# ChenKaiXuSan/Skiing_Analysis_PyTorch

Hardware: AMD Instinct MI355X
Metric: 3D-pose frames/sec, 8-view 518px clips (higher is better)
Workload: dtype f16

## Files before the change

include/skimi.h:

```cpp
#ifndef SKIMI_H
#define SKIMI_H

#include <stddef.h>
#include <stdint.h>

#ifdef __cplusplus
extern "C" {
#endif

#define SKIMI_OK 0
#define SKIMI_ERR_ARG (-1)
#define SKIMI_ERR_HIP (-2)
#define SKIMI_ERR_STATE (-3)
#define SKIMI_ERR_WORKSPACE (-4)

#define SKIMI_F32 0
#define SKIMI_BF16 1
#define SKIMI_BF16X3_REC 2
#define SKIMI_FP8MX 3
#define SKIMI_F16 4

#define SKIMI_PREC_BF16 0
#define SKIMI_PREC_BF16X3 1
#define SKIMI_PREC_FP8 2
#define SKIMI_PREC_F16 3

#define SKIMI_ACT_NONE 0
#define SKIMI_ACT_RELU 1
#define SKIMI_ACT_GELU 2
#define SKIMI_ACT_SILU 3
#define SKIMI_ACT_SIGMOID 4

const char* skimi_last_error(void);
int skimi_version(void);
int skimi_sizeof_gemm_desc(void);
int skimi_device_count(void);

int skimi_profile_start(int32_t kind, int64_t min_size);
int skimi_profile_stop(double* total_ms, int64_t* launches, double* flops, double* bytes);

typedef struct skimi_gemm_desc {
    int32_t M, N, K;
    const void* A;
    const void* W;
    int32_t a_dtype, w_dtype;
    int64_t lda, ldw;
    int32_t prec;
    int32_t a_mode;
    int32_t cN, cH, cW, cC, KH, KW, stride, pad, dil, OH, OW;
    const float* bias;
    const float* gamma;
    const void* resid;
    int32_t resid_dtype;
    int64_t ldr;
    int32_t resid_rows_per_batch;
    int64_t resid_batch_stride;
    int64_t resid_row_off;
    int32_t act;
    const void* resid2;
    int64_t ldr2;
    int32_t post_act;
    int32_t out_rows_per_batch;
    int64_t out_batch_stride;
    int64_t out_row_off;
    void* out;
    void* out2;
    int32_t out_dtype;
    int64_t ldo, ldo2;
    int32_t store_mode, ps_s, ps_C;
    void* splitk_scratch;
    uint64_t splitk_scratch_bytes;
    int32_t force_splitk;
    int32_t splitk_scratch_zeroed;
    const void* W_split;
    void* x3_scratch;
    uint64_t x3_scratch_bytes;
    void* out_records;
} skimi_gemm_desc;

int skimi_split_planes(const float* x, int64_t ld, int64_t rows, int32_t C, void* hi, void* lo, void* stream);

int skimi_split_records(const float* x, int64_t ld, int64_t rows, int32_t C, void* records, void* stream);

int skimi_dpt_fold_pack(const float* w_T, const float* b_T, const float* w_rn, int32_t C_in, int32_t C_mid, int32_t C_out,
                        int32_t s, void* w_records, float* beta, void* stream);

int skimi_gemm(const skimi_gemm_desc* d, void* stream);

#define SKIMI_GEMM_PATH_GENERIC 1
#define SKIMI_GEMM_PATH_SPLITK_ORDERED 2
#define SKIMI_GEMM_PATH_SPLITK_ATOMIC 3
#define SKIMI_GEMM_PATH_X3DMA_WIDE 4
#define SKIMI_GEMM_PATH_X3DMA_NARROW 5
#define SKIMI_GEMM_PATH_GEMM256 6
#define SKIMI_GEMM_PATH_CONV_WIN 7
int32_t skimi_gemm_last_path(void);

int skimi_quant_mx(const void* x, int32_t dtype, int64_t ldx, int64_t rows, int32_t K, void* payload, void* scales,
                   void* stream);
int skimi_layernorm_mx(const float* x, int64_t ldx, int64_t rows, int32_t C, const float* gamma, const float* beta,
                       float eps, void* payload, void* scales, void* stream);
int skimi_gemm_fp8(const void* A, const void* A_scales, const void* W, const void* W_scales, int32_t M, int32_t N,
                   int32_t K, const float* bias, int32_t act, const float* gamma, const float* resid, int64_t ldr,
                   void* out, int32_t out_dtype, int64_t ldo, void* out_scales, void* stream);

int skimi_conv3x3_n32_pack(const float* w, void* packed, int32_t C, void* stream);
int skimi_conv3x3_n32(const void* in_hi, const void* in_lo, const void* packed_w, const float* bias, float* out,
                      int32_t F, int32_t H, int32_t W, int32_t C, int32_t relu, void* stream);
int skimi_conv3x3_n32_strided(const void* in_hi, const void* in_lo, const void* packed_w, const float* bias, float* out,
                              int32_t F, int32_t H, int32_t W, int32_t C, int32_t relu, int64_t px_stride, void* stream);

int skimi_resample_u8(const uint8_t* in, uint8_t* out, int64_t outer, int32_t n_in, int32_t n_out, int64_t inner,
                      const int32_t* kk, const int32_t* bounds, int32_t ksize, void* stream);
int skimi_u8_hwc_to_f32_chw(const uint8_t* in, int32_t H, int32_t W, float* out, int32_t OH, int32_t OW, int32_t y_off,
                            int32_t x_off, float fill, void* stream);

int skimi_layernorm(const float* x, const float* x2, int64_t ldx, int64_t rows, int32_t C,
                    const float* gamma, const float* beta, float eps,
                    void* out, int32_t out_dtype, int64_t ldo, void* stream);

int skimi_qknorm_rope(void* qkv, int32_t dtype, int64_t tokens, int32_t heads,
                      const float* qn_w, const float* qn_b, const float* kn_w, const float* kn_b,
                      float eps, const int32_t* pos, const float* rope_cos, const float* rope_sin,
                      int32_t rope_npos, void* stream);

int skimi_attention(const void* qkv, void* out, int32_t dtype, int32_t batch, int32_t seq,
                    int32_t heads, int32_t head_dim, void* stream);
int skimi_attention_out(const void* qkv, void* out, int32_t dtype, int32_t out_dtype, int32_t batch, int32_t seq,
                        int32_t heads, int32_t head_dim, void* stream);

int skimi_qknorm_rope_scaled(void* qkv, int32_t dtype, int64_t tokens, int32_t heads,
                             const float* qn_w, const float* qn_b, const float* kn_w, const float* kn_b,
                             float eps, const int32_t* pos, const float* rope_cos, const float* rope_sin,
                             int32_t rope_npos, float q_scale, int32_t* q_scaled, void* stream);
int skimi_attention_ex(const void* qkv, void* out, int32_t dtype, int32_t out_dtype, int32_t batch, int32_t seq,
                       int32_t heads, int32_t head_dim, int32_t q_prescaled, void* x3_scratch,
                       uint64_t x3_scratch_bytes, int32_t* out_records, void* stream);
uint64_t skimi_attention_x3_scratch_bytes(int64_t tokens, int64_t row_elems);
void skimi_attention_last_plan(int32_t out[8]);

int skimi_layernorm_ex(const float* x, const float* x2, int64_t ldx, int64_t in_rows, int64_t rows, int32_t C,
                       const float* gamma, const float* beta, float eps, void* out, int32_t out_dtype, int64_t ldo,
                       int64_t grp_rows, int64_t grp_stride, int64_t grp_off, void* stream);
int skimi_attention_f32_strided(const float* q, const float* k, const float* v, float* out, const int64_t* q_strides,
                                const int64_t* k_strides, const int64_t* v_strides, const int64_t* o_strides,
                                int32_t batch, int32_t batch_inner, int32_t heads, int32_t seq_q, int32_t seq_k,
                                int32_t head_dim, float scale, void* stream);

typedef struct skimi_vp3d skimi_vp3d;

skimi_vp3d* skimi_vp3d_create(int32_t joints_in, int32_t in_features, int32_t joints_out,
                              const int32_t* filter_widths, int32_t n_widths,
                              int32_t channels, int32_t causal);
skimi_vp3d* skimi_vp3d_create_ex(int32_t joints_in, int32_t in_features, int32_t joints_out,
                                 const int32_t* filter_widths, int32_t n_widths,
                                 int32_t channels, int32_t causal, int32_t dense);
void skimi_vp3d_destroy(skimi_vp3d*);
int skimi_vp3d_set_weight(skimi_vp3d*, const char* key, const float* host_data, int64_t n);
int skimi_vp3d_finalize(skimi_vp3d*, int32_t prec);
int32_t skimi_vp3d_receptive_field(const skimi_vp3d*);
size_t skimi_vp3d_workspace_bytes(const skimi_vp3d*, int32_t batch, int32_t frames_in);
int skimi_vp3d_forward(skimi_vp3d*, const float* x, float* out, int32_t batch, int32_t frames_in,
                       void* workspace, size_t workspace_bytes, void* stream);

typedef struct skimi_vggt skimi_vggt;

typedef struct skimi_vggt_config {
    int32_t patch_size, embed_dim, depth, num_heads, num_register_tokens;
    int32_t use_dino;
    int32_t dino_depth, dino_heads, dino_img_size;
    int32_t cam_trunk_depth, cam_heads, cam_iters;
    int32_t dpt_features, dpt_out_channels[4], dpt_layers[4];
    int32_t track_features, track_hidden, track_corr_levels, track_corr_radius, track_iters, track_depth,
        track_heads, track_virtual;
    int32_t enable_camera, enable_depth, enable_point, enable_track;
    int32_t prec;
    int32_t head_prec;
} skimi_vggt_config;

skimi_vggt* skimi_vggt_create(const skimi_vggt_config* cfg);
void skimi_vggt_destroy(skimi_vggt*);
int skimi_vggt_set_weight(skimi_vggt*, const char* key, const float* data, int64_t n, int32_t on_device);
int skimi_vggt_finalize(skimi_vggt*);
int skimi_vggt_set_pos_embed(skimi_vggt*, int32_t H, int32_t W, const float* pos_embed, int32_t on_device);
size_t skimi_vggt_workspace_bytes(skimi_vggt*, int32_t B, int32_t S, int32_t H, int32_t W, int32_t n_query);
int skimi_vggt_rope_positions(skimi_vggt*, int32_t frames, int32_t H, int32_t W, int32_t* positions);

typedef struct skimi_vggt_outputs {
    float* pose_enc;
    float* pose_enc_list;
    float* depth;
    float* depth_conf;
    float* world_points;
    float* world_points_conf;
    float* track;
    float* vis;
    float* conf;
    float* tokens_last;
} skimi_vggt_outputs;

int skimi_vggt_forward(skimi_vggt*, const float* images, const float* query_points, int32_t B, int32_t S,
                       int32_t H, int32_t W, int32_t n_query, const skimi_vggt_outputs* out,
                       void* workspace, size_t workspace_bytes, void* stream);

int skimi_pose_to_cameras(const float* pose_enc, int64_t rows, int32_t H, int32_t W, float* extrinsic,
                          float* intrinsic, void* stream);
int skimi_unproject_depth(const float* depth, const float* extrinsic, const float* intrinsic,
                          float* world_points, int32_t frames, int32_t H, int32_t W, void* stream);
int skimi_triangulate_dlt(const float* K, const float* R, const float* t, const float* keypoints,
                          float* joints3d, int64_t steps, int32_t views, int32_t joints, void* stream);

int skimi_triangulate_triage(const float* K, const float* R, const float* t, const float* keypoints, const float* conf,
                             double conf_thr, double err_thresh_px, int64_t steps, int32_t views, int32_t joints,
                             float* joints3d, float* joints3d_clean, double* err, double* depth, uint8_t* keep,
                             double* view_stats, double* report, void* stream);

int skimi_triangulate_robust(const float* K, const float* R, const float* t, const float* keypoints, const float* conf,
                             double conf_thr, double inlier_px, int32_t min_inliers, int32_t refine_iters, int32_t weighted,
                             int64_t steps, int32_t views, int32_t joints, float* joints3d, double* err,
                             uint8_t* inlier_views, double* rms_px, uint8_t* ok, float* joints3d_ok,
                             double* view_inlier_ratio, double* report, void* stream);

size_t skimi_person_workspace_bytes(int64_t maps, int32_t H, int32_t W);
int skimi_person_origin(const float* points, const float* boxes, int64_t maps, int32_t H, int32_t W, int32_t src_h,
                        int32_t src_w, void* workspace, double* stats, void* stream);
int skimi_recenter_cameras(const double* stats, const float* extrinsic, int64_t steps, int32_t views, double* origin_out,
                           float* R_out, float* t_out, void* stream);

size_t skimi_icp_workspace_bytes(int64_t n_src, int64_t n_tgt);
int skimi_estimate_normals(const float* points, int64_t n, double radius, double* normals_out,
                           int32_t* neighbour_count_out, void* ws, size_t ws_bytes, void* stream);
int skimi_icp_correspondences(const float* src, int64_t n_src, const float* tgt, int64_t n_tgt, const double* T4x4,
                              double max_dist, int32_t* tgt_index_out, void* ws, size_t ws_bytes, void* stream);
int skimi_icp_point_to_plane(const float* src, int64_t n_src, const float* tgt, int64_t n_tgt, double max_corr_dist,
                             double normal_radius, int32_t max_iteration, double rel_fitness, double rel_rmse,
                             const double* init4x4, double* T_out, double* fitness_out, double* rmse_out,
                             int32_t* iterations_out, void* ws, size_t ws_bytes, void* stream);

#define SKIMI_BA_POSE_ONLY 0
#define SKIMI_BA_POSE_CAM_T 1
#define SKIMI_BA_FULL 2
#define SKIMI_BA_AUTO 0
#define SKIMI_BA_LDS 1
#define SKIMI_BA_WORKSPACE 2
size_t skimi_ba_workspace_bytes(int64_t T, int32_t C, int32_t J, int32_t modes);
int skimi_bundle_adjust(const double* K, const double* R0, const double* t0, const double* X0, const double* x2d,
                        const double* conf, int64_t T, int32_t C, int32_t J, const int32_t* modes, int32_t n_modes,
                        int32_t num_iters, double lr, double w_reproj, double w_smooth, double w_baseline,
                        double w_bone_length, double w_pose_temporal, int32_t placement, double* R_out, double* t_out,
                        double* X_out, double* history_out, void* ws, size_t ws_bytes, void* stream);

#define SKIMI_RESECT_LINEAR 0
#define SKIMI_RESECT_SOFT_L1 1
size_t skimi_resect_workspace_bytes(int64_t n_points, int32_t views, int64_t group_size);
int skimi_resect_cameras(const double* X, const double* x2d, const double* conf, const double* K, const double* R0,
                         const double* t0, int64_t n_points, int32_t views, int64_t group_size, int32_t loss, double f_scale,
                         double min_conf, int32_t max_evals, double* R, double* t, double* K_out, double* cost0, double* cost,
                         int32_t* n_evals, int32_t* n_used, int32_t* success, double* err, double* stats, void* ws,
                         size_t ws_bytes, void* stream);
int skimi_relative_pose(const double* R, const double* t, int64_t groups, int32_t views, double* R_rel, double* t_rel,
                        void* stream);

size_t skimi_refine_workspace_bytes(int64_t n_points, int32_t views, int64_t group_size);
int skimi_refine_cameras_points(const double* X, const double* x2d, const double* conf, const double* K, const double* R0,
                                const double* t0, int64_t n_points, int32_t views, int64_t group_size, double lambda_x,
                                int32_t loss, double f_scale, double min_conf, int32_t max_evals, double* R, double* t,
                                double* K_out, double* X_opt, double* cost0, double* cost, int32_t* n_evals, int32_t* n_used,
                                int32_t* success, double* err, double* stats, double* moved, void* ws, size_t ws_bytes,
                                void* stream);

size_t skimi_essential_workspace_bytes(int64_t n_points, int64_t group_size, int32_t hypotheses);
int skimi_essential_ransac(const double* x2d, const double* conf, const double* K, int64_t n_points, int64_t group_size,
                           double min_conf, double threshold, int32_t hypotheses, uint64_t seed, int64_t group_offset,
                           double baseline, double distance_thresh, double* R, double* t, double* E, uint8_t* inliers,
                           uint8_t* pose_mask, int32_t* n_used, int32_t* n_inliers, int32_t* n_pose, int32_t* cheirality,
                           double* cost, int32_t* winner, int32_t* n_solutions, double* confidence, int32_t* success,
                           void* ws, size_t ws_bytes, void* stream);
int skimi_five_point(const double* a, const double* b, int64_t samples, double* E, int32_t* counts, void* stream);

int64_t skimi_scene_tile(int64_t n);
size_t skimi_scene_workspace_bytes(int64_t B, int64_t n);
int skimi_scene_cloud(const float* points, const float* conf, const float* images, const float* extrinsic, int64_t B, int32_t S,
                      int32_t H, int32_t W, int32_t images_nchw, double conf_thres, int32_t mask_black_bg, int32_t mask_white_bg,
                      int32_t align, int64_t cap, void* workspace, float* xyz, uint8_t* rgb, int64_t* count, double* stats,
                      double* transform, void* stream);

int skimi_fuse_h36m(const double* left, const double* right, int64_t frames, double tau, const double* tau_j, const double* wL,
                    int64_t wL_stride, const double* wR, int64_t wR_stride, int32_t allow_scale, int32_t mirror_right_x,
                    double* fused, double* R, double* t, double* s, double* diag, int32_t* status, void* stream);

#define SKIMI_FUSE_SCALE_HIP 0
#define SKIMI_FUSE_SCALE_TORSO 1
int skimi_fuse_views(const double* X_l, const double* X_r, const double* U_l, const double* U_r, int64_t frames, int32_t joints,
                     int32_t root_idx, int32_t left_hip_idx, int32_t right_hip_idx, int32_t left_shoulder_idx,
                     int32_t right_shoulder_idx, double sigma_px, double sigma_3d, int32_t scale_mode, int32_t min_points,
                     double* fused, double* aligned, double* q_l, double* q_r, double* conf_l, double* conf_r, double* conf_x,
                     double* err_l, double* err_r, double* dist, int32_t* fit_ok, void* stream);

int skimi_smooth_ema(const double* X, int64_t frames, int64_t joints, const double* base, int32_t adaptive, double alpha_min,
                     double alpha_max, double speed_gain, double* Y, void* stream);

int skimi_smooth_ema_batch(const double* X, int64_t clips, int64_t frames, int64_t joints, const double* base, int32_t adaptive,
                           double alpha_min, double alpha_max, double speed_gain, double* Y, void* stream);

size_t skimi_fuse_group_workspace_bytes(int64_t views, int64_t frames, int32_t joints);
int skimi_fuse_group(const double* X, const double* U, const double* quality, int64_t views, int64_t frames, int32_t joints,
                     int32_t root_idx, int32_t left_hip_idx, int32_t right_hip_idx, int32_t left_shoulder_idx,
                     int32_t right_shoulder_idx, double sigma_px, double sigma_3d, int32_t scale_mode, int32_t min_points,
                     int32_t align, void* workspace, size_t workspace_bytes, double* fused, double* aligned, double* q_a, double* q_b,
                     double* conf_x, double* dist, double* conf, double* err, int32_t* fit_ok, void* stream);

int skimi_joint_quality(const double* X, const double* U, int64_t views, int64_t frames, int32_t joints, const int32_t* edges,
                        int32_t n_edges, const double* size, double beta_temp, double w_bone, double w_temp, double w_san,
                        int32_t med_given, const double* bias, int64_t bias_stride, double* med_lens, double* q, double* q_bone,
                        double* q_temp, double* q_san, void* stream);

#define SKIMI_SKELETON_COCO_TO_H36M 0
#define SKIMI_SKELETON_H36M_TO_COCO 1
int skimi_convert_skeleton(const double* X, int64_t frames, int32_t coords, int32_t direction, int32_t synthesize, double* Y,
                           void* stream);

int skimi_smooth_savgol(const double* X, int64_t frames, int64_t joints, int32_t win, int32_t poly, const double* fir,
                        const double* first, const double* last, double* Y, void* stream);

#define SKIMI_KIN_SERIES 42
#define SKIMI_KIN_BASE_SERIES 14
#define SKIMI_KIN_ROLES 13
#define SKIMI_KIN_LDS_FRAMES 2048
enum {
    SKIMI_KIN_SHOULDER_L = 0, SKIMI_KIN_SHOULDER_R, SKIMI_KIN_ELBOW_L, SKIMI_KIN_ELBOW_R, SKIMI_KIN_HIP_L, SKIMI_KIN_HIP_R,
    SKIMI_KIN_KNEE_L, SKIMI_KIN_KNEE_R, SKIMI_KIN_FOOT_L, SKIMI_KIN_FOOT_R, SKIMI_KIN_HAND_L, SKIMI_KIN_HAND_R, SKIMI_KIN_NECK
};
size_t skimi_kin_workspace_bytes(int64_t clips, int64_t frames);
int skimi_kinematics(const double* X, const int32_t* lengths, int64_t clips, int64_t frames, int32_t joints,
                     const int32_t* layout, const double* up, int32_t min_turn_frames, double min_heading_change_deg,
                     int32_t heading_window, int32_t velocity_window, int32_t max_turns, void* workspace,
                     size_t workspace_bytes, double* series, double* heading, double* heading_smooth, double* velocity_smooth,
                     uint8_t* boundary, int32_t* n_turns, int32_t* turn_frames, double* turn_heading_change,
                     int32_t* turn_direction, double* turn_stats, int32_t* turn_counts, void* stream);

#define SKIMI_EVAL_MAX_JOINTS 128
#define SKIMI_EVAL_MAX_EDGES 128
#define SKIMI_EVAL_MAX_PAIRS 64
#define SKIMI_EVAL_LDS_ELEMS 1440
enum { SKIMI_PE_MPJPE = 0, SKIMI_PE_P_MPJPE, SKIMI_PE_N_MPJPE, SKIMI_PE_MPJVE };
enum {
    SKIMI_CQ_BONE_CV_POOLED = 0, SKIMI_CQ_BONE_CV_MEAN, SKIMI_CQ_LR_LENGTH_SYMMETRY, SKIMI_CQ_SPEED_MEAN, SKIMI_CQ_JERK_MEAN,
    SKIMI_CQ_SPEED_P95, SKIMI_CQ_ACCEL_P95, SKIMI_CQ_MIRROR_SYMMETRY, SKIMI_CQ_SCALARS
};
size_t skimi_eval_workspace_bytes(int64_t clips, int64_t frames, int32_t joints);
int skimi_pose_errors(const double* pred, const double* target, const int32_t* lengths, int64_t clips, int64_t frames, int32_t joints,
                      int32_t zero_root, double* err, double* p_err, double* vel_err, double* mpjpe_f, double* n_mpjpe_f,
                      double* p_mpjpe_f, int32_t* n_valid_f, int32_t* p_status, double* aligned, double* p_R, double* p_scale,
                      double* p_t, double* metrics, int32_t* counts, double* joint_stats, int32_t* joint_n, void* stream);
int skimi_clip_quality(const double* X, const int32_t* lengths, int64_t clips, int64_t frames, int32_t joints, const int32_t* edges,
                       int32_t n_edges, const int32_t* left_edges, int32_t n_left, const int32_t* right_edges, int32_t n_right,
                       const int32_t* lr_pairs, int32_t n_pairs, void* workspace, size_t workspace_bytes, double* scalars,
                       double* bone_cv_edge, double* bone_len, void* stream);

#define SKIMI_LENS_MAX_CAMERAS 8
#define SKIMI_LENS_MAX_ITERS 1000
#define SKIMI_LENS_MAX_SIDE 32768
int skimi_distort_points(const double* x, const double* K, const double* dist, const double* P, const double* K_steps,
                         int64_t outer, int32_t C, int64_t n, int32_t normalized, double* out, void* stream);
int skimi_undistort_points(const double* x, const double* K, const double* dist, const double* P, const double* K_steps,
                           int64_t outer, int32_t C, int64_t n, int32_t iters, int32_t normalized, double* out, double* resid_px,
                           void* stream);
int skimi_project_points(const double* X, const double* R, const double* t, const double* K, const double* dist, int64_t outer,
                         int32_t C, int64_t n, double* px, double* depth, void* stream);
int skimi_undistort_u8(const uint8_t* in, uint8_t* out, const double* K, const double* dist, const double* new_K, int32_t C,
                       int32_t F, int32_t H, int32_t W, int32_t OH, int32_t OW, int32_t ch, void* stream);

int skimi_homography_fit(const double* src, const double* dst, const double* post, int64_t G, int32_t n, double* H, double* Hinv,
                         double* Hn, double* err, double* stats, int32_t* status, void* stream);
int skimi_homography_points(const double* x, const double* H, int64_t G, int64_t n, int32_t shared, double eps, double* out,
                            void* stream);
int skimi_warp_perspective_u8(const uint8_t* in, uint8_t* out, const double* Hinv, int32_t per_frame, int32_t C, int32_t F,
                              int32_t H, int32_t W, int32_t OH, int32_t OW, int32_t ch, void* stream);
int skimi_bev_skeleton(const double* X, const double* center_px, const double* center_world_in, int64_t T, int32_t J,
                       double metres_per_pixel, int32_t ax0, int32_t ax1, int32_t rot90_left, double* uv, int32_t* px, uint8_t* valid,
                       double* center_world, void* stream);
int skimi_ground_track(const double* p, int64_t P, int64_t T, double fps, double* out, void* stream);

size_t skimi_calibrate_workspace_bytes(int64_t G, int32_t V, int32_t n);
int skimi_calibrate_camera(const double* obj, const double* img, const uint8_t* use, const double* K0, const double* dist0, int64_t G,
                           int32_t V, int32_t n, int32_t width, int32_t height, int32_t free_mask, int32_t max_evals, double* K,
                           double* dist, double* R, double* t, double* rvec, double* err, double* view_stats, double* rms,
                           double* cost0, double* cost, double* std, int32_t* n_evals, int32_t* n_views, int32_t* n_corners,
                           int32_t* success, void* ws, size_t ws_bytes, void* stream);

#define SKIMI_CHESS_MAX_PIXELS (1 << 28)
#define SKIMI_CHESS_MAX_NMS 15
#define SKIMI_SUBPIX_MAX_WIN 15
#define SKIMI_SUBPIX_MAX_ITERS 1000
size_t skimi_chess_workspace_bytes(int64_t N, int32_t H, int32_t W);
int skimi_chess_candidates(const uint8_t* frames, int64_t N, int32_t H, int32_t W, int32_t ch, int32_t threshold, int32_t nms_radius,
                           int32_t max_candidates, int32_t* xy, int32_t* response, int32_t* count, int32_t* rmax, void* ws,
                           size_t ws_bytes, void* stream);
int skimi_corner_subpix(const uint8_t* frames, int64_t N, int32_t H, int32_t W, int32_t ch, const double* points, const int32_t* count,
                        int32_t M, int32_t win_x, int32_t win_y, int32_t iters, double* out, uint8_t* ok, void* stream);

#define SKIMI_ORB_MAX_LEVELS 8
#define SKIMI_ORB_MAX_FEATURES 4096
#define SKIMI_ORB_BORDER 16
#define SKIMI_ORB_PATTERN_SEED 0x534B494D494F5242ULL
#define SKIMI_ORB_COS                                                                                                          \
    {16384, 16069, 15137, 13623, 11585, 9102, 6270, 3196, 0, -3196, -6270, -9102, -11585, -13623, -15137, -16069, -16384, -16069, \
     -15137, -13623, -11585, -9102, -6270, -3196, 0, 3196, 6270, 9102, 11585, 13623, 15137, 16069}
#define SKIMI_ORB_SIN                                                                                                          \
    {0, 3196, 6270, 9102, 11585, 13623, 15137, 16069, 16384, 16069, 15137, 13623, 11585, 9102, 6270, 3196, 0, -3196, -6270, -9102, \
     -11585, -13623, -15137, -16069, -16384, -16069, -15137, -13623, -11585, -9102, -6270, -3196}
size_t skimi_orb_workspace_bytes(int64_t N, int32_t H, int32_t W, int32_t levels);
int skimi_orb_features(const uint8_t* frames, int64_t N, int32_t H, int32_t W, int32_t ch, int32_t levels, int32_t threshold,
                       int32_t max_features, const double* roi, const int8_t* pattern, int32_t* xy_level, double* xy,
                       int32_t* level, int32_t* direction, int32_t* score, int64_t* harris, int32_t* desc, int32_t* count,
                       int32_t* level_count, void* ws, size_t ws_bytes, void* stream);
int skimi_match_hamming(const int32_t* d1, const int32_t* n1, int32_t M1, const int32_t* d2, const int32_t* n2, int32_t M2,
                        int64_t B, int32_t cross_check, double ratio, int32_t max_distance, int32_t max_matches, int32_t* pairs,
                        int32_t* dist, int32_t* count, void* stream);

#define SKIMI_SIFT_MAX_OCTAVES 8
#define SKIMI_SIFT_MAX_FEATURES 4096
#define SKIMI_SIFT_MAX_CANDIDATES 32768
#define SKIMI_SIFT_BORDER 5
#define SKIMI_SIFT_MIN_SIDE 16
#define SKIMI_SIFT_MAX_RADIUS 13
#define SKIMI_SIFT_RADII {7, 5, 7, 8, 10, 13}
#define SKIMI_SIFT_PRETHRESH 1.7f
#define SKIMI_SIFT_CONTRAST 3.4
#define SKIMI_SIFT_CBRT4 1.5874010519681994
#define SKIMI_SIFT_LN2 0.6931471805599453
size_t skimi_sift_workspace_bytes(int64_t N, int32_t H, int32_t W, int32_t octaves);
int skimi_sift_features(const uint8_t* frames, int64_t N, int32_t H, int32_t W, int32_t ch, int32_t octaves, int32_t max_features,
                        const double* roi, const float* taps, double* xy, int32_t* xy_level, int32_t* octave, int32_t* layer,
                        double* sigma, double* response, double* angle, uint8_t* desc, int32_t* count, int32_t* octave_count,
                        void* ws, size_t ws_bytes, void* stream);
int skimi_match_l2(const uint8_t* d1, const int32_t* n1, int32_t M1, const uint8_t* d2, const int32_t* n2, int32_t M2, int64_t B,
                   int32_t cross_check, double ratio, int32_t max_distance2, int32_t max_matches, int32_t* pairs, int32_t* dist2,
                   int32_t* second2, int32_t* count, void* ws, size_t ws_bytes, void* stream);


int skimi_resize_bilinear(const void* in, void* out, int32_t dtype, int32_t out_dtype, int32_t N, int32_t h, int32_t w,
                          int32_t H, int32_t W, int32_t C, const float* tabx, const float* taby, const float* ln_g,
                          const float* ln_b, float ln_eps, void* stream);
int skimi_resize_bilinear_planes(const float* in, void* out, int32_t N, int32_t h, int32_t w, int32_t H, int32_t W,
                                 int32_t C, const float* tabx, const float* taby, int32_t slice_records, void* zpage,
                                 void* stream);
int skimi_add_uv_pos(void* x, int32_t dtype, const float* tabx, const float* taby, int32_t N, int32_t H, int32_t W,
                     int32_t C, void* stream);
int skimi_add_uv_pos_records(const float* x, const float* tabx, const float* taby, int32_t N, int32_t H, int32_t W,
                             int32_t C, void* rec, void* stream);
int skimi_dpt_out(const void* in, int32_t dtype, const float* W, const float* b, int32_t n_out, float* pts, float* conf,
                  int64_t npix, int32_t mode, void* stream);
int skimi_patch_gather(const float* img, void* out, int32_t out_dtype, int32_t F, int32_t H, int32_t W, int32_t p,
                       int32_t Kp, void* stream);
int skimi_adaln(const float* xn, const float* x, const float* mod, float* out, int64_t rows, int32_t D, void* stream);
int skimi_pose_update(const float* delta, float* pred_pad, float* act_out, int64_t rows, int32_t first, void* stream);
int skimi_special_tokens(float* x, const float* table, int32_t F, int32_t S, int32_t P, int32_t n, int32_t C, void* stream);

int skimi_track_avgpool2(const float* in, float* out, int32_t N, int32_t H, int32_t W, int32_t C, void* stream);
int skimi_track_sample_border(const float* fmap, int64_t img_stride, const float* coords, int64_t coord_stride, float* out,
                              int32_t B, int32_t N, int32_t H, int32_t W, int32_t C, void* stream);
int skimi_track_corr_sample(const float* tgt, const float* fmap, const float* coords, float* out, int64_t rows, int32_t N,
                            int32_t S, int32_t H, int32_t W, int32_t C, int32_t r, int32_t level, int64_t ldo,
                            int32_t out_off, void* stream);
int skimi_track_pos_embed_sample(const float* coords, int64_t coord_stride, float* out, int32_t BN, int32_t H, int32_t W,
                                 int32_t D, void* stream);
int skimi_track_input(const float* coords, const float* fcorr, const float* tfeat, const float* pos, const float* qrt,
                      float* x, int64_t rows, int32_t S, int32_t L, int64_t ldx, float max_scale, void* stream);
int skimi_track_coord_update(float* coords, const float* delta, int64_t ldd, const float* query, float* pred, int64_t rows,
                             int32_t N, int32_t S, float stride, void* stream);
int skimi_track_init(const float* q, float* coords, float* qs, int64_t BN, int32_t S, float stride, void* stream);
int skimi_track_repeat_rows(const float* src, float* dst, int64_t BN, int32_t S, int32_t C, void* stream);
int skimi_track_bns_to_bsn(const float* in, float* out, int32_t B, int32_t N, int32_t S, void* stream);


int skimi_vp3d_pack_weights(const float* w_host, int32_t N, int32_t Npad, int32_t K, void* dst);
int skimi_vp3d_stream_mm(const void* wrec, int32_t Npad, const void* xrec, const float* bias, const float* resid, int32_t resid_L,
                         int32_t resid_off, float* out_f32, int32_t ldo, void* out_rec, int32_t B, int32_t Lin, int32_t C,
                         int32_t taps, int32_t dil, int32_t N, int32_t relu, int32_t force_family, int32_t force_ct,
                         int32_t force_nw, int32_t force_ms, void* stream);
int skimi_vp3d_stream_win(const void* wrec, int32_t Npad, const void* xrec, const float* bias, float* out_f32, int32_t ldo,
                          void* out_rec, int32_t B, int32_t Lin, int32_t C, int32_t taps, int32_t N, int32_t force_ta,
                          int32_t force_msc, void* stream);
int skimi_vp3d_stream_expand(const float* x, const void* w, int32_t ldw, const float* bias, float* out_f32, void* out_rec,
                             int32_t B, int32_t Lin, int32_t Cin, int32_t taps, int32_t C, int32_t valu, int32_t force_ms,
                             void* stream);
void skimi_vp3d_last_plan(int32_t out[8]);

#ifdef __cplusplus
}
#endif
#endif
```

skiing_analysis_pytorch_amd/_lib.py:

```python
from __future__ import annotations

import ctypes as C
from pathlib import Path

LIB_PATH = Path(__file__).resolve().parent / "lib" / "libskimi.so"

F32, BF16 = 0, 1
F16 = 4
BF16X3_REC = 2
FP8MX = 3
PREC_BF16, PREC_BF16X3, PREC_FP8 = 0, 1, 2
PREC_F16 = 3
ACT_NONE, ACT_RELU, ACT_GELU, ACT_SILU, ACT_SIGMOID = 0, 1, 2, 3, 4
GEMM_PATH_GENERIC, GEMM_PATH_SPLITK_ORDERED, GEMM_PATH_SPLITK_ATOMIC = 1, 2, 3
GEMM_PATH_X3DMA_WIDE, GEMM_PATH_X3DMA_NARROW, GEMM_PATH_GEMM256, GEMM_PATH_CONV_WIN = 4, 5, 6, 7
VP3D_CONV, VP3D_MM, VP3D_WIN, VP3D_EXPAND_MFMA, VP3D_EXPAND_VALU = 1, 2, 3, 4, 5


class SkimiError(RuntimeError):
    pass


class GemmDesc(C.Structure):

    _fields_ = [
        ("M", C.c_int32), ("N", C.c_int32), ("K", C.c_int32),
        ("A", C.c_void_p), ("W", C.c_void_p),
        ("a_dtype", C.c_int32), ("w_dtype", C.c_int32),
        ("lda", C.c_int64), ("ldw", C.c_int64),
        ("prec", C.c_int32),
        ("a_mode", C.c_int32),
        ("cN", C.c_int32), ("cH", C.c_int32), ("cW", C.c_int32), ("cC", C.c_int32),
        ("KH", C.c_int32), ("KW", C.c_int32), ("stride", C.c_int32), ("pad", C.c_int32),
        ("dil", C.c_int32), ("OH", C.c_int32), ("OW", C.c_int32),
        ("bias", C.c_void_p), ("gamma", C.c_void_p), ("resid", C.c_void_p),
        ("resid_dtype", C.c_int32),
        ("ldr", C.c_int64),
        ("resid_rows_per_batch", C.c_int32),
        ("resid_batch_stride", C.c_int64),
        ("resid_row_off", C.c_int64),
        ("act", C.c_int32),
        ("resid2", C.c_void_p), ("ldr2", C.c_int64), ("post_act", C.c_int32),
        ("out_rows_per_batch", C.c_int32), ("out_batch_stride", C.c_int64), ("out_row_off", C.c_int64),
        ("out", C.c_void_p), ("out2", C.c_void_p),
        ("out_dtype", C.c_int32),
        ("ldo", C.c_int64), ("ldo2", C.c_int64),
        ("store_mode", C.c_int32), ("ps_s", C.c_int32), ("ps_C", C.c_int32),
        ("splitk_scratch", C.c_void_p),
        ("splitk_scratch_bytes", C.c_uint64),
        ("force_splitk", C.c_int32), ("splitk_scratch_zeroed", C.c_int32),
        ("W_split", C.c_void_p), ("x3_scratch", C.c_void_p), ("x3_scratch_bytes", C.c_uint64),
        ("out_records", C.c_void_p),
    ]


_vp = C.c_void_p
_SIGNATURES = {
    "skimi_last_error": (C.c_char_p, []),
    "skimi_version": (C.c_int, []),
    "skimi_sizeof_gemm_desc": (C.c_int, []),
    "skimi_device_count": (C.c_int, []),
    "skimi_profile_start": (C.c_int, [C.c_int32, C.c_int64]),
    "skimi_profile_stop": (C.c_int, [C.POINTER(C.c_double), C.POINTER(C.c_int64), C.POINTER(C.c_double),
                                    C.POINTER(C.c_double)]),
    "skimi_gemm": (C.c_int, [C.POINTER(GemmDesc), _vp]),
    "skimi_gemm_last_path": (C.c_int32, []),
    "skimi_dpt_fold_pack": (C.c_int, [_vp, _vp, _vp, C.c_int32, C.c_int32, C.c_int32, C.c_int32, _vp, _vp, _vp]),
    "skimi_quant_mx": (C.c_int, [_vp, C.c_int32, C.c_int64, C.c_int64, C.c_int32, _vp, _vp, _vp]),
    "skimi_layernorm_mx": (C.c_int, [_vp, C.c_int64, C.c_int64, C.c_int32, _vp, _vp, C.c_float, _vp, _vp, _vp]),
    "skimi_gemm_fp8": (C.c_int, [_vp, _vp, _vp, _vp, C.c_int32, C.c_int32, C.c_int32, _vp, C.c_int32, _vp, _vp, C.c_int64,
                                 _vp, C.c_int32, C.c_int64, _vp, _vp]),
    "skimi_split_planes": (C.c_int, [_vp, C.c_int64, C.c_int64, C.c_int32, _vp, _vp, _vp]),
    "skimi_split_records": (C.c_int, [_vp, C.c_int64, C.c_int64, C.c_int32, _vp, _vp]),
    "skimi_resample_u8": (C.c_int, [_vp, _vp, C.c_int64, C.c_int32, C.c_int32, C.c_int64, _vp, _vp, C.c_int32, _vp]),
    "skimi_u8_hwc_to_f32_chw": (C.c_int, [_vp, C.c_int32, C.c_int32, _vp, C.c_int32, C.c_int32, C.c_int32, C.c_int32,
                                          C.c_float, _vp]),
    "skimi_conv3x3_n32_pack": (C.c_int, [_vp, _vp, C.c_int32, _vp]),
    "skimi_conv3x3_n32": (C.c_int, [_vp, _vp, _vp, _vp, _vp, C.c_int32, C.c_int32, C.c_int32, C.c_int32, C.c_int32, _vp]),
    "skimi_conv3x3_n32_strided": (C.c_int, [_vp, _vp, _vp, _vp, _vp, C.c_int32, C.c_int32, C.c_int32, C.c_int32, C.c_int32,
                                            C.c_int64, _vp]),
    "skimi_layernorm": (C.c_int, [_vp, _vp, C.c_int64, C.c_int64, C.c_int32, _vp, _vp, C.c_float, _vp,
                                  C.c_int32, C.c_int64, _vp]),
    "skimi_qknorm_rope": (C.c_int, [_vp, C.c_int32, C.c_int64, C.c_int32, _vp, _vp, _vp, _vp, C.c_float,
                                    _vp, _vp, _vp, C.c_int32, _vp]),
    "skimi_attention": (C.c_int, [_vp, _vp, C.c_int32, C.c_int32, C.c_int32, C.c_int32, C.c_int32, _vp]),
    "skimi_attention_out": (C.c_int, [_vp, _vp, C.c_int32, C.c_int32, C.c_int32, C.c_int32, C.c_int32, C.c_int32, _vp]),
    "skimi_qknorm_rope_scaled": (C.c_int, [_vp, C.c_int32, C.c_int64, C.c_int32, _vp, _vp, _vp, _vp, C.c_float,
                                           _vp, _vp, _vp, C.c_int32, C.c_float, C.POINTER(C.c_int32), _vp]),
    "skimi_attention_ex": (C.c_int, [_vp, _vp, C.c_int32, C.c_int32, C.c_int32, C.c_int32, C.c_int32, C.c_int32, C.c_int32,
                                     _vp, C.c_uint64, C.POINTER(C.c_int32), _vp]),
    "skimi_attention_x3_scratch_bytes": (C.c_uint64, [C.c_int64, C.c_int64]),
    "skimi_attention_last_plan": (None, [C.POINTER(C.c_int32)]),
    "skimi_layernorm_ex": (C.c_int, [_vp, _vp, C.c_int64, C.c_int64, C.c_int64, C.c_int32, _vp, _vp, C.c_float, _vp,
                                     C.c_int32, C.c_int64, C.c_int64, C.c_int64, C.c_int64, _vp]),
    "skimi_attention_f32_strided": (C.c_int, [_vp, _vp, _vp, _vp, C.POINTER(C.c_int64), C.POINTER(C.c_int64),
                                              C.POINTER(C.c_int64), C.POINTER(C.c_int64), C.c_int32, C.c_int32, C.c_int32,
                                              C.c_int32, C.c_int32, C.c_int32, C.c_float, _vp]),
    "skimi_vp3d_create": (_vp, [C.c_int32, C.c_int32, C.c_int32, C.POINTER(C.c_int32), C.c_int32,
                                C.c_int32, C.c_int32]),
    "skimi_vp3d_create_ex": (_vp, [C.c_int32, C.c_int32, C.c_int32, C.POINTER(C.c_int32), C.c_int32,
                                   C.c_int32, C.c_int32, C.c_int32]),
    "skimi_vp3d_destroy": (None, [_vp]),
    "skimi_vp3d_set_weight": (C.c_int, [_vp, C.c_char_p, _vp, C.c_int64]),
    "skimi_vp3d_finalize": (C.c_int, [_vp, C.c_int32]),
    "skimi_vp3d_receptive_field": (C.c_int32, [_vp]),
    "skimi_vp3d_workspace_bytes": (C.c_size_t, [_vp, C.c_int32, C.c_int32]),
    "skimi_vp3d_forward": (C.c_int, [_vp, _vp, _vp, C.c_int32, C.c_int32, _vp, C.c_size_t, _vp]),
    "skimi_vp3d_pack_weights": (C.c_int, [_vp, C.c_int32, C.c_int32, C.c_int32, _vp]),
    "skimi_vp3d_stream_mm": (C.c_int, [_vp, C.c_int32, _vp, _vp, _vp, C.c_int32, C.c_int32, _vp, C.c_int32, _vp, C.c_int32,
                                       C.c_int32, C.c_int32, C.c_int32, C.c_int32, C.c_int32, C.c_int32, C.c_int32, C.c_int32,
                                       C.c_int32, C.c_int32, _vp]),
    "skimi_vp3d_stream_win": (C.c_int, [_vp, C.c_int32, _vp, _vp, _vp, C.c_int32, _vp, C.c_int32, C.c_int32, C.c_int32,
                                        C.c_int32, C.c_int32, C.c_int32, C.c_int32, _vp]),
    "skimi_vp3d_stream_expand": (C.c_int, [_vp, _vp, C.c_int32, _vp, _vp, _vp, C.c_int32, C.c_int32, C.c_int32, C.c_int32,
                                           C.c_int32, C.c_int32, C.c_int32, _vp]),
    "skimi_vp3d_last_plan": (None, [C.POINTER(C.c_int32)]),
    "skimi_pose_to_cameras": (C.c_int, [_vp, C.c_int64, C.c_int32, C.c_int32, _vp, _vp, _vp]),
    "skimi_unproject_depth": (C.c_int, [_vp, _vp, _vp, _vp, C.c_int32, C.c_int32, C.c_int32, _vp]),
    "skimi_triangulate_dlt": (C.c_int, [_vp, _vp, _vp, _vp, _vp, C.c_int64, C.c_int32, C.c_int32, _vp]),
    "skimi_triangulate_triage": (C.c_int, [_vp, _vp, _vp, _vp, _vp, C.c_double, C.c_double, C.c_int64, C.c_int32, C.c_int32,
                                           _vp, _vp, _vp, _vp, _vp, _vp, _vp, _vp]),
    "skimi_triangulate_robust": (C.c_int, [_vp, _vp, _vp, _vp, _vp, C.c_double, C.c_double, C.c_int32, C.c_int32, C.c_int32,
                                           C.c_int64, C.c_int32, C.c_int32, _vp, _vp, _vp, _vp, _vp, _vp, _vp, _vp, _vp]),
    "skimi_person_workspace_bytes": (C.c_size_t, [C.c_int64, C.c_int32, C.c_int32]),
    "skimi_person_origin": (C.c_int, [_vp, _vp, C.c_int64, C.c_int32, C.c_int32, C.c_int32, C.c_int32, _vp, _vp, _vp]),
    "skimi_recenter_cameras": (C.c_int, [_vp, _vp, C.c_int64, C.c_int32, _vp, _vp, _vp, _vp]),
    "skimi_icp_workspace_bytes": (C.c_size_t, [C.c_int64, C.c_int64]),
    "skimi_estimate_normals": (C.c_int, [_vp, C.c_int64, C.c_double, _vp, _vp, _vp, C.c_size_t, _vp]),
    "skimi_icp_correspondences": (C.c_int, [_vp, C.c_int64, _vp, C.c_int64, C.POINTER(C.c_double), C.c_double, _vp, _vp,
                                            C.c_size_t, _vp]),
    "skimi_icp_point_to_plane": (C.c_int, [_vp, C.c_int64, _vp, C.c_int64, C.c_double, C.c_double, C.c_int32, C.c_double,
                                           C.c_double, C.POINTER(C.c_double), C.POINTER(C.c_double), C.POINTER(C.c_double),
                                           C.POINTER(C.c_double), C.POINTER(C.c_int32), _vp, C.c_size_t, _vp]),
    "skimi_ba_workspace_bytes": (C.c_size_t, [C.c_int64, C.c_int32, C.c_int32, C.c_int32]),
    "skimi_bundle_adjust": (C.c_int, [_vp, _vp, _vp, _vp, _vp, _vp, C.c_int64, C.c_int32, C.c_int32, C.POINTER(C.c_int32),
                                      C.c_int32, C.c_int32, C.c_double, C.c_double, C.c_double, C.c_double, C.c_double,
                                      C.c_double, C.c_int32, _vp, _vp, _vp, _vp, _vp, C.c_size_t, _vp]),
    "skimi_resect_workspace_bytes": (C.c_size_t, [C.c_int64, C.c_int32, C.c_int64]),
    "skimi_resect_cameras": (C.c_int, [_vp, _vp, _vp, _vp, _vp, _vp, C.c_int64, C.c_int32, C.c_int64, C.c_int32, C.c_double,
                                       C.c_double, C.c_int32, _vp, _vp, _vp, _vp, _vp, _vp, _vp, _vp, _vp, _vp, _vp, C.c_size_t,
                                       _vp]),
    "skimi_relative_pose": (C.c_int, [_vp, _vp, C.c_int64, C.c_int32, _vp, _vp, _vp]),
    "skimi_refine_workspace_bytes": (C.c_size_t, [C.c_int64, C.c_int32, C.c_int64]),
    "skimi_refine_cameras_points": (C.c_int, [_vp, _vp, _vp, _vp, _vp, _vp, C.c_int64, C.c_int32, C.c_int64, C.c_double, C.c_int32,
                                              C.c_double, C.c_double, C.c_int32, _vp, _vp, _vp, _vp, _vp, _vp, _vp, _vp, _vp, _vp,
                                              _vp, _vp, _vp, C.c_size_t, _vp]),
    "skimi_essential_workspace_bytes": (C.c_size_t, [C.c_int64, C.c_int64, C.c_int32]),
    "skimi_essential_ransac": (C.c_int, [_vp, _vp, _vp, C.c_int64, C.c_int64, C.c_double, C.c_double, C.c_int32, C.c_uint64,
                                         C.c_int64, C.c_double, C.c_double, _vp, _vp, _vp, _vp, _vp, _vp, _vp, _vp, _vp, _vp, _vp,
                                         _vp, _vp, _vp, _vp, C.c_size_t, _vp]),
    "skimi_five_point": (C.c_int, [_vp, _vp, C.c_int64, _vp, _vp, _vp]),
    "skimi_scene_tile": (C.c_int64, [C.c_int64]),
    "skimi_scene_workspace_bytes": (C.c_size_t, [C.c_int64, C.c_int64]),
    "skimi_scene_cloud": (C.c_int, [_vp, _vp, _vp, _vp, C.c_int64, C.c_int32, C.c_int32, C.c_int32, C.c_int32, C.c_double,
                                    C.c_int32, C.c_int32, C.c_int32, C.c_int64, _vp, _vp, _vp, _vp, _vp, _vp, _vp]),
    "skimi_fuse_h36m": (C.c_int, [_vp, _vp, C.c_int64, C.c_double, _vp, _vp, C.c_int64, _vp, C.c_int64, C.c_int32, C.c_int32,
                                  _vp, _vp, _vp, _vp, _vp, _vp, _vp]),
    "skimi_fuse_views": (C.c_int, [_vp, _vp, _vp, _vp, C.c_int64, C.c_int32, C.c_int32, C.c_int32, C.c_int32, C.c_int32, C.c_int32,
                                   C.c_double, C.c_double, C.c_int32, C.c_int32, _vp, _vp, _vp, _vp, _vp, _vp, _vp, _vp, _vp, _vp,
                                   _vp, _vp]),
    "skimi_smooth_ema": (C.c_int, [_vp, C.c_int64, C.c_int64, _vp, C.c_int32, C.c_double, C.c_double, C.c_double, _vp, _vp]),
    "skimi_smooth_ema_batch": (C.c_int, [_vp, C.c_int64, C.c_int64, C.c_int64, _vp, C.c_int32, C.c_double, C.c_double, C.c_double,
                                         _vp, _vp]),
    "skimi_fuse_group_workspace_bytes": (C.c_size_t, [C.c_int64, C.c_int64, C.c_int32]),
    "skimi_fuse_group": (C.c_int, [_vp, _vp, _vp, C.c_int64, C.c_int64, C.c_int32, C.c_int32, C.c_int32, C.c_int32, C.c_int32,
                                   C.c_int32, C.c_double, C.c_double, C.c_int32, C.c_int32, C.c_int32, _vp, C.c_size_t, _vp, _vp,
                                   _vp, _vp, _vp, _vp, _vp, _vp, _vp, _vp]),
    "skimi_joint_quality": (C.c_int, [_vp, _vp, C.c_int64, C.c_int64, C.c_int32, _vp, C.c_int32, _vp, C.c_double, C.c_double,
                                      C.c_double, C.c_double, C.c_int32, _vp, C.c_int64, _vp, _vp, _vp, _vp, _vp, _vp]),
    "skimi_convert_skeleton": (C.c_int, [_vp, C.c_int64, C.c_int32, C.c_int32, C.c_int32, _vp, _vp]),
    "skimi_smooth_savgol": (C.c_int, [_vp, C.c_int64, C.c_int64, C.c_int32, C.c_int32, _vp, _vp, _vp, _vp, _vp]),
    "skimi_kin_workspace_bytes": (C.c_size_t, [C.c_int64, C.c_int64]),
    "skimi_kinematics": (C.c_int, [_vp, _vp, C.c_int64, C.c_int64, C.c_int32, C.POINTER(C.c_int32), C.POINTER(C.c_double), C.c_int32,
                                   C.c_double, C.c_int32, C.c_int32, C.c_int32, _vp, C.c_size_t, _vp, _vp, _vp, _vp, _vp, _vp, _vp, _vp,
                                   _vp, _vp, _vp, _vp]),
    "skimi_eval_workspace_bytes": (C.c_size_t, [C.c_int64, C.c_int64, C.c_int32]),
    "skimi_pose_errors": (C.c_int, [_vp, _vp, _vp, C.c_int64, C.c_int64, C.c_int32, C.c_int32, _vp, _vp, _vp, _vp, _vp, _vp, _vp, _vp,
                                    _vp, _vp, _vp, _vp, _vp, _vp, _vp, _vp, _vp]),
    "skimi_clip_quality": (C.c_int, [_vp, _vp, C.c_int64, C.c_int64, C.c_int32, C.POINTER(C.c_int32), C.c_int32, C.POINTER(C.c_int32),
                                     C.c_int32, C.POINTER(C.c_int32), C.c_int32, C.POINTER(C.c_int32), C.c_int32, _vp, C.c_size_t, _vp,
                                     _vp, _vp, _vp]),
    "skimi_distort_points": (C.c_int, [_vp, _vp, _vp, _vp, _vp, C.c_int64, C.c_int32, C.c_int64, C.c_int32, _vp, _vp]),
    "skimi_undistort_points": (C.c_int, [_vp, _vp, _vp, _vp, _vp, C.c_int64, C.c_int32, C.c_int64, C.c_int32, C.c_int32, _vp, _vp,
                                         _vp]),
    "skimi_project_points": (C.c_int, [_vp, _vp, _vp, _vp, _vp, C.c_int64, C.c_int32, C.c_int64, _vp, _vp, _vp]),
    "skimi_undistort_u8": (C.c_int, [_vp, _vp, _vp, _vp, _vp, C.c_int32, C.c_int32, C.c_int32, C.c_int32, C.c_int32, C.c_int32,
                                     C.c_int32, _vp]),
    "skimi_homography_fit": (C.c_int, [_vp, _vp, _vp, C.c_int64, C.c_int32, _vp, _vp, _vp, _vp, _vp, _vp, _vp]),
    "skimi_homography_points": (C.c_int, [_vp, _vp, C.c_int64, C.c_int64, C.c_int32, C.c_double, _vp, _vp]),
    "skimi_warp_perspective_u8": (C.c_int, [_vp, _vp, _vp, C.c_int32, C.c_int32, C.c_int32, C.c_int32, C.c_int32, C.c_int32,
                                            C.c_int32, C.c_int32, _vp]),
    "skimi_bev_skeleton": (C.c_int, [_vp, _vp, _vp, C.c_int64, C.c_int32, C.c_double, C.c_int32, C.c_int32, C.c_int32, _vp, _vp, _vp,
                                     _vp, _vp]),
    "skimi_ground_track": (C.c_int, [_vp, C.c_int64, C.c_int64, C.c_double, _vp, _vp]),
    "skimi_calibrate_workspace_bytes": (C.c_size_t, [C.c_int64, C.c_int32, C.c_int32]),
    "skimi_calibrate_camera": (C.c_int, [_vp, _vp, _vp, _vp, _vp, C.c_int64, C.c_int32, C.c_int32, C.c_int32, C.c_int32, C.c_int32,
                                         C.c_int32, _vp, _vp, _vp, _vp, _vp, _vp, _vp, _vp, _vp, _vp, _vp, _vp, _vp, _vp, _vp, _vp,
                                         C.c_size_t, _vp]),
    "skimi_chess_workspace_bytes": (C.c_size_t, [C.c_int64, C.c_int32, C.c_int32]),
    "skimi_chess_candidates": (C.c_int, [_vp, C.c_int64, C.c_int32, C.c_int32, C.c_int32, C.c_int32, C.c_int32, C.c_int32, _vp, _vp,
                                         _vp, _vp, _vp, C.c_size_t, _vp]),
    "skimi_corner_subpix": (C.c_int, [_vp, C.c_int64, C.c_int32, C.c_int32, C.c_int32, _vp, _vp, C.c_int32, C.c_int32, C.c_int32,
                                      C.c_int32, _vp, _vp, _vp]),
    "skimi_orb_workspace_bytes": (C.c_size_t, [C.c_int64, C.c_int32, C.c_int32, C.c_int32]),
    "skimi_orb_features": (C.c_int, [_vp, C.c_int64, C.c_int32, C.c_int32, C.c_int32, C.c_int32, C.c_int32, C.c_int32, _vp, _vp, _vp,
                                     _vp, _vp, _vp, _vp, _vp, _vp, _vp, _vp, _vp, C.c_size_t, _vp]),
    "skimi_match_hamming": (C.c_int, [_vp, _vp, C.c_int32, _vp, _vp, C.c_int32, C.c_int64, C.c_int32, C.c_double, C.c_int32,
                                      C.c_int32, _vp, _vp, _vp, _vp]),
    "skimi_sift_workspace_bytes": (C.c_size_t, [C.c_int64, C.c_int32, C.c_int32, C.c_int32]),
    "skimi_sift_features": (C.c_int, [_vp, C.c_int64, C.c_int32, C.c_int32, C.c_int32, C.c_int32, C.c_int32, _vp, _vp, _vp, _vp, _vp,
                                      _vp, _vp, _vp, _vp, _vp, _vp, _vp, _vp, C.c_size_t, _vp]),
    "skimi_match_l2": (C.c_int, [_vp, _vp, C.c_int32, _vp, _vp, C.c_int32, C.c_int64, C.c_int32, C.c_double, C.c_int32, C.c_int32,
                                 _vp, _vp, _vp, _vp, _vp, C.c_size_t, _vp]),
    "skimi_resize_bilinear": (C.c_int, [_vp, _vp, C.c_int32, C.c_int32, C.c_int32, C.c_int32, C.c_int32, C.c_int32, C.c_int32, C.c_int32, _vp, _vp, _vp, _vp, C.c_float, _vp]),
    "skimi_resize_bilinear_planes": (C.c_int, [_vp, _vp, C.c_int32, C.c_int32, C.c_int32, C.c_int32, C.c_int32, C.c_int32, _vp, _vp, C.c_int32, _vp, _vp]),
    "skimi_add_uv_pos": (C.c_int, [_vp, C.c_int32, _vp, _vp, C.c_int32, C.c_int32, C.c_int32, C.c_int32, _vp]),
    "skimi_add_uv_pos_records": (C.c_int, [_vp, _vp, _vp, C.c_int32, C.c_int32, C.c_int32, C.c_int32, _vp, _vp]),
    "skimi_dpt_out": (C.c_int, [_vp, C.c_int32, _vp, _vp, C.c_int32, _vp, _vp, C.c_int64, C.c_int32, _vp]),
    "skimi_patch_gather": (C.c_int, [_vp, _vp, C.c_int32, C.c_int32, C.c_int32, C.c_int32, C.c_int32, C.c_int32, _vp]),
    "skimi_adaln": (C.c_int, [_vp, _vp, _vp, _vp, C.c_int64, C.c_int32, _vp]),
    "skimi_pose_update": (C.c_int, [_vp, _vp, _vp, C.c_int64, C.c_int32, _vp]),
    "skimi_special_tokens": (C.c_int, [_vp, _vp, C.c_int32, C.c_int32, C.c_int32, C.c_int32, C.c_int32, _vp]),
    "skimi_track_avgpool2": (C.c_int, [_vp, _vp, C.c_int32, C.c_int32, C.c_int32, C.c_int32, _vp]),
    "skimi_track_sample_border": (C.c_int, [_vp, C.c_int64, _vp, C.c_int64, _vp, C.c_int32, C.c_int32, C.c_int32, C.c_int32, C.c_int32, _vp]),
    "skimi_track_corr_sample": (C.c_int, [_vp, _vp, _vp, _vp, C.c_int64, C.c_int32, C.c_int32, C.c_int32, C.c_int32, C.c_int32, C.c_int32, C.c_int32, C.c_int64, C.c_int32, _vp]),
    "skimi_track_pos_embed_sample": (C.c_int, [_vp, C.c_int64, _vp, C.c_int32, C.c_int32, C.c_int32, C.c_int32, _vp]),
    "skimi_track_input": (C.c_int, [_vp, _vp, _vp, _vp, _vp, _vp, C.c_int64, C.c_int32, C.c_int32, C.c_int64, C.c_float, _vp]),
    "skimi_track_coord_update": (C.c_int, [_vp, _vp, C.c_int64, _vp, _vp, C.c_int64, C.c_int32, C.c_int32, C.c_float, _vp]),
    "skimi_track_init": (C.c_int, [_vp, _vp, _vp, C.c_int64, C.c_int32, C.c_float, _vp]),
    "skimi_track_repeat_rows": (C.c_int, [_vp, _vp, C.c_int64, C.c_int32, C.c_int32, _vp]),
    "skimi_track_bns_to_bsn": (C.c_int, [_vp, _vp, C.c_int32, C.c_int32, C.c_int32, _vp]),
    "skimi_vggt_create": (_vp, [_vp]),
    "skimi_vggt_destroy": (None, [_vp]),
    "skimi_vggt_set_weight": (C.c_int, [_vp, C.c_char_p, _vp, C.c_int64, C.c_int32]),
    "skimi_vggt_finalize": (C.c_int, [_vp]),
    "skimi_vggt_set_pos_embed": (C.c_int, [_vp, C.c_int32, C.c_int32, _vp, C.c_int32]),
    "skimi_vggt_rope_positions": (C.c_int, [_vp, C.c_int32, C.c_int32, C.c_int32, _vp]),
    "skimi_vggt_workspace_bytes": (C.c_size_t, [_vp, C.c_int32, C.c_int32, C.c_int32, C.c_int32, C.c_int32]),
    "skimi_vggt_forward": (C.c_int, [_vp, _vp, _vp, C.c_int32, C.c_int32, C.c_int32, C.c_int32, C.c_int32, _vp,
                                     _vp, C.c_size_t, _vp]),
}

_lib = None


def exported_symbols():
    return sorted(_SIGNATURES)


def lib() -> C.CDLL:
    global _lib
    if _lib is not None:
        return _lib
    if not LIB_PATH.exists():
        raise SkimiError(
            f"{LIB_PATH} not found: build it with `python -m skiing_analysis_pytorch_amd.build` "
            "(or __graft_entry__.build()). There is no fallback path."
        )
    import torch

    handle = C.CDLL(str(LIB_PATH))
    for name, (res, args) in _SIGNATURES.items():
        try:
            fn = getattr(handle, name)
        except AttributeError as e:
            raise SkimiError(f"libskimi.so does not export {name}") from e
        fn.restype = res
        fn.argtypes = args
    if handle.skimi_sizeof_gemm_desc() != C.sizeof(GemmDesc):
        raise SkimiError(f"skimi_gemm_desc is {handle.skimi_sizeof_gemm_desc()} bytes in libskimi.so but "
                         f"{C.sizeof(GemmDesc)} in _lib.py: rebuild the library (python -m skiing_analysis_pytorch_amd.build)")
    _lib = handle
    return _lib


def check(rc: int, what: str = "") -> None:
    if rc != 0:
        msg = lib().skimi_last_error()
        raise SkimiError(f"{what} failed ({rc}): {msg.decode() if msg else ''}")


def ptr(t) -> int | None:
    if t is None:
        return None
    return t.data_ptr()


def current_stream() -> int:
    import torch

    return torch.cuda.current_stream().cuda_stream
```

skiing_analysis_pytorch_amd/csrc/api.hip:

```cpp
#include <stdarg.h>

#include <mutex>
#include <vector>

#include "common.h"
#include "gemm_epilogue.h"
#include "kernels.h"
#include "track_kernels.h"
#include "vggt_kernels.h"

namespace skimi {

static thread_local char g_err[512] = "";

void set_error(const char* fmt, ...) {
    va_list ap;
    va_start(ap, fmt);
    vsnprintf(g_err, sizeof(g_err), fmt, ap);
    va_end(ap);
}

int lds_opt_in(std::atomic<unsigned>& done, const void* kernel, int bytes, const char* what) {
    int dev = 0;
    if (hipGetDevice(&dev) != hipSuccess) {
        set_error("hipGetDevice failed (%s)", what);
        return SKIMI_ERR_HIP;
    }
    const unsigned bit = 1u << (dev & 31);
    if (done.load(std::memory_order_acquire) & bit) return SKIMI_OK;
    const hipError_t e = hipFuncSetAttribute(kernel, hipFuncAttributeMaxDynamicSharedMemorySize, bytes);
    if (e != hipSuccess) {
        set_error("hipFuncSetAttribute(%s, %d bytes of LDS) failed: %s", what, bytes, hipGetErrorString(e));
        return SKIMI_ERR_HIP;
    }
    done.fetch_or(bit, std::memory_order_release);
    return SKIMI_OK;
}

struct ProfState {
    int kind = PROF_NONE;
    long min_key = 0;
    std::vector<std::pair<hipEvent_t, hipEvent_t>> ev;
    std::vector<std::pair<hipEvent_t, hipEvent_t>> pool;
    double flops = 0, bytes = 0;
    hipEvent_t pending = nullptr;
};
static ProfState g_prof;
static std::mutex g_prof_mu;
static thread_local size_t tl_prof_idx = 0;

bool prof_armed(int kind, long size_key) { return g_prof.kind == kind && size_key >= g_prof.min_key; }
void prof_before(hipStream_t st) {
    std::lock_guard<std::mutex> lk(g_prof_mu);
    std::pair<hipEvent_t, hipEvent_t> e;
    if (!g_prof.pool.empty()) {
        e = g_prof.pool.back();
        g_prof.pool.pop_back();
    } else {
        (void)hipEventCreate(&e.first);
        (void)hipEventCreate(&e.second);
    }
    (void)hipEventRecord(e.first, st);
    g_prof.ev.push_back(e);
    tl_prof_idx = g_prof.ev.size() - 1;
}
void prof_after(hipStream_t st, double flops, double bytes) {
    std::lock_guard<std::mutex> lk(g_prof_mu);
    if (tl_prof_idx >= g_prof.ev.size()) return;
    (void)hipEventRecord(g_prof.ev[tl_prof_idx].second, st);
    g_prof.flops += flops;
    g_prof.bytes += bytes;
}

}

using namespace skimi;

extern "C" {

const char* skimi_last_error(void) { return g_err; }

int skimi_version(void) { return 100; }
int skimi_sizeof_gemm_desc(void) { return (int)sizeof(skimi_gemm_desc); }

int skimi_device_count(void) {
    int n = 0;
    if (hipGetDeviceCount(&n) != hipSuccess) return 0;
    return n;
}

int skimi_profile_start(int32_t kind, int64_t min_size) {
    SKIMI_CHECK_ARG(kind == PROF_ATTN_BF16 || kind == PROF_GEMM, "skimi_profile_start: unknown kernel kind %d", kind);
    for (auto& e : g_prof.ev) g_prof.pool.push_back(e);
    g_prof.ev.clear();
    g_prof.flops = g_prof.bytes = 0;
    g_prof.kind = kind;
    g_prof.min_key = min_size;
    return SKIMI_OK;
}

int skimi_profile_stop(double* total_ms, int64_t* launches, double* flops, double* bytes) {
    double ms = 0;
    for (auto& e : g_prof.ev) {
        SKIMI_HIP(hipEventSynchronize(e.second));
        float t = 0;
        SKIMI_HIP(hipEventElapsedTime(&t, e.first, e.second));
        ms += t;
    }
    if (total_ms) *total_ms = ms;
    if (launches) *launches = (int64_t)g_prof.ev.size();
    if (flops) *flops = g_prof.flops;
    if (bytes) *bytes = g_prof.bytes;
    for (auto& e : g_prof.ev) g_prof.pool.push_back(e);
    g_prof.ev.clear();
    g_prof.kind = PROF_NONE;
    return SKIMI_OK;
}

int32_t skimi_gemm_last_path(void) { return gemm_last_path(); }

int skimi_gemm(const skimi_gemm_desc* d, void* stream) {
    if (!d) {
        set_gemm_path(0, 0, 0, 0, 0);
        set_error("skimi_gemm: null descriptor");
        return SKIMI_ERR_ARG;
    }
    return gemm_dispatch(d, (hipStream_t)stream, d->splitk_scratch, (size_t)d->splitk_scratch_bytes,
                         d->force_splitk);
}

int skimi_resample_u8(const uint8_t* in, uint8_t* out, int64_t outer, int32_t n_in, int32_t n_out, int64_t inner,
                      const int32_t* kk, const int32_t* bounds, int32_t ksize, void* stream) {
    return resample_u8_launch(in, out, outer, n_in, n_out, inner, kk, bounds, ksize, (hipStream_t)stream);
}

int skimi_u8_hwc_to_f32_chw(const uint8_t* in, int32_t H, int32_t W, float* out, int32_t OH, int32_t OW, int32_t y_off,
                            int32_t x_off, float fill, void* stream) {
    return u8_hwc_to_f32_chw_launch(in, H, W, out, OH, OW, y_off, x_off, fill, (hipStream_t)stream);
}

int skimi_conv3x3_n32_pack(const float* w, void* packed, int32_t C, void* stream) {
    SKIMI_CHECK_ARG(w && packed && C > 0, "skimi_conv3x3_n32_pack: bad arguments");
    return conv_direct_pack_launch(w, (unsigned short*)packed, C, (hipStream_t)stream);
}

int skimi_conv3x3_n32(const void* in_hi, const void* in_lo, const void* packed_w, const float* bias, float* out,
                      int32_t F, int32_t H, int32_t W, int32_t C, int32_t relu, void* stream) {
    return conv_direct_n32_launch((const unsigned short*)in_hi, (const unsigned short*)in_lo,
                                  (const unsigned short*)packed_w, bias, out, F, H, W, C, relu, (hipStream_t)stream);
}

int skimi_conv3x3_n32_strided(const void* in_hi, const void* in_lo, const void* packed_w, const float* bias, float* out,
                              int32_t F, int32_t H, int32_t W, int32_t C, int32_t relu, int64_t px_stride, void* stream) {
    SKIMI_CHECK_ARG(px_stride > 0, "skimi_conv3x3_n32_strided: px_stride must be positive");
    return conv_direct_n32_launch((const unsigned short*)in_hi, (const unsigned short*)in_lo,
                                  (const unsigned short*)packed_w, bias, out, F, H, W, C, relu, (hipStream_t)stream,
                                  (long)px_stride);
}

int skimi_split_planes(const float* x, int64_t ld, int64_t rows, int32_t C, void* hi, void* lo, void* stream) {
    SKIMI_CHECK_ARG(x && hi && lo && rows > 0 && C > 0, "skimi_split_planes: bad arguments");
    return split_planes_launch(x, (long)ld, (long)rows, C, hi, lo, (hipStream_t)stream);
}

int skimi_split_records(const float* x, int64_t ld, int64_t rows, int32_t C, void* records, void* stream) {
    SKIMI_CHECK_ARG(x && records && rows > 0 && C > 0, "skimi_split_records: bad arguments");
    return split_records_launch(x, (long)ld, (long)rows, C, records, (hipStream_t)stream);
}

int skimi_dpt_fold_pack(const float* w_T, const float* b_T, const float* w_rn, int32_t C_in, int32_t C_mid, int32_t C_out,
                        int32_t s, void* w_records, float* beta, void* stream) {
    SKIMI_CHECK_ARG(w_T && w_rn && w_records && beta, "skimi_dpt_fold_pack: null buffer");
    SKIMI_CHECK_ARG(s >= 2 && s <= 16 && C_in > 0 && C_in % 32 == 0 && C_mid > 0 && C_out > 0, "skimi_dpt_fold_pack: bad sizes");
    float* tmp = nullptr;
    SKIMI_HIP(hipMalloc((void**)&tmp, (size_t)(s + 2) * (s + 2) * C_out * C_in * 4));
    const int rc = dpt_fold_pack_launch(w_T, b_T, w_rn, C_in, C_mid, C_out, s, tmp, w_records, beta, (hipStream_t)stream);
    const hipError_t e = hipStreamSynchronize((hipStream_t)stream);
    (void)hipFree(tmp);
    if (rc) return rc;
    SKIMI_HIP(e);
    return SKIMI_OK;
}

int skimi_quant_mx(const void* x, int32_t dtype, int64_t ldx, int64_t rows, int32_t K, void* payload, void* scales,
                   void* stream) {
    return quant_mx_launch(x, dtype, (long)ldx, (long)rows, K, payload, scales, (hipStream_t)stream);
}

int skimi_layernorm_mx(const float* x, int64_t ldx, int64_t rows, int32_t C, const float* gamma, const float* beta,
                       float eps, void* payload, void* scales, void* stream) {
    return layernorm_mx_launch(x, ldx, rows, C, gamma, beta, eps, payload, scales, (hipStream_t)stream);
}

int skimi_gemm_fp8(const void* A, const void* A_scales, const void* W, const void* W_scales, int32_t M, int32_t N,
                   int32_t K, const float* bias, int32_t act, const float* gamma, const float* resid, int64_t ldr,
                   void* out, int32_t out_dtype, int64_t ldo, void* out_scales, void* stream) {
    return gemm_fp8_launch(A, A_scales, W, W_scales, M, N, K, bias, act, gamma, resid, (long)ldr, out, out_dtype, (long)ldo,
                           (hipStream_t)stream, out_scales);
}

int skimi_layernorm(const float* x, const float* x2, int64_t ldx, int64_t rows, int32_t C,
                    const float* gamma, const float* beta, float eps, void* out, int32_t out_dtype,
                    int64_t ldo, void* stream) {
    return layernorm_launch(x, x2, ldx, rows, C, gamma, beta, eps, out, out_dtype, ldo,
                            (hipStream_t)stream);
}

int skimi_qknorm_rope(void* qkv, int32_t dtype, int64_t tokens, int32_t heads, const float* qn_w,
                      const float* qn_b, const float* kn_w, const float* kn_b, float eps,
                      const int32_t* pos, const float* rope_cos, const float* rope_sin,
                      int32_t rope_npos, void* stream) {
    return qknorm_rope_launch(qkv, dtype, tokens, heads, qn_w, qn_b, kn_w, kn_b, eps, pos, rope_cos,
                              rope_sin, rope_npos, (hipStream_t)stream);
}

static int attention_entry(const void* qkv, void* out, int32_t dtype, int32_t out_dtype, int32_t batch, int32_t seq, int32_t heads,
                           int32_t head_dim, int32_t q_prescaled, void* x3_scratch, uint64_t x3_scratch_bytes,
                           int32_t* out_records, void* stream) {
    AttnRequest r = {};
    r.qkv = qkv; r.out = out; r.dtype = dtype; r.out_dtype = out_dtype;
    r.batch = batch; r.seq = seq; r.heads = heads; r.head_dim = head_dim; r.q_prescaled = q_prescaled;
    r.x3_scratch = x3_scratch; r.x3_scratch_bytes = (size_t)x3_scratch_bytes;
    r.want_records = out_records != nullptr && *out_records != 0;
    return attention_launch(r, (hipStream_t)stream, out_records);
}

int skimi_attention(const void* qkv, void* out, int32_t dtype, int32_t batch, int32_t seq,
                    int32_t heads, int32_t head_dim, void* stream) {
    return attention_entry(qkv, out, dtype, dtype, batch, seq, heads, head_dim, 0, nullptr, 0, nullptr, stream);
}

int skimi_attention_out(const void* qkv, void* out, int32_t dtype, int32_t out_dtype, int32_t batch, int32_t seq,
                        int32_t heads, int32_t head_dim, void* stream) {
    return attention_entry(qkv, out, dtype, out_dtype, batch, seq, heads, head_dim, 0, nullptr, 0, nullptr, stream);
}

int skimi_qknorm_rope_scaled(void* qkv, int32_t dtype, int64_t tokens, int32_t heads, const float* qn_w,
                             const float* qn_b, const float* kn_w, const float* kn_b, float eps,
                             const int32_t* pos, const float* rope_cos, const float* rope_sin,
                             int32_t rope_npos, float q_scale, int32_t* q_scaled, void* stream) {
    return qknorm_rope_launch(qkv, dtype, tokens, heads, qn_w, qn_b, kn_w, kn_b, eps, pos, rope_cos,
                              rope_sin, rope_npos, (hipStream_t)stream, q_scale, q_scaled);
}

int skimi_attention_ex(const void* qkv, void* out, int32_t dtype, int32_t out_dtype, int32_t batch, int32_t seq,
                       int32_t heads, int32_t head_dim, int32_t q_prescaled, void* x3_scratch,
                       uint64_t x3_scratch_bytes, int32_t* out_records, void* stream) {
    return attention_entry(qkv, out, dtype, out_dtype, batch, seq, heads, head_dim, q_prescaled, x3_scratch, x3_scratch_bytes,
                           out_records, stream);
}

void skimi_attention_last_plan(int32_t out[8]) {
    if (!out) return;
    const AttnPlan& p = attention_last_plan();
    const int32_t v[8] = {p.family, p.queries, p.out_form, p.q_prescaled, (int32_t)p.grid, p.hd, p.lds_pad, 0};
    for (int i = 0; i < 8; ++i) out[i] = v[i];
}

uint64_t skimi_attention_x3_scratch_bytes(int64_t tokens, int64_t row_elems) {
    return (uint64_t)attention_x3_scratch_bytes((long)tokens, (long)row_elems);
}

static inline bool is_elem_dtype(int32_t d) { return d == SKIMI_F32 || d == SKIMI_BF16 || d == SKIMI_F16; }
static inline bool al16(const void* p) { return ((uintptr_t)p & 15) == 0; }

int skimi_layernorm_ex(const float* x, const float* x2, int64_t ldx, int64_t in_rows, int64_t rows, int32_t C,
                       const float* gamma, const float* beta, float eps, void* out, int32_t out_dtype, int64_t ldo,
                       int64_t grp_rows, int64_t grp_stride, int64_t grp_off, void* stream) {
    SKIMI_CHECK_ARG(rows > 0 && in_rows > 0 && ldx >= 0, "skimi_layernorm_ex: rows, in_rows must be positive, ldx not negative");
    SKIMI_CHECK_ARG(grp_rows >= 0, "skimi_layernorm_ex: grp_rows = %ld is negative", (long)grp_rows);
    int64_t last = rows - 1;
    if (grp_rows > 0) {
        SKIMI_CHECK_ARG(grp_off >= 0 && grp_stride >= grp_off + grp_rows,
                        "skimi_layernorm_ex: the gather needs grp_off >= 0 and grp_stride >= grp_off + grp_rows (got %ld, %ld, %ld)",
                        (long)grp_rows, (long)grp_stride, (long)grp_off);
        last = (rows - 1) / grp_rows * grp_stride + grp_off + (rows - 1) % grp_rows;
    }
    SKIMI_CHECK_ARG(last < in_rows, "skimi_layernorm_ex: input row %ld is read, the input has %ld rows", (long)last, (long)in_rows);
    SKIMI_CHECK_ARG(out_dtype == SKIMI_BF16X3_REC || ldo >= C, "skimi_layernorm_ex: ldo = %ld is below C = %d", (long)ldo, C);
    return layernorm_launch(x, x2, ldx, rows, C, gamma, beta, eps, out, out_dtype, ldo, (hipStream_t)stream, grp_rows,
                            grp_stride, grp_off);
}

int skimi_attention_f32_strided(const float* q, const float* k, const float* v, float* out, const int64_t* q_strides,
                                const int64_t* k_strides, const int64_t* v_strides, const int64_t* o_strides,
                                int32_t batch, int32_t batch_inner, int32_t heads, int32_t seq_q, int32_t seq_k,
                                int32_t head_dim, float scale, void* stream) {
    SKIMI_CHECK_ARG(q_strides && k_strides && v_strides && o_strides, "skimi_attention_f32_strided: null stride list");
    SKIMI_CHECK_ARG(batch <= 65535 && heads <= 65535, "skimi_attention_f32_strided: batch %d and heads %d are grid dimensions (<= 65535)",
                    batch, heads);
    SKIMI_CHECK_ARG(batch_inner >= 0 && (batch_inner == 0 || batch % batch_inner == 0),
                    "skimi_attention_f32_strided: batch_inner %d must divide batch %d", batch_inner, batch);
    for (int i = 0; i < 4; ++i)
        SKIMI_CHECK_ARG(q_strides[i] % 4 == 0 && k_strides[i] % 4 == 0 && v_strides[i] % 4 == 0 && o_strides[i] % 4 == 0,
                        "skimi_attention_f32_strided: every stride must be a multiple of 4 elements (16-B loads)");
    SKIMI_CHECK_ARG(al16(q) && al16(k) && al16(v) && al16(out), "skimi_attention_f32_strided: 16-byte aligned buffers");
    AttnArgs a;
    a.q = q; a.k = k; a.v = v; a.out = out;
    a.q_row = q_strides[0]; a.k_row = k_strides[0]; a.v_row = v_strides[0]; a.o_row = o_strides[0];
    a.q_head = q_strides[1]; a.k_head = k_strides[1]; a.v_head = v_strides[1]; a.o_head = o_strides[1];
    a.q_batch = q_strides[2]; a.k_batch = k_strides[2]; a.v_batch = v_strides[2]; a.o_batch = o_strides[2];
    a.q_batch2 = q_strides[3]; a.k_batch2 = k_strides[3]; a.v_batch2 = v_strides[3]; a.o_batch2 = o_strides[3];
    a.batch = batch; a.batch_inner = batch_inner; a.heads = heads; a.seq_q = seq_q; a.seq_k = seq_k; a.head_dim = head_dim;
    a.scale = scale;
    return attention_f32_launch(a, (hipStream_t)stream);
}


int skimi_resize_bilinear(const void* in, void* out, int32_t dtype, int32_t out_dtype, int32_t N, int32_t h, int32_t w,
                          int32_t H, int32_t W, int32_t C, const float* tabx, const float* taby, const float* ln_g,
                          const float* ln_b, float ln_eps, void* stream) {
    SKIMI_CHECK_ARG(in && out, "skimi_resize_bilinear: null map");
    SKIMI_CHECK_ARG(N > 0 && h > 0 && w > 0 && H > 0 && W > 0 && C > 0, "skimi_resize_bilinear: sizes must be positive");
    SKIMI_CHECK_ARG(is_elem_dtype(dtype) && (out_dtype < 0 || is_elem_dtype(out_dtype)), "skimi_resize_bilinear: bad dtype");
    SKIMI_CHECK_ARG(al16(in) && al16(out) && al16(tabx) && al16(taby), "skimi_resize_bilinear: 16-byte aligned buffers");
    return bilinear_ac_launch(in, out, dtype, N, h, w, H, W, C, (hipStream_t)stream, tabx, taby, out_dtype, ln_g, ln_b, ln_eps);
}

int skimi_resize_bilinear_planes(const float* in, void* out, int32_t N, int32_t h, int32_t w, int32_t H, int32_t W,
                                 int32_t C, const float* tabx, const float* taby, int32_t slice_records, void* zpage,
                                 void* stream) {
    SKIMI_CHECK_ARG(in && out, "skimi_resize_bilinear_planes: null map");
    SKIMI_CHECK_ARG(N > 0 && h > 0 && w > 0 && H > 0 && W > 0 && C > 0, "skimi_resize_bilinear_planes: sizes must be positive");
    SKIMI_CHECK_ARG(al16(in) && al16(out) && al16(tabx) && al16(taby) && al16(zpage),
                    "skimi_resize_bilinear_planes: 16-byte aligned buffers");
    return bilinear_ac_planes_launch(in, (unsigned short*)out, N, h, w, H, W, C, (hipStream_t)stream, tabx, taby, slice_records,
                                     zpage);
}

int skimi_add_uv_pos(void* x, int32_t dtype, const float* tabx, const float* taby, int32_t N, int32_t H, int32_t W,
                     int32_t C, void* stream) {
    SKIMI_CHECK_ARG(x && tabx && taby, "skimi_add_uv_pos: null map or table");
    SKIMI_CHECK_ARG(N > 0 && H > 0 && W > 0 && C > 0, "skimi_add_uv_pos: sizes must be positive");
    SKIMI_CHECK_ARG(is_elem_dtype(dtype), "skimi_add_uv_pos: bad dtype %d", dtype);
    SKIMI_CHECK_ARG(al16(x) && al16(tabx) && al16(taby), "skimi_add_uv_pos: 16-byte aligned buffers");
    return add_uv_pos_launch(x, dtype, tabx, taby, N, H, W, C, (hipStream_t)stream);
}

int skimi_add_uv_pos_records(const float* x, const float* tabx, const float* taby, int32_t N, int32_t H, int32_t W,
                             int32_t C, void* rec, void* stream) {
    SKIMI_CHECK_ARG(x && rec, "skimi_add_uv_pos_records: null map or records");
    SKIMI_CHECK_ARG(tabx == nullptr || taby != nullptr, "skimi_add_uv_pos_records: needs both tables or none");
    SKIMI_CHECK_ARG(N > 0 && H > 0 && W > 0 && C > 0, "skimi_add_uv_pos_records: sizes must be positive");
    SKIMI_CHECK_ARG(al16(x) && al16(tabx) && al16(taby) && al16(rec), "skimi_add_uv_pos_records: 16-byte aligned buffers");
    return add_uv_pos_records_launch(x, tabx, taby, N, H, W, C, rec, (hipStream_t)stream);
}

int skimi_dpt_out(const void* in, int32_t dtype, const float* W, const float* b, int32_t n_out, float* pts, float* conf,
                  int64_t npix, int32_t mode, void* stream) {
    SKIMI_CHECK_ARG(in && W && b && pts && conf, "skimi_dpt_out: null buffer");
    SKIMI_CHECK_ARG(npix > 0, "skimi_dpt_out: npix must be positive");
    SKIMI_CHECK_ARG(is_elem_dtype(dtype) && (mode == 0 || mode == 1), "skimi_dpt_out: bad dtype or mode");
    SKIMI_CHECK_ARG(al16(in), "skimi_dpt_out: 16-byte aligned input");
    return dpt_out_launch(in, dtype, W, b, n_out, pts, conf, (long)npix, mode, (hipStream_t)stream);
}

int skimi_patch_gather(const float* img, void* out, int32_t out_dtype, int32_t F, int32_t H, int32_t W, int32_t p,
                       int32_t Kp, void* stream) {
    SKIMI_CHECK_ARG(img && out, "skimi_patch_gather: null buffer");
    SKIMI_CHECK_ARG(F > 0 && p > 0 && H >= p && W >= p, "skimi_patch_gather: needs F > 0 and 0 < p <= H, W");
    SKIMI_CHECK_ARG(is_elem_dtype(out_dtype), "skimi_patch_gather: bad out_dtype %d", out_dtype);
    SKIMI_CHECK_ARG((long)Kp >= 3L * p * p, "skimi_patch_gather: Kp = %d is less than 3 p^2", Kp);
    return patch_gather_launch(img, out, out_dtype, F, H, W, p, Kp, (hipStream_t)stream);
}

int skimi_adaln(const float* xn, const float* x, const float* mod, float* out, int64_t rows, int32_t D, void* stream) {
    SKIMI_CHECK_ARG(xn && x && mod && out, "skimi_adaln: null buffer");
    SKIMI_CHECK_ARG(rows > 0 && D > 0, "skimi_adaln: sizes must be positive");
    return adaln_launch(xn, x, mod, out, (long)rows, D, (hipStream_t)stream);
}

int skimi_pose_update(const float* delta, float* pred_pad, float* act_out, int64_t rows, int32_t first, void* stream) {
    SKIMI_CHECK_ARG(delta && pred_pad && act_out, "skimi_pose_update: null buffer");
    SKIMI_CHECK_ARG(rows > 0, "skimi_pose_update: rows must be positive");
    return pose_update_launch(delta, pred_pad, act_out, (long)rows, first, (hipStream_t)stream);
}

int skimi_special_tokens(float* x, const float* table, int32_t F, int32_t S, int32_t P, int32_t n, int32_t C, void* stream) {
    SKIMI_CHECK_ARG(x && table, "skimi_special_tokens: null buffer");
    SKIMI_CHECK_ARG(F > 0 && S > 0 && n > 0 && C > 0, "skimi_special_tokens: sizes must be positive");
    SKIMI_CHECK_ARG(n <= P, "skimi_special_tokens: n = %d special tokens exceed the %d tokens of a frame", n, P);
    return special_tokens_launch(x, table, F, S, P, n, C, (hipStream_t)stream);
}

int skimi_track_avgpool2(const float* in, float* out, int32_t N, int32_t H, int32_t W, int32_t C, void* stream) {
    SKIMI_CHECK_ARG(in && out, "skimi_track_avgpool2: null buffer");
    SKIMI_CHECK_ARG(N > 0 && H >= 2 && W >= 2 && C > 0, "skimi_track_avgpool2: needs N, C > 0 and H, W >= 2");
    return avgpool2_launch(in, out, N, H, W, C, (hipStream_t)stream);
}

int skimi_track_sample_border(const float* fmap, int64_t img_stride, const float* coords, int64_t coord_stride, float* out,
                              int32_t B, int32_t N, int32_t H, int32_t W, int32_t C, void* stream) {
    SKIMI_CHECK_ARG(fmap && coords && out, "skimi_track_sample_border: null buffer");
    SKIMI_CHECK_ARG(B > 0 && N > 0 && H > 0 && W > 0 && C > 0, "skimi_track_sample_border: sizes must be positive");
    SKIMI_CHECK_ARG(img_stride >= (int64_t)H * W * C, "skimi_track_sample_border: img_stride is less than H * W * C");
    SKIMI_CHECK_ARG(coord_stride >= 2, "skimi_track_sample_border: coord_stride must be >= 2");
    return sample_border_launch(fmap, (long)img_stride, coords, (long)coord_stride, out, B, N, H, W, C, (hipStream_t)stream);
}

int skimi_track_corr_sample(const float* tgt, const float* fmap, const float* coords, float* out, int64_t rows, int32_t N,
                            int32_t S, int32_t H, int32_t W, int32_t C, int32_t r, int32_t level, int64_t ldo,
                            int32_t out_off, void* stream) {
    SKIMI_CHECK_ARG(tgt && fmap && coords && out, "skimi_track_corr_sample: null buffer");
    SKIMI_CHECK_ARG(rows > 0 && N > 0 && S > 0 && H > 0 && W > 0 && C > 0, "skimi_track_corr_sample: sizes must be positive");
    SKIMI_CHECK_ARG(rows % ((int64_t)N * S) == 0, "skimi_track_corr_sample: rows must be a multiple of N * S");
    SKIMI_CHECK_ARG(r >= 0 && r <= 64 && level >= 0 && level < 16, "skimi_track_corr_sample: needs 0 <= r <= 64, 0 <= level < 16");
    SKIMI_CHECK_ARG(out_off >= 0 && ldo >= (int64_t)out_off + (2 * r + 1) * (2 * r + 1),
                    "skimi_track_corr_sample: ldo is less than out_off + (2r+1)^2");
    return corr_sample_launch(tgt, fmap, coords, out, (long)rows, N, S, H, W, C, r, level, (long)ldo, out_off, (hipStream_t)stream);
}

int skimi_track_pos_embed_sample(const float* coords, int64_t coord_stride, float* out, int32_t BN, int32_t H, int32_t W,
                                 int32_t D, void* stream) {
    SKIMI_CHECK_ARG(coords && out, "skimi_track_pos_embed_sample: null buffer");
    SKIMI_CHECK_ARG(BN > 0 && H > 0 && W > 0 && D > 0, "skimi_track_pos_embed_sample: sizes must be positive");
    SKIMI_CHECK_ARG(D % 4 == 0, "skimi_track_pos_embed_sample: needs D %% 4 == 0 (got %d)", D);
    SKIMI_CHECK_ARG(coord_stride >= 2, "skimi_track_pos_embed_sample: coord_stride must be >= 2");
    return pos_embed_sample_launch(coords, (long)coord_stride, out, BN, H, W, D, (hipStream_t)stream);
}

int skimi_track_input(const float* coords, const float* fcorr, const float* tfeat, const float* pos, const float* qrt,
                      float* x, int64_t rows, int32_t S, int32_t L, int64_t ldx, float max_scale, void* stream) {
    SKIMI_CHECK_ARG(coords && fcorr && tfeat && pos && qrt && x, "skimi_track_input: null buffer");
    SKIMI_CHECK_ARG(rows > 0 && S > 0 && L > 0 && rows % S == 0, "skimi_track_input: needs rows, S, L > 0 and rows %% S == 0");
    SKIMI_CHECK_ARG(L % 4 == 0, "skimi_track_input: needs L %% 4 == 0 (got %d)", L);
    SKIMI_CHECK_ARG(ldx >= 3L * L + 4, "skimi_track_input: ldx is less than 3 L + 4");
    SKIMI_CHECK_ARG(max_scale > 0.f, "skimi_track_input: max_scale must be positive");
    return track_input_launch(coords, fcorr, tfeat, pos, qrt, x, (long)rows, S, L, (long)ldx, max_scale, (hipStream_t)stream);
}

int skimi_track_coord_update(float* coords, const float* delta, int64_t ldd, const float* query, float* pred, int64_t rows,
                             int32_t N, int32_t S, float stride, void* stream) {
    SKIMI_CHECK_ARG(coords && delta && query, "skimi_track_coord_update: null buffer");
    SKIMI_CHECK_ARG(rows > 0 && N > 0 && S > 0 && rows % ((int64_t)N * S) == 0,
                    "skimi_track_coord_update: needs rows, N, S > 0 and rows a multiple of N * S");
    SKIMI_CHECK_ARG(ldd >= 2, "skimi_track_coord_update: ldd must be >= 2");
    return track_coord_update_launch(coords, delta, (long)ldd, query, pred, (long)rows, N, S, stride, (hipStream_t)stream);
}

int skimi_track_init(const float* q, float* coords, float* qs, int64_t BN, int32_t S, float stride, void* stream) {
    SKIMI_CHECK_ARG(q && coords && qs, "skimi_track_init: null buffer");
    SKIMI_CHECK_ARG(BN > 0 && S > 0, "skimi_track_init: sizes must be positive");
    SKIMI_CHECK_ARG(stride > 0.f, "skimi_track_init: stride must be positive");
    return track_init_launch(q, coords, qs, (long)BN, S, stride, (hipStream_t)stream);
}

int skimi_track_repeat_rows(const float* src, float* dst, int64_t BN, int32_t S, int32_t C, void* stream) {
    SKIMI_CHECK_ARG(src && dst, "skimi_track_repeat_rows: null buffer");
    SKIMI_CHECK_ARG(BN > 0 && S > 0 && C > 0, "skimi_track_repeat_rows: sizes must be positive");
    return repeat_rows_launch(src, dst, (long)BN, S, C, (hipStream_t)stream);
}

int skimi_track_bns_to_bsn(const float* in, float* out, int32_t B, int32_t N, int32_t S, void* stream) {
    SKIMI_CHECK_ARG(in && out, "skimi_track_bns_to_bsn: null buffer");
    SKIMI_CHECK_ARG(B > 0 && N > 0 && S > 0, "skimi_track_bns_to_bsn: sizes must be positive");
    return bns_to_bsn_launch(in, out, B, N, S, (hipStream_t)stream);
}

}
```

skiing_analysis_pytorch_amd/csrc/conv_direct.hip:

```cpp
#include "common.h"
#include "gfx950.h"
#include "kernels.h"

namespace skimi {

__device__ uint4 g_conv_zero_page[4] = {{0, 0, 0, 0}, {0, 0, 0, 0}, {0, 0, 0, 0}, {0, 0, 0, 0}};

constexpr int CD_WIN = 18 * 18;
constexpr int CD_IN_PLANE = 21 * 1024;
constexpr int CD_W_PLANE = 9 * 32 * 64;
constexpr int CD_BUF = 2 * CD_IN_PLANE + 2 * CD_W_PLANE;

__global__ void conv_direct_pack_kernel(const float* __restrict__ w, unsigned short* __restrict__ out, int Cin) {
    const long n = 32L * Cin * 9;
    for (long i = (long)blockIdx.x * 256 + threadIdx.x; i < n; i += (long)gridDim.x * 256) {
        const int c32 = (int)(i % 32);
        const int co = (int)((i / 32) % 32);
        const int tap = (int)((i / 1024) % 9);
        const int cs = (int)(i / 9216);
        const float v = w[((long)co * Cin + cs * 32 + c32) * 9 + tap];
        const unsigned short hi = f2bf(v);
        const unsigned short lo = f2bf(v - bf2f(hi));
        const long base = (long)cs * 2 * 9216 + tap * 1024 + co * 32 + c32;
        out[base] = hi;
        out[base + 9216] = lo;
    }
}

int conv_direct_pack_launch(const float* w, unsigned short* out, int Cin, hipStream_t st) {
    SKIMI_CHECK_ARG(Cin % 32 == 0, "conv_direct: Cin %% 32 != 0");
    hipLaunchKernelGGL(conv_direct_pack_kernel, dim3(64), dim3(256), 0, st, w, out, Cin);
    SKIMI_LAUNCH_CHECK();
    return SKIMI_OK;
}

struct ConvDirectArgs {
    const unsigned short* in_hi;
    const unsigned short* in_lo;
    const unsigned short* w;
    const float* bias;
    float* out;
    int F, H, W, C, relu, tiles_x, tiles_y;
    long px_stride;
};

__global__ __launch_bounds__(512, 2) void conv_direct_n32_kernel(const ConvDirectArgs p) {
    extern __shared__ __attribute__((aligned(16))) char smem[];
    const int tid = threadIdx.x, lane = tid & 63;
    const int wave = __builtin_amdgcn_readfirstlane(tid >> 6);
    const int l31 = lane & 31, lh = lane >> 5;

    int bid = blockIdx.x;
    const int tx = bid % p.tiles_x;
    bid /= p.tiles_x;
    const int ty = bid % p.tiles_y;
    const int f = bid / p.tiles_y;
    const int y0 = ty * 16, x0 = tx * 16;
    const int nsl = p.C / 32;
    const unsigned short* zero = reinterpret_cast<const unsigned short*>(g_conv_zero_page);

    long in_off[3];
    int in_piece[3];
    int nin = 0;
#pragma unroll
    for (int j = 0; j < 3; ++j) {
        const int q = wave + 8 * j;
        in_piece[j] = q;
        in_off[j] = -1;
        if (q < 21) {
            nin = j + 1;
            const int px = 16 * q + (lane >> 2);
            const int hy = px / 18, hx = px - hy * 18;
            const int y = y0 - 1 + hy, x = x0 - 1 + hx;
            const int sc = (lane & 3) ^ (((hx + 2 * hy) >> 2) & 3);
            if (px < CD_WIN && y >= 0 && y < p.H && x >= 0 && x < p.W)
                in_off[j] = (((long)f * p.H + y) * p.W + x) * p.px_stride + sc * 8;
        }
    }
    int w_off[3], w_piece[3];
    int nw = 0;
#pragma unroll
    for (int j = 0; j < 3; ++j) {
        const int q = wave + 8 * j;
        w_piece[j] = q;
        w_off[j] = 0;
        if (q < 18) {
            nw = j + 1;
            const int row = 16 * q + (lane >> 2);
            const int sc = (lane & 3) ^ ((row >> 2) & 3);
            w_off[j] = row * 32 + sc * 8;
        }
    }
    auto stage = [&](int buf, int s) {
        char* base = smem + buf * CD_BUF;
#pragma unroll
        for (int j = 0; j < 3; ++j) {
            if (j < nin) {
                const bool ok = in_off[j] >= 0;
                const unsigned short* sh = ok ? p.in_hi + in_off[j] + s * 32 : zero;
                const unsigned short* sl = ok ? p.in_lo + in_off[j] + s * 32 : zero;
                char* dst = base + in_piece[j] * 1024;
                __builtin_amdgcn_global_load_lds((gbl_void*)sh, (lds_void*)dst, 16, 0, 0);
                __builtin_amdgcn_global_load_lds((gbl_void*)sl, (lds_void*)(dst + CD_IN_PLANE), 16, 0, 0);
            }
        }
        const unsigned short* ws = p.w + (long)s * 2 * 9216;
#pragma unroll
        for (int j = 0; j < 3; ++j) {
            if (j < nw) {
                char* dst = base + 2 * CD_IN_PLANE + w_piece[j] * 1024;
                __builtin_amdgcn_global_load_lds((gbl_void*)(ws + w_off[j]), (lds_void*)dst, 16, 0, 0);
                __builtin_amdgcn_global_load_lds((gbl_void*)(ws + 9216 + w_off[j]), (lds_void*)(dst + CD_W_PLANE), 16, 0, 0);
            }
        }
    };

    const int col = ((l31 & 15) + ((l31 >> 4) ? 14 : 0)) & 15;
    int a_off[9][2];
#pragma unroll
    for (int tap = 0; tap < 9; ++tap) {
        const int dy = tap / 3, dx = tap - dy * 3;
        const int hy = 2 * wave + (l31 >> 4) + dy, hx = col + dx;
        const int px = hy * 18 + hx;
#pragma unroll
        for (int ks = 0; ks < 2; ++ks) a_off[tap][ks] = px * 64 + (((2 * ks + lh) ^ (((hx + 2 * hy) >> 2) & 3)) << 4);
    }
    int b_off[2];
#pragma unroll
    for (int ks = 0; ks < 2; ++ks) b_off[ks] = l31 * 64 + (((2 * ks + lh) ^ ((l31 >> 2) & 3)) << 4);

    f32x16 acc;
#pragma unroll
    for (int r = 0; r < 16; ++r) acc[r] = 0.f;

    stage(0, 0);
    __syncthreads();
    for (int s = 0; s < nsl; ++s) {
        const int cur = s & 1;
        if (s + 1 < nsl) stage(cur ^ 1, s + 1);
        const char* ih = smem + cur * CD_BUF;
        const char* wh = ih + 2 * CD_IN_PLANE;
#pragma unroll
        for (int tap = 0; tap < 9; ++tap) {
#pragma unroll
            for (int ks = 0; ks < 2; ++ks) {
                const bf16x8 a_hi = *reinterpret_cast<const bf16x8*>(ih + a_off[tap][ks]);
                const bf16x8 a_lo = *reinterpret_cast<const bf16x8*>(ih + CD_IN_PLANE + a_off[tap][ks]);
                const bf16x8 w_hi = *reinterpret_cast<const bf16x8*>(wh + tap * 2048 + b_off[ks]);
                const bf16x8 w_lo = *reinterpret_cast<const bf16x8*>(wh + CD_W_PLANE + tap * 2048 + b_off[ks]);
                acc = __builtin_amdgcn_mfma_f32_32x32x16_bf16(a_lo, w_hi, acc, 0, 0, 0);
                acc = __builtin_amdgcn_mfma_f32_32x32x16_bf16(a_hi, w_lo, acc, 0, 0, 0);
                acc = __builtin_amdgcn_mfma_f32_32x32x16_bf16(a_hi, w_hi, acc, 0, 0, 0);
            }
        }
        __syncthreads();
    }

    const float bs = p.bias ? p.bias[l31] : 0.f;
    const bool interior = y0 + 16 <= p.H && x0 + 16 <= p.W;
    float* ob = p.out + ((long)f * p.H * p.W) * 32 + l31;
    if (interior) {
#pragma unroll
        for (int r = 0; r < 16; ++r) {
            const int pix = (r & 3) + 8 * (r >> 2) + 4 * lh;
            const int y = y0 + 2 * wave + (pix >> 4), x = x0 + (((pix & 15) + ((pix >> 4) ? 14 : 0)) & 15);
            float v = acc[r] + bs;
            if (p.relu) v = fmaxf(v, 0.f);
            ob[((long)y * p.W + x) * 32] = v;
        }
    } else {
#pragma unroll 1
        for (int r = 0; r < 16; ++r) {
            const int pix = (r & 3) + 8 * (r >> 2) + 4 * lh;
            const int y = y0 + 2 * wave + (pix >> 4), x = x0 + (((pix & 15) + ((pix >> 4) ? 14 : 0)) & 15);
            float v = acc[r] + bs;
            if (p.relu) v = fmaxf(v, 0.f);
            if (y < p.H && x < p.W) ob[((long)y * p.W + x) * 32] = v;
        }
    }
}

int conv_direct_n32_launch(const unsigned short* in_hi, const unsigned short* in_lo, const unsigned short* w_packed,
                           const float* bias, float* out, int F, int H, int W, int C, int relu, hipStream_t st,
                           long px_stride) {
    SKIMI_CHECK_ARG(in_hi && in_lo && w_packed && out, "conv_direct: null buffer");
    SKIMI_CHECK_ARG(C % 32 == 0 && C >= 32 && F > 0 && H > 0 && W > 0, "conv_direct: bad shape");
    SKIMI_CHECK_ARG((((uintptr_t)in_hi | (uintptr_t)in_lo | (uintptr_t)w_packed) & 15) == 0, "conv_direct: 16-B alignment");
    if (px_stride <= 0) px_stride = C;
    SKIMI_CHECK_ARG(px_stride >= C, "conv_direct: px_stride < C");
    SKIMI_CHECK_ARG(px_stride % 8 == 0, "conv_direct: px_stride %% 8 != 0 (16-B aligned pixels)");
    constexpr size_t lds = 2ull * CD_BUF;
    SKIMI_LDS_OPT_IN(conv_direct_n32_kernel, lds, "conv_direct");
    ConvDirectArgs a;
    a.in_hi = in_hi; a.in_lo = in_lo; a.w = w_packed; a.bias = bias; a.out = out;
    a.F = F; a.H = H; a.W = W; a.C = C; a.relu = relu;
    a.px_stride = px_stride;
    a.tiles_x = (int)cdiv(W, 16);
    a.tiles_y = (int)cdiv(H, 16);
    const long nblk = (long)F * a.tiles_x * a.tiles_y;
    SKIMI_CHECK_ARG(nblk < (1l << 31), "conv_direct: grid too large");
    hipLaunchKernelGGL(conv_direct_n32_kernel, dim3((unsigned)nblk), dim3(512), lds, st, a);
    SKIMI_LAUNCH_CHECK();
    return SKIMI_OK;
}

}
```

skiing_analysis_pytorch_amd/csrc/kernels.h:

```cpp
#pragma once
#include "common.h"

namespace skimi {

int gemm_dispatch(const skimi_gemm_desc* d, hipStream_t st, void* scratch, size_t scratch_bytes,
                  int force_splitk);

int layernorm_launch(const float* x, const float* x2, int64_t ldx, int64_t rows, int C,
                     const float* gamma, const float* beta, float eps, void* out, int out_dtype,
                     int64_t ldo, hipStream_t st, int64_t grp_rows = 0, int64_t grp_stride = 0,
                     int64_t grp_off = 0);
static inline bool layernorm_records_ok(int C) {
    return C % 256 == 0 && (C / 256 <= 4 || C / 256 == 6 || C / 256 == 8);
}

int qknorm_rope_launch(void* qkv, int dtype, int64_t tokens, int heads, const float* qn_w,
                       const float* qn_b, const float* kn_w, const float* kn_b, float eps,
                       const int32_t* pos, const float* rope_cos, const float* rope_sin, int rope_npos,
                       hipStream_t st, float q_scale = 1.f, int* q_scaled = nullptr);

struct AttnArgs {
    const void* q;
    const void* k;
    const void* v;
    void* out;
    long q_row, k_row, v_row, o_row;
    long q_batch, k_batch, v_batch, o_batch;
    long q_head, k_head, v_head, o_head;
    int batch, heads, seq_q, seq_k, head_dim;
    float scale;
    int batch_inner = 0;
    long q_batch2 = 0, k_batch2 = 0, v_batch2 = 0, o_batch2 = 0;
    int q_prescaled = 0;
    int out_f16 = 0;
    void* out_mx = nullptr;
    void* out_mx_scales = nullptr;
    long mx_row = 0, mx_srow = 0;
};

enum { ATTN_FAM_F32 = 1, ATTN_FAM_X3 = 2, ATTN_FAM_BF16_Q32 = 3, ATTN_FAM_BF16_Q64 = 4 };
enum { ATTN_OUT_ROWS = 0, ATTN_OUT_F16 = 1, ATTN_OUT_MX = 2, ATTN_OUT_RECORDS = 3 };
struct AttnRequest {
    const void* qkv;
    void* out;
    int dtype, out_dtype;
    int batch, seq, heads, head_dim;
    int q_prescaled;
    void* x3_scratch;
    size_t x3_scratch_bytes;
    bool want_records;
    void* out_scales;
};
struct AttnSwitches { int x3, mx, q64; long ldspad; int abl; };
struct AttnPlan {
    int family;
    int hd;
    int queries;
    long grid;
    int out_form;
    int q_prescaled;
    int lds_pad;
    int dbg;
    long c0, pw, koff, voff;
};
int check_attention(const AttnRequest& r);
AttnPlan plan_attention(const AttnRequest& r, const AttnSwitches& s);
AttnPlan plan_attention_f32(int batch, int heads, int seq_q, int head_dim);
AttnArgs attention_args(const AttnRequest& r, const AttnPlan& p);
int attention_launch(const AttnRequest& r, hipStream_t st, int* out_records = nullptr);
void attention_set_last_plan(const AttnPlan& plan);
const AttnPlan& attention_last_plan();
bool attention_mx_output_ok(int dtype, int heads, int head_dim);
int check_attention_shape(const AttnArgs& a);
int attention_f32_launch(const AttnArgs& a, const AttnPlan& p, hipStream_t st);
int attention_bf16_launch(const AttnArgs& a, const AttnPlan& p, hipStream_t st);
int attention_q64_dispatch(const AttnArgs& a, const AttnPlan& p, hipStream_t st);
size_t attention_x3_scratch_bytes(long tokens, long row_elems);
int attention_x3_launch(const AttnArgs& a, const AttnPlan& p, void* scratch, hipStream_t st);
int check_attention_f32(const AttnArgs& a);
int attention_f32_launch(const AttnArgs& a, hipStream_t st);
int resample_u8_launch(const unsigned char* in, unsigned char* out, long outer, int n_in, int n_out, long inner,
                       const int* kk, const int* bounds, int ksize, hipStream_t st);
int u8_hwc_to_f32_chw_launch(const unsigned char* in, int H, int W, float* out, int OH, int OW, int y_off, int x_off,
                             float fill, hipStream_t st);
int conv_direct_pack_launch(const float* w, unsigned short* out, int Cin, hipStream_t st);
int conv_direct_n32_launch(const unsigned short* in_hi, const unsigned short* in_lo, const unsigned short* w_packed,
                           const float* bias, float* out, int F, int H, int W, int C, int relu, hipStream_t st,
                           long px_stride = 0);

int vp3d_im2col_launch(const float* x, float* a0, int B, int L, int Cin, int k, int Kpad, hipStream_t st);

int quant_mx_launch(const void* x, int dtype, long ldx, long rows, int K, void* q, void* scales, hipStream_t st);
int gemm_fp8_launch(const void* A, const void* As, const void* W, const void* Ws, int M, int N, int K, const float* bias, int act,
                    const float* gamma, const float* resid, long ldr, void* out, int out_dtype, long ldo, hipStream_t st,
                    void* out_scales = nullptr);
bool gemm_fp8_mx_output_ok(int M, int N);
int layernorm_mx_launch(const float* x, int64_t ldx, int64_t rows, int C, const float* gamma, const float* beta, float eps,
                        void* payload, void* scales, hipStream_t st);

enum { VP3D_FAM_CONV = 1, VP3D_FAM_MM = 2, VP3D_FAM_WIN = 3, VP3D_FAM_EXPAND_MFMA = 4, VP3D_FAM_EXPAND_VALU = 5 };
struct Vp3dPlan {
    int family;
    int ct;
    int rt;
    int taps;
    int nw;
    int ms;
    int R;
    int grid;
    int lds;
};
struct Vp3dForce {
    int family;
    int ct;
    int nw;
    int ms;
};
int plan_vp3d_mm(int Npad, int B, int Lin, int C, int taps, int dil, const Vp3dForce* force, Vp3dPlan* plan);
int plan_vp3d_expand(int B, int Lin, int Cin, int taps, int C, int valu, int force_ms, Vp3dPlan* plan);
void vp3d_set_last_plan(const Vp3dPlan& plan);
const Vp3dPlan& vp3d_last_plan();
int vp3d_expand_launch(const float* x, const float* w, int ldw, const float* bias, float* out_f32, void* out_rec, int B, int Lin,
                       int Cin, int taps, int C, hipStream_t st, int force_ms = 0);
int vp3d_expand_mfma_launch(const float* x, const void* wfrag, int Kpad, const float* bias, float* out_f32, void* out_rec, int B,
                            int Lin, int Cin, int taps, int C, hipStream_t st, int force_ms = 0);
int vp3d_mm_launch(const void* wrec, int Npad, const void* xrec, const float* bias, const float* resid, int resid_L,
                   int resid_off, float* out_f32, int ldo, void* out_rec, int B, int Lin, int C, int taps, int dil, int N,
                   int relu, hipStream_t st, const Vp3dForce* force = nullptr);
bool vp3d_window_enabled();
int plan_vp3d_win(int Npad, int B, int Lin, int C, int taps, const Vp3dForce* force, Vp3dPlan* plan);
int vp3d_win_launch(const void* wrec, int Npad, const void* xrec, const float* bias, float* out_f32, int ldo, void* out_rec,
                    int B, int Lin, int C, int taps, int N, hipStream_t st, const Vp3dForce* force = nullptr);

}
```

skiing_analysis_pytorch_amd/csrc/vggt_dpt.hip:

```cpp
#include "env.h"
#include "gemm_epilogue.h"
#include "kernels.h"
#include "vggt_kernels.h"
#include "vggt_model.h"

namespace skimi {
namespace vggt {

const UvTab* find_uv(const ShapeTabs* h, int w, int hh, int C) {
    if (!h) return nullptr;
    for (const auto& t : h->uv)
        if (t.w == w && t.h == hh && t.C == C) return &t;
    return nullptr;
}

bool dpt_fused_ln(const DptW& w, int f2, int udt) {
    const bool off = !(int)env_once("SKIMI_TRACK_LN_FUSED", 1);
    return !off && w.feature_only && w.out_ln != nullptr && w.out_ln->g != nullptr && w.out_ln->b != nullptr && f2 == 128 && udt == SKIMI_F32;
}

static int uv_missing() {
    set_error("uv table missing");
    return SKIMI_ERR_STATE;
}

void* run_dpt(Ctx& c, const DptW& w, float* const* sf, float* const* sg, int F, int P, int nsp, int ph, int pw, int C,
              int H, int W, float* pts, float* conf, int act_mode) {
    const int prec = w.proj[0].prec;
    const int adt = Ctx::act_dt(prec);
    const size_t es = Ctx::esz(adt);
    const int D = 2 * C, np = ph * pw, feat = w.features;
    const size_t mk = c.ar.mark();
    int hh[4] = {ph * 4, ph * 2, ph, (ph - 1) / 2 + 1};
    int ww[4] = {pw * 4, pw * 2, pw, (pw - 1) / 2 + 1};
    void* rn[4];
    for (int i = 0; i < 4; ++i) rn[i] = c.ar.alloc((size_t)F * hh[i] * ww[i] * feat * es);
    char* const fake = (char*)(uintptr_t)0x10000000;
    auto rec_bytes = [&](int lvl) { return (size_t)F * hh[lvl] * ww[lvl] * feat * 4 + 256; };
    auto takes_records = [&](const Lin& L, const ConvW* cw, int lvl) {
        if (adt != SKIMI_F32 || feat % 32 != 0 || L.w_split == nullptr) return false;
        auto d = Ctx::as_records(c.desc(L, nullptr, adt, feat, F * hh[lvl] * ww[lvl], fake, adt, L.N), fake, rec_bytes(lvl) - 256);
        if (cw) c.conv_geom(d, *cw, F, hh[lvl], ww[lvl], hh[lvl], ww[lvl]);
        return gemm_x3dma_eligible(&d);
    };
    bool use_rec[4];
    char* rn_rec[4] = {nullptr, nullptr, nullptr, nullptr};
    for (int i = 0; i < 4; ++i) {
        use_rec[i] = takes_records(w.ref[i].r2c1.lin, &w.ref[i].r2c1, i);
        if (use_rec[i]) rn_rec[i] = (char*)c.ar.alloc(rec_bytes(i));
    }
    {
        const size_t mk2 = c.ar.mark();
        void* lnb = c.ar.alloc((size_t)F * np * D * es);
        void* lnb_rec = adt == SKIMI_F32 ? c.ar.alloc((size_t)F * np * D * 4 + 256) : nullptr;
        for (int i = 0; i < 4; ++i) {
            const size_t mk3 = c.ar.mark();
            void* t0 = c.ar.alloc((size_t)F * np * w.oc[i] * es);
            {
                auto d = c.desc(w.proj[i], lnb, adt, D, F * np, t0, adt, w.oc[i]);
                bool rec_in = false;
                if (adt == SKIMI_F32 && layernorm_records_ok(D) && w.proj[i].w_split != nullptr) {
                    const auto q = Ctx::as_records(d, lnb_rec, (size_t)F * np * D * 4);
                    if ((rec_in = gemm_x3dma_eligible(&q))) d = q;
                }
                c.ln(sf[i], sg[i], C, (long)F * np, D, w.norm, 1e-5f, rec_in ? lnb_rec : lnb, rec_in ? SKIMI_BF16X3_REC : adt, np, P, nsp);
                c.gemm(d);
            }
            if (i < 2 && adt == SKIMI_F32 && w.fold[i].w_split != nullptr) {
                const size_t t0_bytes = (size_t)F * np * w.oc[i] * 4;
                auto d = Ctx::as_records(c.desc(w.fold[i], nullptr, adt, w.oc[i], F * np, fake, adt, feat), fake, t0_bytes);
                d.a_mode = 3; d.store_mode = 2; d.ps_s = i == 0 ? 4 : 2; d.ps_C = feat;
                d.cN = F; d.cH = ph; d.cW = pw; d.cC = w.oc[i];
                d.act = SKIMI_ACT_RELU;
                if (gemm_x3dma_eligible(&d)) {
                    char* t0_rec = (char*)c.ar.alloc(t0_bytes + 256);
                    const UvTab* t = w.pos_embed ? find_uv(c.tabs, pw, ph, w.oc[i]) : nullptr;
                    if (w.pos_embed && !t) c.run(uv_missing);
                    c.run([&] {
                        return add_uv_pos_records_launch((const float*)t0, t ? t->tx : nullptr, t ? t->ty : nullptr, F, ph, pw, w.oc[i],
                                                         t0_rec, c.st);
                    });
                    d = Ctx::as_records(d, t0_rec, t0_bytes);
                    d.out = rn[i];
                    d.out_records = rn_rec[i];
                    c.gemm(d);
                    c.ar.release(mk3);
                    continue;
                }
            }
            if (w.pos_embed)
                c.run([&] {
                    const UvTab* t = find_uv(c.tabs, pw, ph, w.oc[i]);
                    return t ? add_uv_pos_launch(t0, adt, t->tx, t->ty, F, ph, pw, w.oc[i], c.st) : uv_missing();
                });
            void* t1 = t0;
            if (i == 0 || i == 1) {
                const int s = i == 0 ? 4 : 2;
                const Lin& L = i == 0 ? w.rs0 : w.rs1;
                t1 = c.ar.alloc((size_t)F * hh[i] * ww[i] * w.oc[i] * es);
                auto d = c.desc(L, t0, adt, w.oc[i], F * np, t1, adt, w.oc[i]);
                d.store_mode = 1; d.ps_s = s; d.ps_C = w.oc[i];
                d.cN = F; d.cH = ph; d.cW = pw;
                c.gemm(d);
            } else if (i == 3) {
                t1 = c.ar.alloc((size_t)F * hh[i] * ww[i] * w.oc[i] * es);
                auto d = c.desc(w.rs3.lin, t0, adt, w.oc[i], F * hh[i] * ww[i], t1, adt, w.oc[i]);
                c.conv_geom(d, w.rs3, F, ph, pw, hh[i], ww[i]);
                c.gemm(d);
            }
            {
                auto d = c.desc(w.rn[i].lin, t1, adt, w.oc[i], F * hh[i] * ww[i], rn[i], adt, feat);
                c.conv_geom(d, w.rn[i], F, hh[i], ww[i], hh[i], ww[i]);
                d.act = SKIMI_ACT_RELU;
                d.out_records = rn_rec[i];
                c.gemm(d);
            }
            c.ar.release(mk3);
        }
        c.ar.release(mk2);
    }
    void* prev = nullptr;
    char* prev_rec = nullptr;
    for (int r = 3; r >= 0; --r) {
        const FusionW& f = w.ref[r];
        const int h0 = hh[r], w0 = ww[r];
        const int M = F * h0 * w0;
        const size_t bytes = (size_t)M * feat * es;
        const bool recs = use_rec[r];
        auto conv_in = [&](const ConvW& cw, const void* in_f32, char* in_rec, void* out_f32, char* out_rec) {
            auto d = c.desc(cw.lin, in_f32, adt, feat, M, out_f32, adt, feat);
            c.conv_geom(d, cw, F, h0, w0, h0, w0);
            if (recs) d = Ctx::as_records(d, in_rec, rec_bytes(r) - 256);
            d.out_records = out_rec;
            return d;
        };
        void* cur;
        char* cur_rec = nullptr;
        void* tmp = recs ? nullptr : c.ar.alloc(bytes);
        char* tmp_rec = recs ? (char*)c.ar.alloc(rec_bytes(r)) : nullptr;
        if (f.has_r1) {
            cur = c.ar.alloc(bytes);
            if (recs) cur_rec = (char*)c.ar.alloc(rec_bytes(r));
            auto d1 = conv_in(f.r1c1, rn[r], rn_rec[r], tmp, tmp_rec);
            d1.act = SKIMI_ACT_RELU;
            c.gemm(d1);
            auto d2 = conv_in(f.r1c2, tmp, tmp_rec, cur, cur_rec);
            d2.resid = rn[r]; d2.ldr = feat; d2.resid_dtype = adt;
            d2.resid2 = prev; d2.ldr2 = feat;
            d2.post_act = SKIMI_ACT_RELU;
            c.gemm(d2);
        } else {
            cur = rn[r];
            cur_rec = rn_rec[r];
        }
        const bool u_recs = recs && takes_records(f.out_conv, nullptr, r);
        void* u = u_recs ? nullptr : c.ar.alloc(bytes);
        char* u_rec = u_recs ? (char*)c.ar.alloc(rec_bytes(r)) : nullptr;
        {
            auto d1 = conv_in(f.r2c1, cur, cur_rec, tmp, tmp_rec);
            d1.act = SKIMI_ACT_RELU;
            c.gemm(d1);
            auto d2 = conv_in(f.r2c2, tmp, tmp_rec, u, u_rec);
            d2.resid = cur; d2.ldr = feat; d2.resid_dtype = adt;
            c.gemm(d2);
        }
        const int h1 = r > 0 ? hh[r - 1] : 2 * h0, w1 = r > 0 ? ww[r - 1] : 2 * w0;
        void* olow = c.ar.alloc(bytes);
        {
            auto d = c.desc(f.out_conv, u, adt, feat, M, olow, adt, feat);
            if (u_recs) d = Ctx::as_records(d, u_rec, rec_bytes(r) - 256);
            c.gemm(d);
        }
        if (r == 0 && adt == SKIMI_F32 && w.oc1.lin.w_split != nullptr && feat % 32 == 0) {
            const size_t rec_bytes = (size_t)F * h1 * w1 * feat * 4;
            const size_t mk_rec = c.ar.mark();
            char* rec = (char*)c.ar.alloc(rec_bytes + 256);
            auto d = Ctx::as_records(c.desc(w.oc1.lin, nullptr, adt, feat, F * h1 * w1, rec, adt, w.feature_only ? feat : feat / 2), rec,
                                     rec_bytes);
            c.conv_geom(d, w.oc1, F, h1, w1, h1, w1);
            if (gemm_x3dma_eligible(&d)) {
                prev_rec = rec;
                c.run([&] {
                    return bilinear_ac_planes_launch((const float*)olow, (unsigned short*)rec, F, h0, w0, h1, w1, feat, c.st,
                                                     nullptr, nullptr, 1, rec + rec_bytes);
                });
                prev = nullptr;
                hh[r] = h1; ww[r] = w1;
                continue;
            }
            c.ar.release(mk_rec);
        }
        void* o = c.ar.alloc((size_t)F * h1 * w1 * feat * es);
        c.run([&] { return bilinear_ac_launch(olow, o, adt, F, h0, w0, h1, w1, feat, c.st); });
        prev = o;
        hh[r] = h1; ww[r] = w1;
    }
    const int h1 = hh[0], w1 = ww[0];
    const int f2 = w.feature_only ? feat : feat / 2;
    void* c1 = c.ar.alloc((size_t)F * h1 * w1 * f2 * es);
    if (prev_rec != nullptr) {
        auto d = Ctx::as_records(c.desc(w.oc1.lin, nullptr, adt, feat, F * h1 * w1, c1, adt, f2), prev_rec, (size_t)F * h1 * w1 * feat * 4);
        c.conv_geom(d, w.oc1, F, h1, w1, h1, w1);
        c.gemm(d);
    } else {
        auto d = c.desc(w.oc1.lin, prev, adt, feat, F * h1 * w1, c1, adt, f2);
        c.conv_geom(d, w.oc1, F, h1, w1, h1, w1);
        c.gemm(d);
    }
    const int Ho = ph * c.h->cfg.patch_size / w.down_ratio, Wo = pw * c.h->cfg.patch_size / w.down_ratio;
    const UvTab* uvt = w.pos_embed ? find_uv(c.tabs, Wo, Ho, f2) : nullptr;
    if (w.pos_embed && !uvt) c.run(uv_missing);
    const int no_direct = !(int)env_once("SKIMI_CONV_DIRECT", 1);
    const bool direct = !w.feature_only && w.oc2a_direct != nullptr && adt == SKIMI_F32 && !no_direct;
    void* c2 = nullptr;
    if (direct) {
        const size_t pe = (size_t)F * Ho * Wo * f2;
        unsigned short* rec = (unsigned short*)c.ar.alloc(pe * 4);
        c2 = c.ar.alloc((size_t)F * Ho * Wo * 32 * es);
        c.run([&] {
            return bilinear_ac_planes_launch((const float*)c1, rec, F, h1, w1, Ho, Wo, f2, c.st, uvt ? uvt->tx : nullptr,
                                             uvt ? uvt->ty : nullptr);
        });
        c.run([&] {
            return conv_direct_n32_launch(rec, rec + f2, w.oc2a_direct, w.oc2a.lin.b, (float*)c2, F, Ho, Wo, f2, 1, c.st,
                                          2L * f2);
        });
    } else {
        const int udt = (w.feature_only && w.out_f32) ? SKIMI_F32 : adt;
        void* c1u = c.ar.alloc((size_t)F * Ho * Wo * f2 * Ctx::esz(udt));
        c.run([&] {
            return dpt_fused_ln(w, f2, udt)
                       ? bilinear_ac_launch(c1, c1u, adt, F, h1, w1, Ho, Wo, f2, c.st, uvt ? uvt->tx : nullptr, uvt ? uvt->ty : nullptr, udt,
                                            w.out_ln->g, w.out_ln->b, 1e-5f)
                       : bilinear_ac_launch(c1, c1u, adt, F, h1, w1, Ho, Wo, f2, c.st, uvt ? uvt->tx : nullptr, uvt ? uvt->ty : nullptr, udt);
        });
        if (w.feature_only) return c1u;
        c2 = c.ar.alloc((size_t)F * Ho * Wo * 32 * es);
        auto d = c.desc(w.oc2a.lin, c1u, adt, f2, F * Ho * Wo, c2, adt, 32);
        c.conv_geom(d, w.oc2a, F, Ho, Wo, Ho, Wo);
        d.act = SKIMI_ACT_RELU;
        c.gemm(d);
    }
    c.run([&] { return dpt_out_launch(c2, adt, w.oc2b_w, w.oc2b_b, w.n_out, pts, conf, (long)F * Ho * Wo, act_mode, c.st); });
    c.ar.release(mk);
    (void)H; (void)W;
    return nullptr;
}

}
}
```

skiing_analysis_pytorch_amd/csrc/vggt_kernels.h:

```cpp
#pragma once
#include "common.h"

namespace skimi {

int patch_gather_launch(const float* img, void* out, int out_dtype, int F, int H, int W, int p, int Kp,
                        hipStream_t st);
int special_tokens_launch(float* x, const float* table, int F, int S, int P, int n, int C, hipStream_t st);
int bilinear_ac_planes_launch(const float* in, unsigned short* out, int N, int h, int w, int H, int W, int C, hipStream_t st,
                              const float* tabx = nullptr, const float* taby = nullptr,
                              int slice_records = 0, void* zpage = nullptr);
int bilinear_ac_launch(const void* in, void* out, int dtype, int N, int h, int w, int H, int W, int C,
                       hipStream_t st, const float* tabx = nullptr, const float* taby = nullptr, int out_dtype = -1,
                       const float* ln_g = nullptr, const float* ln_b = nullptr, float ln_eps = 0.f);
int add_uv_pos_launch(void* x, int dtype, const float* tabx, const float* taby, int N, int H, int W, int C,
                      hipStream_t st);
int add_uv_pos_records_launch(const float* x, const float* tabx, const float* taby, int N, int H, int W, int C, void* rec,
                              hipStream_t st);
int dpt_fold_pack_launch(const float* wT, const float* bT, const float* wrn, int Ci, int Cm, int Co, int s, float* tmp, void* rec,
                         float* beta, hipStream_t st);
int adaln_launch(const float* xn, const float* x, const float* mod, float* out, long rows, int D, hipStream_t st);
int pose_update_launch(const float* delta, float* pred_pad, float* act_out, long rows, int first, hipStream_t st);
int dpt_out_launch(const void* in, int dtype, const float* W, const float* b, int n_out, float* pts, float* conf,
                   long npix, int mode, hipStream_t st);
int f32_to_bf16_launch(const float* in, void* out, long n, hipStream_t st);
int f32_to_f16_launch(const float* in, void* out, long n, hipStream_t st);
int permute_conv_launch(const float* in, float* out, int Co, int Ci, int kh, int kw, hipStream_t st, int slice_major = 0);
int permute_convT_launch(const float* in, float* out, int Ci, int Co, int s, hipStream_t st);
int pad_cols_launch(const float* in, float* out, long rows, int K, int Kp, hipStream_t st);
int tile_vec_launch(const float* in, float* out, int n, int reps, hipStream_t st);

}
```

skiing_analysis_pytorch_amd/csrc/vggt_kernels.hip:

```cpp
#include <algorithm>

#include "common.h"
#include "gemm_epilogue.h"
#include "vggt_kernels.h"

namespace skimi {

static inline int grid_for(long n, int per_block = 256, int cap = 8192) {
    return (int)std::max<long>(1, std::min<long>(cdiv(n, per_block), cap));
}

template <typename T, bool F16 = false>
__global__ __launch_bounds__(256) void patch_gather_kernel(const float* __restrict__ img, T* __restrict__ out,
                                                           int F, int H, int W, int p, int Kp) {
    const int ph = H / p, pw = W / p, K = 3 * p * p;
    const long total = (long)F * ph * pw * Kp;
    const float mean[3] = {0.485f, 0.456f, 0.406f};
    const float stdv[3] = {0.229f, 0.224f, 0.225f};
    for (long i = (long)blockIdx.x * 256 + threadIdx.x; i < total; i += (long)gridDim.x * 256) {
        const int k = (int)(i % Kp);
        const long r = i / Kp;
        float v = 0.f;
        if (k < K) {
            const int px = (int)(r % pw);
            const int py = (int)((r / pw) % ph);
            const long f = r / ((long)pw * ph);
            const int c = k / (p * p);
            const int rem = k - c * p * p;
            const int dy = rem / p, dx = rem - dy * p;
            const float x = img[((f * 3 + c) * H + (py * p + dy)) * (long)W + (px * p + dx)];
            v = (x - mean[c]) / stdv[c];
        }
        if (sizeof(T) == 4) ((float*)out)[i] = v;
        else ((unsigned short*)out)[i] = F16 ? f2h(v) : f2bf(v);
    }
}

int patch_gather_launch(const float* img, void* out, int out_dtype, int F, int H, int W, int p, int Kp,
                        hipStream_t st) {
    const long total = (long)F * (H / p) * (W / p) * Kp;
    if (out_dtype == SKIMI_F32)
        hipLaunchKernelGGL(patch_gather_kernel<float>, dim3(grid_for(total)), dim3(256), 0, st, img, (float*)out, F, H, W, p, Kp);
    else if (out_dtype == SKIMI_F16)
        hipLaunchKernelGGL((patch_gather_kernel<unsigned short, true>), dim3(grid_for(total)), dim3(256), 0, st, img,
                           (unsigned short*)out, F, H, W, p, Kp);
    else
        hipLaunchKernelGGL(patch_gather_kernel<unsigned short>, dim3(grid_for(total)), dim3(256), 0, st, img,
                           (unsigned short*)out, F, H, W, p, Kp);
    SKIMI_LAUNCH_CHECK();
    return SKIMI_OK;
}

__global__ __launch_bounds__(256) void special_tokens_kernel(float* __restrict__ x, const float* __restrict__ table,
                                                             int F, int S, int P, int n, int C) {
    const long total = (long)F * n * C;
    for (long i = (long)blockIdx.x * 256 + threadIdx.x; i < total; i += (long)gridDim.x * 256) {
        const int c = (int)(i % C);
        const int t = (int)((i / C) % n);
        const long f = i / ((long)C * n);
        const int sel = (f % S == 0) ? 0 : 1;
        x[(f * P + t) * C + c] = table[((long)sel * n + t) * C + c];
    }
}

int special_tokens_launch(float* x, const float* table, int F, int S, int P, int n, int C, hipStream_t st) {
    hipLaunchKernelGGL(special_tokens_kernel, dim3(grid_for((long)F * n * C)), dim3(256), 0, st, x, table, F, S, P, n, C);
    SKIMI_LAUNCH_CHECK();
    return SKIMI_OK;
}

template <typename T, typename TO = T, bool LN = false>
__global__ __launch_bounds__(256) void bilinear_ac_kernel(const T* __restrict__ in, TO* __restrict__ out, int N,
                                                          int h, int w, int H, int W, int C,
                                                          const float* __restrict__ tabx,
                                                          const float* __restrict__ taby, bool f16 = false,
                                                          const float* __restrict__ ln_g = nullptr,
                                                          const float* __restrict__ ln_b = nullptr, float ln_eps = 0.f) {
    const int C4 = C / 4;
    const int rowlen = W * C4;
    const float sy = H > 1 ? (float)(h - 1) / (float)(H - 1) : 0.f;
    const float sx = W > 1 ? (float)(w - 1) / (float)(W - 1) : 0.f;
    const int Y = (int)(blockIdx.y % (unsigned)H);
    const long n = blockIdx.y / (unsigned)H;
    for (int i = blockIdx.x * 256 + threadIdx.x; i < rowlen; i += gridDim.x * 256) {
        const int X = i / C4;
        const int c4 = i - X * C4;
        const float fy = sy * Y, fx = sx * X;
        const int y0 = min((int)fy, h - 1), x0 = min((int)fx, w - 1);
        const int y1 = min(y0 + 1, h - 1), x1 = min(x0 + 1, w - 1);
        const float ly1 = fminf(fmaxf(fy - y0, 0.f), 1.f), lx1 = fminf(fmaxf(fx - x0, 0.f), 1.f);
        const float ly0 = 1.f - ly1, lx0 = 1.f - lx1;
        const T* base = in + n * (long)h * w * C + c4 * 4;
        float p00[4], p01[4], p10[4], p11[4];
        auto ld = [&](const T* p, float* d) {
            if (sizeof(T) == 4) {
                const float4 v = *reinterpret_cast<const float4*>(p);
                d[0] = v.x; d[1] = v.y; d[2] = v.z; d[3] = v.w;
            } else {
                const bf16x4 v = *reinterpret_cast<const bf16x4*>(p);
#pragma unroll
                for (int k = 0; k < 4; ++k) d[k] = x16tof((unsigned short)v[k], f16);
            }
        };
        ld(base + ((long)y0 * w + x0) * C, p00);
        ld(base + ((long)y0 * w + x1) * C, p01);
        ld(base + ((long)y1 * w + x0) * C, p10);
        ld(base + ((long)y1 * w + x1) * C, p11);
        float r[4];
#pragma unroll
        for (int k = 0; k < 4; ++k)
            r[k] = ly0 * (lx0 * p00[k] + lx1 * p01[k]) + ly1 * (lx0 * p10[k] + lx1 * p11[k]);
        if (tabx != nullptr) {
            const int half = C / 2, c = c4 * 4;
            const float4 e = *reinterpret_cast<const float4*>(c < half ? tabx + (long)X * half + c
                                                                        : taby + (long)Y * half + (c - half));
            r[0] += e.x; r[1] += e.y; r[2] += e.z; r[3] += e.w;
        }
        if constexpr (LN) {
            float s = (r[0] + r[1]) + (r[2] + r[3]);
#pragma unroll
            for (int o_ = 16; o_ > 0; o_ >>= 1) s += __shfl_xor(s, o_, 32);
            const float mean = s * (1.0f / 128.0f);
            float q = 0.f;
#pragma unroll
            for (int k = 0; k < 4; ++k) {
                r[k] -= mean;
                q += r[k] * r[k];
            }
#pragma unroll
            for (int o_ = 16; o_ > 0; o_ >>= 1) q += __shfl_xor(q, o_, 32);
            const float rstd = rsqrtf(q * (1.0f / 128.0f) + ln_eps);
            const float4 g4 = *reinterpret_cast<const float4*>(ln_g + c4 * 4), b4 = *reinterpret_cast<const float4*>(ln_b + c4 * 4);
            r[0] = r[0] * rstd * g4.x + b4.x;
            r[1] = r[1] * rstd * g4.y + b4.y;
            r[2] = r[2] * rstd * g4.z + b4.z;
            r[3] = r[3] * rstd * g4.w + b4.w;
        }
        TO* o = out + ((n * H + Y) * (long)W + X) * C + c4 * 4;
        if (sizeof(TO) == 4) {
            *reinterpret_cast<float4*>(o) = make_float4(r[0], r[1], r[2], r[3]);
        } else {
            bf16x4 v;
#pragma unroll
            for (int k = 0; k < 4; ++k) v[k] = (short)f2x16(r[k], f16);
            *reinterpret_cast<bf16x4*>(o) = v;
        }
    }
}

__global__ __launch_bounds__(256) void bilinear_ac_planes_kernel(const float* __restrict__ in,
                                                                 unsigned short* __restrict__ out, int N, int h, int w,
                                                                 int H, int W, int C, const float* __restrict__ tabx,
                                                                 const float* __restrict__ taby, int slice_records,
                                                                 uint4* __restrict__ zpage) {
    if (zpage != nullptr && blockIdx.x == 0 && blockIdx.y == 0 && threadIdx.x < 16) zpage[threadIdx.x] = uint4{0, 0, 0, 0};
    const int C8 = C / 8;
    const int rowlen = W * C8;
    const float sy = H > 1 ? (float)(h - 1) / (float)(H - 1) : 0.f;
    const float sx = W > 1 ? (float)(w - 1) / (float)(W - 1) : 0.f;
    const int Y = (int)(blockIdx.y % (unsigned)H);
    const long n = blockIdx.y / (unsigned)H;
    for (int i = blockIdx.x * 256 + threadIdx.x; i < rowlen; i += gridDim.x * 256) {
        const int X = i / C8;
        const int c8 = i - X * C8;
        const float fy = sy * Y, fx = sx * X;
        const int y0 = min((int)fy, h - 1), x0 = min((int)fx, w - 1);
        const int y1 = min(y0 + 1, h - 1), x1 = min(x0 + 1, w - 1);
        const float ly1 = fminf(fmaxf(fy - y0, 0.f), 1.f), lx1 = fminf(fmaxf(fx - x0, 0.f), 1.f);
        const float ly0 = 1.f - ly1, lx0 = 1.f - lx1;
        const float* base = in + n * (long)h * w * C + c8 * 8;
        float p00[8], p01[8], p10[8], p11[8];
        auto ld8 = [&](const float* q, float* d) {
            const float4 a = *reinterpret_cast<const float4*>(q), b = *reinterpret_cast<const float4*>(q + 4);
            d[0] = a.x; d[1] = a.y; d[2] = a.z; d[3] = a.w; d[4] = b.x; d[5] = b.y; d[6] = b.z; d[7] = b.w;
        };
        ld8(base + ((long)y0 * w + x0) * C, p00);
        ld8(base + ((long)y0 * w + x1) * C, p01);
        ld8(base + ((long)y1 * w + x0) * C, p10);
        ld8(base + ((long)y1 * w + x1) * C, p11);
        float r[8];
#pragma unroll
        for (int k = 0; k < 8; ++k)
            r[k] = ly0 * (lx0 * p00[k] + lx1 * p01[k]) + ly1 * (lx0 * p10[k] + lx1 * p11[k]);
        if (tabx != nullptr) {
            const int half = C / 2, c = c8 * 8;
            float e[8];
            ld8(c < half ? tabx + (long)X * half + c : taby + (long)Y * half + (c - half), e);
#pragma unroll
            for (int k = 0; k < 8; ++k) r[k] += e[k];
        }
        bf16x8 hi, lo;
#pragma unroll
        for (int k = 0; k < 8; ++k) {
            const unsigned short hb = f2bf(r[k]);
            hi[k] = (short)hb;
            lo[k] = (short)f2bf(r[k] - bf2f(hb));
        }
        const long pix = ((n * H + Y) * (long)W + X) * 2 * C;
        if (slice_records) {
            const int c = c8 * 8;
            const long o = pix + (c >> 5) * 64 + (c & 31);
            __builtin_nontemporal_store(hi, reinterpret_cast<bf16x8*>(out + o));
            __builtin_nontemporal_store(lo, reinterpret_cast<bf16x8*>(out + o + 32));
        } else {
            const long o = pix + c8 * 8;
            __builtin_nontemporal_store(hi, reinterpret_cast<bf16x8*>(out + o));
            __builtin_nontemporal_store(lo, reinterpret_cast<bf16x8*>(out + o + C));
        }
    }
}

int bilinear_ac_planes_launch(const float* in, unsigned short* out, int N, int h, int w, int H, int W, int C, hipStream_t st,
                              const float* tabx, const float* taby, int slice_records, void* zpage) {
    SKIMI_CHECK_ARG(C % 16 == 0, "bilinear resize into planes needs C %% 16 == 0");
    SKIMI_CHECK_ARG(!slice_records || C % 32 == 0, "bilinear resize into records needs C %% 32 == 0");
    SKIMI_CHECK_ARG(tabx == nullptr || taby != nullptr, "fused uv pos embed needs both tables");
    SKIMI_CHECK_ARG((long)N * H < 65536, "bilinear resize into planes: N * H must be < 65536");
    const int rowlen = W * (C / 8);
    hipLaunchKernelGGL(bilinear_ac_planes_kernel, dim3((unsigned)cdiv(rowlen, 256), (unsigned)(N * H)), dim3(256), 0, st, in, out, N,
                       h, w, H, W, C, tabx, taby, slice_records, (uint4*)zpage);
    SKIMI_LAUNCH_CHECK();
    return SKIMI_OK;
}

int bilinear_ac_launch(const void* in, void* out, int dtype, int N, int h, int w, int H, int W, int C,
                       hipStream_t st, const float* tabx, const float* taby, int out_dtype, const float* ln_g, const float* ln_b,
                       float ln_eps) {
    if (out_dtype < 0) out_dtype = dtype;
    if (ln_g != nullptr) {
        SKIMI_CHECK_ARG(ln_b != nullptr && C == 128 && out_dtype == SKIMI_F32 && (((uintptr_t)ln_g | (uintptr_t)ln_b) & 15) == 0,
                        "bilinear resize + LayerNorm: C == 128, fp32 output, 16-byte aligned gamma / beta");
        SKIMI_CHECK_ARG(tabx == nullptr || taby != nullptr, "fused uv pos embed needs both tables");
        SKIMI_CHECK_ARG((long)N * H < 65536, "bilinear resize: N * H must be < 65536");
        const dim3 grid((unsigned)cdiv((long)W * (C / 4), 256), (unsigned)(N * H));
        if (dtype == SKIMI_F32)
            hipLaunchKernelGGL((bilinear_ac_kernel<float, float, true>), grid, dim3(256), 0, st, (const float*)in, (float*)out, N, h, w,
                               H, W, C, tabx, taby, false, ln_g, ln_b, ln_eps);
        else
            hipLaunchKernelGGL((bilinear_ac_kernel<unsigned short, float, true>), grid, dim3(256), 0, st, (const unsigned short*)in,
                               (float*)out, N, h, w, H, W, C, tabx, taby, dtype == SKIMI_F16, ln_g, ln_b, ln_eps);
        SKIMI_LAUNCH_CHECK();
        return SKIMI_OK;
    }
    SKIMI_CHECK_ARG(out_dtype == dtype || (dtype != SKIMI_F32 && out_dtype == SKIMI_F32),
                    "bilinear resize: the output type is the input's, or fp32 from a 16-bit map");
    SKIMI_CHECK_ARG(C % 4 == 0, "bilinear resize needs C %% 4 == 0");
    SKIMI_CHECK_ARG(tabx == nullptr || (taby != nullptr && C % 8 == 0), "fused uv pos embed needs both tables, C %% 8 == 0");
    SKIMI_CHECK_ARG((long)N * H < 65536, "bilinear resize: N * H must be < 65536");
    const dim3 grid((unsigned)cdiv((long)W * (C / 4), 256), (unsigned)(N * H));
    if (dtype == SKIMI_F32)
        hipLaunchKernelGGL(bilinear_ac_kernel<float>, grid, dim3(256), 0, st, (const float*)in, (float*)out, N, h, w, H, W, C,
                           tabx, taby);
    else if (out_dtype == SKIMI_F32)
        hipLaunchKernelGGL((bilinear_ac_kernel<unsigned short, float>), grid, dim3(256), 0, st, (const unsigned short*)in,
                           (float*)out, N, h, w, H, W, C, tabx, taby, dtype == SKIMI_F16);
    else
        hipLaunchKernelGGL(bilinear_ac_kernel<unsigned short>, grid, dim3(256), 0, st, (const unsigned short*)in,
                           (unsigned short*)out, N, h, w, H, W, C, tabx, taby, dtype == SKIMI_F16);
    SKIMI_LAUNCH_CHECK();
    return SKIMI_OK;
}

template <typename T>
__global__ __launch_bounds__(256) void add_uv_pos_kernel(T* __restrict__ x, const float* __restrict__ tabx,
                                                         const float* __restrict__ taby, int N, int H, int W, int C, bool f16 = false) {
    const int C4 = C / 4, half = C / 2;
    const long total = (long)N * H * W * C4;
    for (long i = (long)blockIdx.x * 256 + threadIdx.x; i < total; i += (long)gridDim.x * 256) {
        const int c = (int)(i % C4) * 4;
        const int X = (int)((i / C4) % W);
        const int Y = (int)((i / ((long)C4 * W)) % H);
        const float* t = c < half ? tabx + (long)X * half + c : taby + (long)Y * half + (c - half);
        const float4 e = *reinterpret_cast<const float4*>(t);
        T* p = x + i * 4;
        if (sizeof(T) == 4) {
            float4 v = *reinterpret_cast<float4*>(p);
            v.x += e.x; v.y += e.y; v.z += e.z; v.w += e.w;
            *reinterpret_cast<float4*>(p) = v;
        } else {
            bf16x4 v = *reinterpret_cast<bf16x4*>(p);
            v[0] = (short)f2x16(x16tof((unsigned short)v[0], f16) + e.x, f16);
            v[1] = (short)f2x16(x16tof((unsigned short)v[1], f16) + e.y, f16);
            v[2] = (short)f2x16(x16tof((unsigned short)v[2], f16) + e.z, f16);
            v[3] = (short)f2x16(x16tof((unsigned short)v[3], f16) + e.w, f16);
            *reinterpret_cast<bf16x4*>(p) = v;
        }
    }
}

int add_uv_pos_launch(void* x, int dtype, const float* tabx, const float* taby, int N, int H, int W, int C,
                      hipStream_t st) {
    SKIMI_CHECK_ARG(C % 8 == 0, "uv pos embed needs C %% 8 == 0");
    const long total = (long)N * H * W * (C / 4);
    if (dtype == SKIMI_F32)
        hipLaunchKernelGGL(add_uv_pos_kernel<float>, dim3(grid_for(total, 256, 65536)), dim3(256), 0, st, (float*)x, tabx, taby, N, H, W, C);
    else
        hipLaunchKernelGGL(add_uv_pos_kernel<unsigned short>, dim3(grid_for(total, 256, 65536)), dim3(256), 0, st,
                           (unsigned short*)x, tabx, taby, N, H, W, C, dtype == SKIMI_F16);
    SKIMI_LAUNCH_CHECK();
    return SKIMI_OK;
}

__global__ __launch_bounds__(256) void adaln_kernel(const float* __restrict__ xn, const float* __restrict__ x,
                                                    const float* __restrict__ mod, float* __restrict__ out, long rows,
                                                    int D) {
    const long total = rows * D;
    for (long i = (long)blockIdx.x * 256 + threadIdx.x; i < total; i += (long)gridDim.x * 256) {
        const long r = i / D;
        const int c = (int)(i - r * D);
        const float shift = mod[r * 3 * D + c], scale = mod[r * 3 * D + D + c], gate = mod[r * 3 * D + 2 * D + c];
        out[i] = gate * (xn[i] * (1.f + scale) + shift) + x[i];
    }
}

int adaln_launch(const float* xn, const float* x, const float* mod, float* out, long rows, int D, hipStream_t st) {
    hipLaunchKernelGGL(adaln_kernel, dim3(grid_for(rows * D)), dim3(256), 0, st, xn, x, mod, out, rows, D);
    SKIMI_LAUNCH_CHECK();
    return SKIMI_OK;
}

__global__ void pose_update_kernel(const float* __restrict__ delta, float* __restrict__ pred_pad,
                                   float* __restrict__ act_out, long rows, int first) {
    const long i = (long)blockIdx.x * blockDim.x + threadIdx.x;
    if (i >= rows * 9) return;
    const long r = i / 9;
    const int c = (int)(i - r * 9);
    const float p = first ? delta[i] : pred_pad[r * 16 + c] + delta[i];
    pred_pad[r * 16 + c] = p;
    act_out[i] = c >= 7 ? fmaxf(p, 0.f) : p;
}

int pose_update_launch(const float* delta, float* pred_pad, float* act_out, long rows, int first, hipStream_t st) {
    hipLaunchKernelGGL(pose_update_kernel, dim3((unsigned)cdiv(rows * 9, 128)), dim3(128), 0, st, delta, pred_pad, act_out, rows, first);
    SKIMI_LAUNCH_CHECK();
    return SKIMI_OK;
}

template <typename T, int NOUT>
__global__ __launch_bounds__(256) void dpt_out_kernel(const T* __restrict__ in, const float* __restrict__ Wt,
                                                      const float* __restrict__ b, float* __restrict__ pts,
                                                      float* __restrict__ conf, long npix, int mode, bool f16 = false) {
    __shared__ float ws[NOUT * 32 + NOUT];
    for (int i = threadIdx.x; i < NOUT * 32 + NOUT; i += 256) ws[i] = i < NOUT * 32 ? Wt[i] : b[i - NOUT * 32];
    __syncthreads();
    for (long px = (long)blockIdx.x * 256 + threadIdx.x; px < npix; px += (long)gridDim.x * 256) {
        float v[32];
        if (sizeof(T) == 4) {
#pragma unroll
            for (int k = 0; k < 8; ++k) {
                const float4 t = *reinterpret_cast<const float4*>((const float*)in + px * 32 + 4 * k);
                v[4 * k] = t.x; v[4 * k + 1] = t.y; v[4 * k + 2] = t.z; v[4 * k + 3] = t.w;
            }
        } else {
#pragma unroll
            for (int k = 0; k < 4; ++k) {
                const bf16x8 t = *reinterpret_cast<const bf16x8*>((const unsigned short*)in + px * 32 + 8 * k);
#pragma unroll
                for (int j = 0; j < 8; ++j) v[8 * k + j] = x16tof((unsigned short)t[j], f16);
            }
        }
        float o[NOUT];
#pragma unroll
        for (int n = 0; n < NOUT; ++n) {
            float s = 0.f;
#pragma unroll
            for (int k = 0; k < 32; ++k) s += v[k] * ws[n * 32 + k];
            o[n] = s + ws[NOUT * 32 + n];
        }
#pragma unroll
        for (int n = 0; n < NOUT - 1; ++n) {
            float y = o[n];
            if (mode == 0) y = expf(y);
            else y = copysignf(expm1f(fabsf(y)), y) * (y != 0.f ? 1.f : 0.f);
            pts[px * (NOUT - 1) + n] = y;
        }
        conf[px] = 1.f + expf(o[NOUT - 1]);
    }
}

int dpt_out_launch(const void* in, int dtype, const float* W, const float* b, int n_out, float* pts, float* conf,
                   long npix, int mode, hipStream_t st) {
    SKIMI_CHECK_ARG(n_out == 2 || n_out == 4, "dpt output stage supports 2 or 4 channels (got %d)", n_out);
    dim3 g(grid_for(npix, 256, 16384)), blk(256);
#define GO(T, N) hipLaunchKernelGGL((dpt_out_kernel<T, N>), g, blk, 0, st, (const T*)in, W, b, pts, conf, npix, mode, dtype == SKIMI_F16)
    if (dtype == SKIMI_F32) { if (n_out == 2) GO(float, 2); else GO(float, 4); }
    else { if (n_out == 2) GO(unsigned short, 2); else GO(unsigned short, 4); }
#undef GO
    SKIMI_LAUNCH_CHECK();
    return SKIMI_OK;
}

__global__ void f32_to_bf16_kernel(const float* __restrict__ in, unsigned short* __restrict__ out, long n) {
    for (long i = (long)blockIdx.x * 256 + threadIdx.x; i < n; i += (long)gridDim.x * 256) out[i] = f2bf(in[i]);
}
int f32_to_bf16_launch(const float* in, void* out, long n, hipStream_t st) {
    hipLaunchKernelGGL(f32_to_bf16_kernel, dim3(grid_for(n)), dim3(256), 0, st, in, (unsigned short*)out, n);
    SKIMI_LAUNCH_CHECK();
    return SKIMI_OK;
}
__global__ void f32_to_f16_kernel(const float* __restrict__ in, unsigned short* __restrict__ out, long n) {
    for (long i = (long)blockIdx.x * 256 + threadIdx.x; i < n; i += (long)gridDim.x * 256) out[i] = f2h(in[i]);
}
int f32_to_f16_launch(const float* in, void* out, long n, hipStream_t st) {
    hipLaunchKernelGGL(f32_to_f16_kernel, dim3(grid_for(n)), dim3(256), 0, st, in, (unsigned short*)out, n);
    SKIMI_LAUNCH_CHECK();
    return SKIMI_OK;
}

__global__ void permute_conv_kernel(const float* __restrict__ in, float* __restrict__ out, int Co, int Ci, int kh, int kw,
                                    int slice_major) {
    const long n = (long)Co * Ci * kh * kw;
    for (long i = (long)blockIdx.x * 256 + threadIdx.x; i < n; i += (long)gridDim.x * 256) {
        int ci, x, y;
        long co;
        if (slice_major) {
            const int c32 = (int)(i % 32);
            x = (int)((i / 32) % kw);
            y = (int)((i / (32L * kw)) % kh);
            const int cs = (int)((i / (32L * kw * kh)) % (Ci / 32));
            co = i / ((long)Ci * kw * kh);
            ci = cs * 32 + c32;
        } else {
            ci = (int)(i % Ci);
            x = (int)((i / Ci) % kw);
            y = (int)((i / ((long)Ci * kw)) % kh);
            co = i / ((long)Ci * kw * kh);
        }
        out[i] = in[((co * Ci + ci) * kh + y) * kw + x];
    }
}
int permute_conv_launch(const float* in, float* out, int Co, int Ci, int kh, int kw, hipStream_t st, int slice_major) {
    SKIMI_CHECK_ARG(!slice_major || Ci % 32 == 0, "slice-major conv weights need Cin %% 32 == 0");
    hipLaunchKernelGGL(permute_conv_kernel, dim3(grid_for((long)Co * Ci * kh * kw)), dim3(256), 0, st, in, out, Co, Ci, kh, kw,
                       slice_major);
    SKIMI_LAUNCH_CHECK();
    return SKIMI_OK;
}

__global__ void permute_convT_kernel(const float* __restrict__ in, float* __restrict__ out, int Ci, int Co, int s) {
    const long n = (long)Ci * Co * s * s;
    for (long i = (long)blockIdx.x * 256 + threadIdx.x; i < n; i += (long)gridDim.x * 256) {
        const int ci = (int)(i % Ci);
        const long r = i / Ci;
        const int co = (int)(r % Co);
        const int ab = (int)(r / Co);
        const int a = ab / s, b = ab - a * s;
        out[i] = in[(((long)ci * Co + co) * s + a) * s + b];
    }
}
int permute_convT_launch(const float* in, float* out, int Ci, int Co, int s, hipStream_t st) {
    hipLaunchKernelGGL(permute_convT_kernel, dim3(grid_for((long)Ci * Co * s * s)), dim3(256), 0, st, in, out, Ci, Co, s);
    SKIMI_LAUNCH_CHECK();
    return SKIMI_OK;
}

__global__ __launch_bounds__(256) void dpt_fold_phase_kernel(const float* __restrict__ wT, const float* __restrict__ wrn, int Ci,
                                                             int Cm, int Co, int s, int p, int q, float* __restrict__ out) {
    const int KH = (p == 0 || p == s - 1) ? 2 : 1, KW = (q == 0 || q == s - 1) ? 2 : 1;
    const int oy = p == 0 ? -1 : 0, ox = q == 0 ? -1 : 0;
    const long K = (long)KH * KW * Ci, total = (long)Co * K;
    for (long i = (long)blockIdx.x * 256 + threadIdx.x; i < total; i += (long)gridDim.x * 256) {
        const int co = (int)(i / K);
        const int k = (int)(i - co * K);
        const int u = k >> 5, tap = u % (KH * KW);
        const int ci = (u / (KH * KW)) * 32 + (k & 31);
        const int ky = tap / KW, kx = tap - ky * KW;
        double acc = 0.0;
        for (int a = 0; a < 3; ++a) {
            const int ty = p + a - 1, fy = ty < 0 ? -1 : ty >= s ? 1 : 0;
            if (fy != oy + ky) continue;
            for (int b = 0; b < 3; ++b) {
                const int tx = q + b - 1, fx = tx < 0 ? -1 : tx >= s ? 1 : 0;
                if (fx != ox + kx) continue;
                const float* r = wrn + (long)co * Cm * 9 + a * 3 + b;
                const float* t = wT + (long)ci * Cm * s * s + (ty - fy * s) * s + (tx - fx * s);
                for (int cm = 0; cm < Cm; ++cm) acc += (double)r[(long)cm * 9] * (double)t[(long)cm * s * s];
            }
        }
        out[i] = (float)acc;
    }
}
__global__ __launch_bounds__(256) void dpt_fold_bias_kernel(const float* __restrict__ bT, const float* __restrict__ wrn, int Cm, int Co,
                                                            float* __restrict__ beta) {
    const int i = blockIdx.x * 256 + threadIdx.x;
    if (i >= 9 * Co) return;
    const int cls = i / Co, co = i - cls * Co, yc = cls / 3, xc = cls - yc * 3;
    double acc = 0.0;
    if (bT != nullptr)
        for (int a = 0; a < 3; ++a) {
            if ((yc == 1 && a == 0) || (yc == 2 && a == 2)) continue;
            for (int b = 0; b < 3; ++b) {
                if ((xc == 1 && b == 0) || (xc == 2 && b == 2)) continue;
                for (int cm = 0; cm < Cm; ++cm) acc += (double)wrn[((long)co * Cm + cm) * 9 + a * 3 + b] * (double)bT[cm];
            }
        }
    beta[i] = (float)acc;
}
int dpt_fold_pack_launch(const float* wT, const float* bT, const float* wrn, int Ci, int Cm, int Co, int s, float* tmp, void* rec,
                         float* beta, hipStream_t st) {
    SKIMI_CHECK_ARG(s >= 2 && Ci % 32 == 0 && Ci > 0 && Cm > 0 && Co > 0, "dpt_fold_pack: needs s >= 2 and Ci %% 32 == 0");
    long off = 0;
    for (int p = 0; p < s; ++p)
        for (int q = 0; q < s; ++q) {
            const int taps = ((p == 0 || p == s - 1) ? 2 : 1) * ((q == 0 || q == s - 1) ? 2 : 1);
            const long n = (long)Co * taps * Ci;
            hipLaunchKernelGGL(dpt_fold_phase_kernel, dim3(grid_for(n)), dim3(256), 0, st, wT, wrn, Ci, Cm, Co, s, p, q, tmp + off);
            SKIMI_LAUNCH_CHECK();
            const int rc = split_records_launch(tmp + off, (long)taps * Ci, Co, taps * Ci, (char*)rec + off * 4, st);
            if (rc) return rc;
            off += n;
        }
    hipLaunchKernelGGL(dpt_fold_bias_kernel, dim3((unsigned)cdiv(9L * Co, 256)), dim3(256), 0, st, bT, wrn, Cm, Co, beta);
    SKIMI_LAUNCH_CHECK();
    return SKIMI_OK;
}

__global__ __launch_bounds__(256) void add_uv_pos_records_kernel(const float* __restrict__ x, const float* __restrict__ tabx,
                                                                 const float* __restrict__ taby, int N, int H, int W, int C,
                                                                 unsigned short* __restrict__ rec) {
    const int C4 = C / 4, half = C / 2;
    const long total = (long)N * H * W * C4;
    if (blockIdx.x == 0 && threadIdx.x < 16) reinterpret_cast<uint4*>(rec + total * 8)[threadIdx.x] = uint4{0, 0, 0, 0};
    for (long i = (long)blockIdx.x * 256 + threadIdx.x; i < total; i += (long)gridDim.x * 256) {
        const int c = (int)(i % C4) * 4;
        float4 v = *reinterpret_cast<const float4*>(x + i * 4);
        if (tabx != nullptr) {
            const int X = (int)((i / C4) % W);
            const int Y = (int)((i / ((long)C4 * W)) % H);
            const float4 e = *reinterpret_cast<const float4*>(c < half ? tabx + (long)X * half + c : taby + (long)Y * half + (c - half));
            v.x += e.x; v.y += e.y; v.z += e.z; v.w += e.w;
        }
        const float f[4] = {v.x, v.y, v.z, v.w};
        bf16x4 h, l;
#pragma unroll
        for (int k = 0; k < 4; ++k) {
            const unsigned short hb = f2bf(f[k]);
            h[k] = (short)hb;
            l[k] = (short)f2bf(f[k] - bf2f(hb));
        }
        unsigned short* o = rec + (i / C4) * (2L * C) + (c >> 5) * 64 + (c & 31);
        *reinterpret_cast<bf16x4*>(o) = h;
        *reinterpret_cast<bf16x4*>(o + 32) = l;
    }
}
int add_uv_pos_records_launch(const float* x, const float* tabx, const float* taby, int N, int H, int W, int C, void* rec,
                              hipStream_t st) {
    SKIMI_CHECK_ARG(C % 32 == 0, "uv pos embed to records needs C %% 32 == 0");
    const long total = (long)N * H * W * (C / 4);
    hipLaunchKernelGGL(add_uv_pos_records_kernel, dim3(grid_for(total, 256, 65536)), dim3(256), 0, st, x, tabx, taby, N, H, W, C,
                       (unsigned short*)rec);
    SKIMI_LAUNCH_CHECK();
    return SKIMI_OK;
}

__global__ void pad_cols_kernel(const float* __restrict__ in, float* __restrict__ out, long rows, int K, int Kp) {
    const long n = rows * Kp;
    for (long i = (long)blockIdx.x * 256 + threadIdx.x; i < n; i += (long)gridDim.x * 256) {
        const int k = (int)(i % Kp);
        out[i] = k < K ? in[(i / Kp) * K + k] : 0.f;
    }
}
int pad_cols_launch(const float* in, float* out, long rows, int K, int Kp, hipStream_t st) {
    hipLaunchKernelGGL(pad_cols_kernel, dim3(grid_for(rows * Kp)), dim3(256), 0, st, in, out, rows, K, Kp);
    SKIMI_LAUNCH_CHECK();
    return SKIMI_OK;
}
__global__ void tile_vec_kernel(const float* __restrict__ in, float* __restrict__ out, int n, int reps) {
    const int i = blockIdx.x * 256 + threadIdx.x;
    if (i < n * reps) out[i] = in[i % n];
}
int tile_vec_launch(const float* in, float* out, int n, int reps, hipStream_t st) {
    hipLaunchKernelGGL(tile_vec_kernel, dim3((unsigned)cdiv((long)n * reps, 256)), dim3(256), 0, st, in, out, n, reps);
    SKIMI_LAUNCH_CHECK();
    return SKIMI_OK;
}

}
```

skiing_analysis_pytorch_amd/ops.py:

```python
from __future__ import annotations

import ctypes as C
from typing import NamedTuple, Optional

import torch

from . import _lib
from ._lib import ACT_NONE, BF16, F16, F32, PREC_BF16, PREC_BF16X3, GemmDesc, check, lib, ptr


def _dt(t: torch.Tensor) -> int:
    if t.dtype == torch.float32:
        return F32
    if t.dtype == torch.bfloat16:
        return BF16
    if t.dtype == torch.float16:
        return F16
    raise TypeError(f"unsupported dtype {t.dtype}")


def _require_cuda(*ts):
    for t in ts:
        if t is not None and not t.is_cuda:
            raise _lib.SkimiError("libskimi ops need device (HBM) tensors; got a CPU tensor")


def gemm(a, w, *, prec=PREC_BF16X3, bias=None, gamma=None, resid=None, act=ACT_NONE, out=None,
         out_dtype=torch.float32, conv=None, resid_map=None, pixel_shuffle=None, splitk_scratch=None,
         force_splitk=0, M=None, lda=None, w_split=None, x3_scratch=None, a_records=None, out_records=None,
         records_only=False, post_act=ACT_NONE, resid2=None, out2=None, out_map=None, splitk_zeroed=False):
    _require_cuda(w, bias, gamma, resid, out, resid2, out2)
    if out_map is not None and out is None:
        raise _lib.SkimiError("gemm: out_map needs a caller-owned out (the remapped rows cannot be sized here)")
    if resid is not None and resid2 is not None and resid.dtype != resid2.dtype:
        raise _lib.SkimiError("gemm: resid and resid2 share one dtype (resid_dtype)")
    d = GemmDesc()
    N, K = w.shape
    d.N, d.K = N, K
    d.W, d.w_dtype = ptr(w), _dt(w)
    if a_records is not None:
        _require_cuda(a_records)
        d.A, d.a_dtype = ptr(a_records), _lib.BF16X3_REC
        d.lda = lda if lda is not None else (conv["C"] if conv is not None else K)
    else:
        _require_cuda(a)
        d.A, d.a_dtype = ptr(a), _dt(a)
        d.lda = lda if lda is not None else a.stride(-2) if a.dim() >= 2 else a.shape[-1]
    dev = w.device
    d.ldw = w.stride(0)
    d.prec = prec
    if conv is not None:
        d.a_mode = 2 if conv.get("slice_major") else 1
        d.cN, d.cH, d.cW, d.cC = conv["N"], conv["H"], conv["W"], conv["C"]
        d.KH, d.KW, d.stride, d.pad, d.dil = conv["KH"], conv["KW"], conv["stride"], conv["pad"], conv["dil"]
        d.OH, d.OW = conv["OH"], conv["OW"]
        d.M = M if M is not None else d.cN * d.OH * d.OW
    else:
        d.M = M if M is not None else a.shape[0]
    if records_only:
        assert out is None and out_records is not None and pixel_shuffle is None
        d.out_dtype = _lib.F32
    elif pixel_shuffle is not None:
        s, cout, n_img, h, w_ = pixel_shuffle
        d.store_mode, d.ps_s, d.ps_C = 1, s, cout
        d.cN, d.cH, d.cW = n_img, h, w_
        if out is None:
            out = torch.empty((n_img, h * s, w_ * s, cout), dtype=out_dtype, device=dev)
        d.ldo = out.stride(-2)
    else:
        if out is None:
            out = torch.empty((d.M, N), dtype=out_dtype, device=dev)
        d.ldo = out.stride(-2)
    if not records_only:
        d.out, d.out_dtype = ptr(out), _dt(out)
    if out2 is not None:
        if out is None or (out2.dtype == torch.float32) == (out.dtype == torch.float32) or \
                (out.dtype == torch.float32 and out2.dtype != torch.bfloat16):
            raise _lib.SkimiError("gemm: out2 is the other dtype of out (bf16 next to fp32, fp32 next to 16-bit)")
        d.out2, d.ldo2 = ptr(out2), out2.stride(-2)
    if out_map is not None:
        d.out_rows_per_batch, d.out_batch_stride, d.out_row_off = out_map
    d.bias, d.gamma, d.resid = ptr(bias), ptr(gamma), ptr(resid)
    if resid is not None:
        d.ldr = resid.stride(-2)
        d.resid_dtype = _dt(resid)
    if resid2 is not None:
        d.resid2, d.ldr2 = ptr(resid2), resid2.stride(-2)
        d.resid_dtype = _dt(resid2)
    if resid_map is not None:
        d.resid_rows_per_batch, d.resid_batch_stride, d.resid_row_off = resid_map
    d.act = act
    d.post_act = post_act
    if splitk_scratch is not None:
        d.splitk_scratch = ptr(splitk_scratch)
        d.splitk_scratch_bytes = splitk_scratch.numel() * splitk_scratch.element_size()
    d.force_splitk = force_splitk
    d.splitk_scratch_zeroed = int(splitk_zeroed)
    if w_split is not None:
        d.W_split = ptr(w_split)
        if a_records is not None:
            d.x3_scratch = ptr(a_records) + a_records.numel() * 2 - 256
            d.x3_scratch_bytes = 256
        else:
            d.x3_scratch = ptr(x3_scratch)
            d.x3_scratch_bytes = x3_scratch.numel() * x3_scratch.element_size()
    if out_records is not None:
        _require_cuda(out_records)
        d.out_records = ptr(out_records)
    check(lib().skimi_gemm(C.byref(d), _lib.current_stream()), "skimi_gemm")
    return out


class GemmPath(NamedTuple):
    family: Optional[str]
    tile: Optional[str]
    loop: Optional[str]
    mfma: Optional[int]
    epi: int
    splitk: int
    raw: int


_PATH_FAMILY = {1: "generic", 2: "splitk_ordered", 3: "splitk_atomic", 4: "x3dma_wide", 5: "x3dma_narrow",
                6: "gemm256", 7: "conv_win"}
_PATH_TILE = {1: "64x64", 2: "128x64", 3: "128x128"}
_PATH_LOOP = {1: "two_phase_256", 2: "two_phase_192", 3: "ping_pong", 4: "single_stream"}


def gemm_last_path() -> GemmPath:
    v = int(lib().skimi_gemm_last_path())
    fam = _PATH_FAMILY.get(v & 15)
    sub = (v >> 4) & 15
    generic = fam in ("generic", "splitk_ordered", "splitk_atomic")
    return GemmPath(family=fam, tile=_PATH_TILE.get(sub) if generic else None,
                    loop=_PATH_LOOP.get(sub) if fam == "gemm256" else None,
                    mfma={1: 16, 2: 32}.get((v >> 8) & 15), epi=(v >> 12) & 15, splitk=(v >> 16) & 255, raw=v)


def layernorm(x, gamma=None, beta=None, eps=1e-5, *, x2=None, out_dtype=torch.float32, out=None, rows=None, ldo=None,
              grp_rows=0, grp_stride=0, grp_off=0):
    _require_cuda(x, x2, gamma, beta, out)
    Cc = x.shape[-1] * (2 if x2 is not None else 1)
    if out is None and rows is None and ldo is None and not grp_rows and not isinstance(out_dtype, str):
        rows = x.numel() // x.shape[-1]
        out = torch.empty((*x.shape[:-1], Cc), dtype=out_dtype, device=x.device)
        check(lib().skimi_layernorm(ptr(x), ptr(x2), x.stride(-2), rows, Cc, ptr(gamma), ptr(beta), eps, ptr(out),
                                    _dt(out), Cc, _lib.current_stream()), "skimi_layernorm")
        return out
    if x.dim() != 2 or x.stride(-1) != 1 or (x2 is not None and (x2.shape != x.shape or x2.stride() != x.stride())):
        raise _lib.SkimiError("layernorm: the strided form takes x [in_rows, C] with unit column stride, x2 laid out like x")
    in_rows = x.shape[0]
    if rows is None:
        rows = in_rows // grp_stride * grp_rows if grp_rows else in_rows
    records = isinstance(out_dtype, str)
    if records:
        assert out_dtype == "records", out_dtype
        if out is None:
            out = records_buffer(rows, Cc, x.device)
        if out.numel() * out.element_size() < rows * Cc * 4 + 256:
            raise _lib.SkimiError("layernorm: `out` is too small for the records and their zero page")
        odt, ldo = _lib.BF16X3_REC, Cc
    else:
        if out is None:
            out = torch.empty((rows, ldo or Cc), dtype=out_dtype, device=x.device)
        odt = _dt(out)
        if out.dim() != 2 or out.stride(1) != 1 or out.shape[0] < rows or out.shape[1] < Cc:
            raise _lib.SkimiError("layernorm: `out` is [>= rows, >= C] with unit column stride")
        if ldo is None:
            ldo = out.stride(0)
        elif ldo != out.stride(0):
            raise _lib.SkimiError("layernorm: ldo is the row stride of `out`")
    check(lib().skimi_layernorm_ex(ptr(x), ptr(x2), x.stride(0), in_rows, rows, Cc, ptr(gamma), ptr(beta), eps, ptr(out), odt,
                                   ldo, grp_rows, grp_stride, grp_off, _lib.current_stream()), "skimi_layernorm_ex")
    return out


def qknorm_rope_(qkv, heads, qn_w=None, qn_b=None, kn_w=None, kn_b=None, eps=1e-5, pos=None, rope_cos=None,
                 rope_sin=None, *, q_scale=None):
    _require_cuda(qkv, pos, rope_cos, rope_sin)
    tokens = qkv.numel() // (3 * heads * 64)
    npos = rope_cos.shape[0] if rope_cos is not None else 0
    if q_scale is not None:
        flag = C.c_int32(0)
        check(lib().skimi_qknorm_rope_scaled(ptr(qkv), _dt(qkv), tokens, heads, ptr(qn_w), ptr(qn_b), ptr(kn_w), ptr(kn_b),
                                             eps, ptr(pos), ptr(rope_cos), ptr(rope_sin), npos, q_scale, C.byref(flag),
                                             _lib.current_stream()), "skimi_qknorm_rope_scaled")
        return qkv, bool(flag.value)
    check(lib().skimi_qknorm_rope(ptr(qkv), _dt(qkv), tokens, heads, ptr(qn_w), ptr(qn_b), ptr(kn_w), ptr(kn_b),
                                  eps, ptr(pos), ptr(rope_cos), ptr(rope_sin), npos, _lib.current_stream()),
          "skimi_qknorm_rope")
    return qkv


def attention_x3_scratch_bytes(tokens, row_elems):
    return int(lib().skimi_attention_x3_scratch_bytes(tokens, row_elems))


class AttnPlan(NamedTuple):
    family: int
    queries: int
    out_form: int
    q_prescaled: int
    grid: int
    hd: int
    lds: int
    reserved: int


def attention_last_plan() -> AttnPlan:
    out = (C.c_int32 * 8)()
    lib().skimi_attention_last_plan(out)
    return AttnPlan(*out)


def attention(qkv, batch, seq, heads, head_dim, out_dtype=None, *, q_prescaled=0, x3_scratch=None, out_records=False,
              out=None):
    _require_cuda(qkv)
    if q_prescaled or x3_scratch is not None or out_records or out is not None:
        return _attention_ex(qkv, batch, seq, heads, head_dim, out_dtype, q_prescaled, x3_scratch, out_records, out)
    if isinstance(out_dtype, str):
        assert out_dtype == "fp8mx", out_dtype
        rows, Kp = batch * seq, (heads * head_dim + 127) // 128 * 128
        buf = torch.zeros(rows * (Kp + Kp // 32), dtype=torch.uint8, device=qkv.device)
        check(lib().skimi_attention_out(ptr(qkv), ptr(buf), _dt(qkv), _lib.FP8MX, batch, seq, heads, head_dim,
                                        _lib.current_stream()), "skimi_attention_out")
        return buf[:rows * Kp].view(rows, Kp), buf[rows * Kp:].view(rows, Kp // 32)
    out = torch.empty((batch * seq, heads * head_dim), dtype=out_dtype or qkv.dtype, device=qkv.device)
    if out_dtype is None or out_dtype == qkv.dtype:
        check(lib().skimi_attention(ptr(qkv), ptr(out), _dt(qkv), batch, seq, heads, head_dim, _lib.current_stream()),
              "skimi_attention")
    else:
        check(lib().skimi_attention_out(ptr(qkv), ptr(out), _dt(qkv), _dt(out), batch, seq, heads, head_dim,
                                        _lib.current_stream()), "skimi_attention_out")
    return out


def attention_f32_strided(q, k, v, out, *, q_strides, k_strides, v_strides, o_strides, batch, heads, seq_q, seq_k, head_dim,
                          scale=None, batch_inner=0):
    _require_cuda(q, k, v, out)
    no, ni = (batch // batch_inner, batch_inner) if batch_inner > 0 else (1, batch)
    for name, t, s, seq in (("q", q, q_strides, seq_q), ("k", k, k_strides, seq_k), ("v", v, v_strides, seq_k),
                            ("out", out, o_strides, seq_q)):
        if t.dtype != torch.float32:
            raise _lib.SkimiError(f"attention_f32_strided: {name} must be fp32")
        if len(s) != 4 or min(s) < 0:
            raise _lib.SkimiError(f"attention_f32_strided: {name}_strides = (token, head, batch, outer batch), not negative")
        room = t.untyped_storage().nbytes() // 4 - t.storage_offset()
        last = (seq - 1) * s[0] + (heads - 1) * s[1] + (ni - 1) * s[2] + (no - 1) * s[3] + head_dim
        if min(batch, heads, seq, head_dim) > 0 and last > room:
            raise _lib.SkimiError(f"attention_f32_strided: the {name} stream ends {last - room} elements past its buffer")
    arr = [(C.c_int64 * 4)(*map(int, s)) for s in (q_strides, k_strides, v_strides, o_strides)]
    sc = float(scale) if scale is not None else (1.0 / head_dim ** 0.5 if head_dim > 0 else 0.0)
    check(lib().skimi_attention_f32_strided(ptr(q), ptr(k), ptr(v), ptr(out), *arr, batch, batch_inner, heads, seq_q, seq_k,
                                            head_dim, sc, _lib.current_stream()), "skimi_attention_f32_strided")
    return out


def _attention_ex(qkv, batch, seq, heads, head_dim, out_dtype, q_prescaled, x3_scratch, out_records, out):
    _require_cuda(x3_scratch, out)
    rows, Cc = batch * seq, heads * head_dim
    flag = C.c_int32(1 if out_records else 0)
    sc_bytes = x3_scratch.numel() * x3_scratch.element_size() if x3_scratch is not None else 0
    mx = isinstance(out_dtype, str)
    if mx:
        assert out_dtype == "fp8mx", out_dtype
        odt, Kp = _lib.FP8MX, (Cc + 127) // 128 * 128
        need = rows * (Kp + Kp // 32)
        if out is None:
            out = torch.zeros(need, dtype=torch.uint8, device=qkv.device)
    else:
        odt = {torch.float32: F32, torch.bfloat16: BF16, torch.float16: F16}[out_dtype or qkv.dtype]
        need = rows * Cc * (4 if odt == F32 else 2) + (256 if out_records else 0)
        if out is None:
            out = records_buffer(rows, Cc, qkv.device) if out_records else \
                torch.empty((rows, Cc), dtype=out_dtype or qkv.dtype, device=qkv.device)
    assert out.numel() * out.element_size() >= need, "attention: `out` is too small"
    check(lib().skimi_attention_ex(ptr(qkv), ptr(out), _dt(qkv), odt, batch, seq, heads, head_dim, int(q_prescaled),
                                   ptr(x3_scratch), sc_bytes, C.byref(flag), _lib.current_stream()), "skimi_attention_ex")
    if mx:
        buf = out.view(torch.uint8).reshape(-1)
        return buf[:rows * Kp].view(rows, Kp), buf[rows * Kp:need].view(rows, Kp // 32)
    return (out, bool(flag.value)) if out_records else out


def conv3x3_n32_pack(w):
    _require_cuda(w)
    Cc = w.shape[1]
    assert w.shape == (32, Cc, 3, 3) and w.dtype == torch.float32
    packed = torch.empty(((Cc + 31) // 32, 2, 9, 32, 32), dtype=torch.bfloat16, device=w.device)
    check(lib().skimi_conv3x3_n32_pack(ptr(w.contiguous()), ptr(packed), Cc, _lib.current_stream()), "skimi_conv3x3_n32_pack")
    return packed


def conv3x3_n32(x, w, bias=None, relu=False, *, planes=None, px_stride=None, packed=None, out=None):
    _require_cuda(bias, packed, out)
    F_, H, W_, Cc = x if planes is not None else x.shape
    st = _lib.current_stream()
    if planes is None:
        _require_cuda(x)
        planes = split_planes(x.reshape(-1, Cc).contiguous())
        dev = x.device
    else:
        _require_cuda(*planes)
        dev = next((t.device for t in planes if t is not None), "cuda")
    if packed is None:
        assert w.shape == (32, Cc, 3, 3) and Cc % 32 == 0
        packed = conv3x3_n32_pack(w)
    if out is None:
        out = torch.empty((F_, H, W_, 32), dtype=torch.float32, device=dev)
    if px_stride is None:
        check(lib().skimi_conv3x3_n32(ptr(planes[0]), ptr(planes[1]), ptr(packed), ptr(bias), ptr(out), F_, H, W_, Cc,
                                      1 if relu else 0, st), "skimi_conv3x3_n32")
    else:
        check(lib().skimi_conv3x3_n32_strided(ptr(planes[0]), ptr(planes[1]), ptr(packed), ptr(bias), ptr(out), F_, H, W_,
                                              Cc, 1 if relu else 0, int(px_stride), st), "skimi_conv3x3_n32_strided")
    return out


def split_records(x):
    _require_cuda(x)
    rows, Cc = x.shape
    out = torch.empty((rows, (Cc + 31) // 32, 2, 32), dtype=torch.bfloat16, device=x.device)
    check(lib().skimi_split_records(ptr(x), x.stride(0), rows, Cc, ptr(out), _lib.current_stream()), "skimi_split_records")
    return out


def records_buffer(rows, Cc, device="cuda"):
    return torch.empty(rows * ((Cc + 31) // 32) * 64 + 128, dtype=torch.bfloat16, device=device)


def x3_scratch_numel(rows, Cc):
    return rows * ((Cc + 31) // 32 * 32) + 64


def dpt_fold_pack(w_T, b_T, w_rn):
    _require_cuda(w_T, b_T, w_rn)
    Ci, Cm, s, s2 = w_T.shape
    Co = w_rn.shape[0]
    assert s == s2 and w_rn.shape == (Co, Cm, 3, 3)
    rec = torch.empty((s + 2) * (s + 2) * Co * Ci * 2, dtype=torch.bfloat16, device=w_T.device)
    beta = torch.empty((9, Co), dtype=torch.float32, device=w_T.device)
    check(lib().skimi_dpt_fold_pack(ptr(w_T.contiguous()), ptr(b_T.contiguous()) if b_T is not None else None, ptr(w_rn.contiguous()),
                                    Ci, Cm, Co, s, ptr(rec), ptr(beta), _lib.current_stream()), "skimi_dpt_fold_pack")
    return rec, beta


def convT_conv3x3_folded(x, w_records, beta, s, Co, *, act=ACT_NONE, out=None, out_records=None, records_only=False,
                         a_records=None):
    _require_cuda(w_records, beta, out, out_records, a_records)
    F_, h, w_, Ci = x if a_records is not None else x.shape
    nrec = F_ * h * w_ * Ci * 2
    ar = a_records
    if ar is None:
        _require_cuda(x)
        ar = records_buffer(F_ * h * w_, Ci, device=x.device)
        ar[:nrec] = split_records(x.reshape(-1, Ci).contiguous()).reshape(-1)
        ar[nrec:] = 0
    d = GemmDesc()
    d.M, d.N, d.K = F_ * h * w_, Co, 4 * Ci
    d.A, d.a_dtype, d.lda = ptr(ar), _lib.BF16X3_REC, Ci
    d.W, d.w_dtype, d.ldw = ptr(w_records), _lib.F32, 4 * Ci
    d.W_split = ptr(w_records)
    d.x3_scratch, d.x3_scratch_bytes = ptr(ar) + nrec * 2, 256
    d.prec = PREC_BF16X3
    d.a_mode, d.store_mode, d.ps_s, d.ps_C = 3, 2, s, Co
    d.cN, d.cH, d.cW, d.cC = F_, h, w_, Ci
    d.bias, d.act = ptr(beta), act
    d.out_dtype = _lib.F32
    if not records_only:
        if out is None:
            out = torch.empty((F_, h * s, w_ * s, Co), dtype=torch.float32, device=w_records.device)
        d.out = ptr(out)
    d.ldo = Co
    if out_records is not None:
        d.out_records = ptr(out_records)
    check(lib().skimi_gemm(C.byref(d), _lib.current_stream()), "skimi_gemm")
    return out


def split_planes(x):
    _require_cuda(x)
    rows, Cc = x.shape
    out = torch.empty((2, rows, Cc), dtype=torch.bfloat16, device=x.device)
    check(lib().skimi_split_planes(ptr(x), x.stride(0), rows, Cc, ptr(out[0]), ptr(out[1]), _lib.current_stream()),
          "skimi_split_planes")
    return out


def quant_mx(x: torch.Tensor):
    _require_cuda(x)
    x = x.contiguous()
    rows, K = x.shape
    Kp = (K + 127) // 128 * 128
    q = torch.empty((rows, Kp), dtype=torch.uint8, device=x.device)
    s = torch.empty((rows, Kp // 32), dtype=torch.uint8, device=x.device)
    check(lib().skimi_quant_mx(ptr(x), _dt(x), x.stride(0), rows, K, ptr(q), ptr(s), _lib.current_stream()), "skimi_quant_mx")
    return q, s


def layernorm_mx(x, gamma, beta, eps=1e-5):
    _require_cuda(x, gamma, beta)
    rows, Cc = x.shape
    q = torch.empty((rows, Cc), dtype=torch.uint8, device=x.device)
    s = torch.empty((rows, Cc // 32), dtype=torch.uint8, device=x.device)
    check(lib().skimi_layernorm_mx(ptr(x), x.stride(0), rows, Cc, ptr(gamma), ptr(beta), eps, ptr(q), ptr(s),
                                   _lib.current_stream()), "skimi_layernorm_mx")
    return q, s


def gemm_fp8(a_q, a_s, w_q, w_s, K, *, bias=None, act=ACT_NONE, gamma=None, resid=None, out=None, out_dtype=torch.float32,
             out_mx=False):
    _require_cuda(a_q, a_s, w_q, w_s, bias, gamma, resid, out)
    M, N = a_q.shape[0], w_q.shape[0]
    Kp = (K + 127) // 128 * 128
    for t, cols, what in ((a_q, Kp, "a_q"), (w_q, Kp, "w_q"), (a_s, Kp // 32, "a_s"), (w_s, Kp // 32, "w_s")):
        if t.dtype != torch.uint8 or t.dim() != 2 or t.shape[1] != cols or not t.is_contiguous():
            raise _lib.SkimiError(f"gemm_fp8: {what} must be a contiguous uint8 [rows, {cols}] array for K = {K} "
                                  f"(got {tuple(t.shape)} {t.dtype}); operands come from quant_mx")
    if a_s.shape[0] != M or w_s.shape[0] != N:
        raise _lib.SkimiError("gemm_fp8: scale rows do not match the payload rows")
    if out_mx:
        q = torch.empty((M, N), dtype=torch.uint8, device=a_q.device)
        sc = torch.empty((M, N // 32), dtype=torch.uint8, device=a_q.device)
        check(lib().skimi_gemm_fp8(ptr(a_q), ptr(a_s), ptr(w_q), ptr(w_s), M, N, K, ptr(bias), act, None, None, 0, ptr(q),
                                   _lib.FP8MX, N, ptr(sc), _lib.current_stream()), "skimi_gemm_fp8")
        return q, sc
    if out is None:
        out = torch.empty((M, N), dtype=out_dtype, device=a_q.device)
    check(lib().skimi_gemm_fp8(ptr(a_q), ptr(a_s), ptr(w_q), ptr(w_s), M, N, K, ptr(bias), act, ptr(gamma), ptr(resid),
                               resid.stride(0) if resid is not None else 0, ptr(out), _dt(out), out.stride(0), None,
                               _lib.current_stream()), "skimi_gemm_fp8")
    return out


def _stream():
    return _lib.current_stream()


def resize_bilinear(x, H, W, *, out=None, out_dtype=None, tabx=None, taby=None, ln_g=None, ln_b=None, ln_eps=0.0):
    _require_cuda(x, out, tabx, taby, ln_g, ln_b)
    N, h, w, Cc = x.shape
    if out is None:
        out = torch.empty((N, H, W, Cc), dtype=out_dtype or x.dtype, device=x.device)
    check(lib().skimi_resize_bilinear(ptr(x), ptr(out), _dt(x), _dt(out), N, h, w, H, W, Cc, ptr(tabx), ptr(taby), ptr(ln_g),
                                      ptr(ln_b), ln_eps, _stream()), "skimi_resize_bilinear")
    return out


def resize_bilinear_planes(x, H, W, out, *, tabx=None, taby=None, records=False, zpage=None):
    _require_cuda(x, out, tabx, taby, zpage)
    N, h, w, Cc = x.shape
    check(lib().skimi_resize_bilinear_planes(ptr(x), ptr(out), N, h, w, H, W, Cc, ptr(tabx), ptr(taby), int(records),
                                             ptr(zpage), _stream()), "skimi_resize_bilinear_planes")
    return out


def add_uv_pos_(x, tabx, taby):
    _require_cuda(x, tabx, taby)
    N, H, W, Cc = x.shape
    check(lib().skimi_add_uv_pos(ptr(x), _dt(x), ptr(tabx), ptr(taby), N, H, W, Cc, _stream()), "skimi_add_uv_pos")
    return x


def add_uv_pos_records(x, rec, tabx=None, taby=None):
    _require_cuda(x, rec, tabx, taby)
    N, H, W, Cc = x.shape
    check(lib().skimi_add_uv_pos_records(ptr(x), ptr(tabx), ptr(taby), N, H, W, Cc, ptr(rec), _stream()),
          "skimi_add_uv_pos_records")
    return rec


def dpt_out(x, weight, bias, mode, *, pts=None, conf=None):
    _require_cuda(x, weight, bias, pts, conf)
    npix, n_out = x.shape[0], weight.shape[0]
    if pts is None:
        pts = torch.empty((npix, n_out - 1), dtype=torch.float32, device=x.device)
    if conf is None:
        conf = torch.empty((npix,), dtype=torch.float32, device=x.device)
    check(lib().skimi_dpt_out(ptr(x), _dt(x), ptr(weight), ptr(bias), n_out, ptr(pts), ptr(conf), npix, mode, _stream()),
          "skimi_dpt_out")
    return pts, conf


def patch_gather(img, p, Kp, *, out=None, out_dtype=torch.float32):
    _require_cuda(img, out)
    F, _, H, W = img.shape
    if out is None:
        out = torch.empty((F * (H // p) * (W // p), Kp), dtype=out_dtype, device=img.device)
    check(lib().skimi_patch_gather(ptr(img), ptr(out), _dt(out), F, H, W, p, Kp, _stream()), "skimi_patch_gather")
    return out


def adaln(xn, x, mod, *, out=None):
    _require_cuda(xn, x, mod, out)
    rows, D = x.shape
    if out is None:
        out = torch.empty_like(x)
    check(lib().skimi_adaln(ptr(xn), ptr(x), ptr(mod), ptr(out), rows, D, _stream()), "skimi_adaln")
    return out


def pose_update_(delta, pred_pad, act_out, first):
    _require_cuda(delta, pred_pad, act_out)
    check(lib().skimi_pose_update(ptr(delta), ptr(pred_pad), ptr(act_out), delta.shape[0], int(first), _stream()),
          "skimi_pose_update")
    return act_out


def special_tokens_(x, table, S):
    _require_cuda(x, table)
    F, P, Cc = x.shape
    check(lib().skimi_special_tokens(ptr(x), ptr(table), F, S, P, table.shape[1], Cc, _stream()), "skimi_special_tokens")
    return x


def track_avgpool2(x, *, out=None):
    _require_cuda(x, out)
    N, H, W, Cc = x.shape
    if out is None:
        out = torch.empty((N, H // 2, W // 2, Cc), dtype=torch.float32, device=x.device)
    check(lib().skimi_track_avgpool2(ptr(x), ptr(out), N, H, W, Cc, _stream()), "skimi_track_avgpool2")
    return out


def track_sample_border(fmap, img_stride, coords, coord_stride, B, N, H, W, Cc, *, out=None):
    _require_cuda(fmap, coords, out)
    if out is None:
        out = torch.empty((B, N, Cc), dtype=torch.float32, device=fmap.device)
    check(lib().skimi_track_sample_border(ptr(fmap), img_stride, ptr(coords), coord_stride, ptr(out), B, N, H, W, Cc,
                                          _stream()), "skimi_track_sample_border")
    return out


def track_corr_sample(tgt, fmap, coords, out, N, S, r, level, ldo, out_off):
    _require_cuda(tgt, fmap, coords, out)
    rows, Cc = tgt.shape
    _, H, W, _ = fmap.shape
    check(lib().skimi_track_corr_sample(ptr(tgt), ptr(fmap), ptr(coords), ptr(out), rows, N, S, H, W, Cc, r, level, ldo,
                                        out_off, _stream()), "skimi_track_corr_sample")
    return out


def track_pos_embed_sample(coords, coord_stride, BN, H, W, D, *, out=None):
    _require_cuda(coords, out)
    if out is None:
        out = torch.empty((BN, D), dtype=torch.float32, device=coords.device)
    check(lib().skimi_track_pos_embed_sample(ptr(coords), coord_stride, ptr(out), BN, H, W, D, _stream()),
          "skimi_track_pos_embed_sample")
    return out


def track_input(coords, fcorr, tfeat, pos, qrt, x, S, L, ldx, max_scale):
    _require_cuda(coords, fcorr, tfeat, pos, qrt, x)
    check(lib().skimi_track_input(ptr(coords), ptr(fcorr), ptr(tfeat), ptr(pos), ptr(qrt), ptr(x), coords.shape[0], S, L, ldx,
                                  max_scale, _stream()), "skimi_track_input")
    return x


def track_coord_update_(coords, delta, ldd, query, N, S, stride, *, pred=None):
    _require_cuda(coords, delta, query, pred)
    check(lib().skimi_track_coord_update(ptr(coords), ptr(delta), ldd, ptr(query), ptr(pred), coords.shape[0], N, S, stride,
                                         _stream()), "skimi_track_coord_update")
    return coords


def track_init(q, coords, qs, S, stride):
    _require_cuda(q, coords, qs)
    check(lib().skimi_track_init(ptr(q), ptr(coords), ptr(qs), q.shape[0], S, stride, _stream()), "skimi_track_init")
    return coords, qs


def track_repeat_rows(src, S, *, out=None):
    _require_cuda(src, out)
    BN, Cc = src.shape
    if out is None:
        out = torch.empty((BN, S, Cc), dtype=torch.float32, device=src.device)
    check(lib().skimi_track_repeat_rows(ptr(src), ptr(out), BN, S, Cc, _stream()), "skimi_track_repeat_rows")
    return out


def track_bns_to_bsn(x, *, out=None):
    _require_cuda(x, out)
    B, N, S = x.shape
    if out is None:
        out = torch.empty((B, S, N), dtype=torch.float32, device=x.device)
    check(lib().skimi_track_bns_to_bsn(ptr(x), ptr(out), B, N, S, _stream()), "skimi_track_bns_to_bsn")
    return out
```

Measured before the change: 18.06.

## Fuse bilinear upsample into the direct 3x3 conv with persistent tiles

Adds a templated UP variant of the direct n32 conv kernel that stages the low-res source window and position tables into LDS and performs the bilinear interpolation plus hi/lo bf16 split in-kernel. This removes the separate upsample launch and the full-resolution hi/lo record buffer round trip through HBM. The fused path runs as a persistent grid capped at the CU count, prefetching the next tile's slice during the last slice of the current one. The trade-off is LDS pressure, per-slice interpolation work done on the ALUs, and extra barriers. The bilinear math is moved into shared helpers so both paths round identically.

```diff
diff --git a/include/skimi.h b/include/skimi.h
--- a/include/skimi.h
+++ b/include/skimi.h
@@ -109,6 +109,9 @@
                       int32_t F, int32_t H, int32_t W, int32_t C, int32_t relu, void* stream);
 int skimi_conv3x3_n32_strided(const void* in_hi, const void* in_lo, const void* packed_w, const float* bias, float* out,
                               int32_t F, int32_t H, int32_t W, int32_t C, int32_t relu, int64_t px_stride, void* stream);
+int skimi_conv3x3_n32_upsampled(const float* src, int32_t h, int32_t w, const float* tabx, const float* taby,
+                                const void* packed_w, const float* bias, float* out, int32_t F, int32_t H, int32_t W, int32_t C,
+                                int32_t relu, void* rec, int32_t* fused, void* stream);
 
 int skimi_resample_u8(const uint8_t* in, uint8_t* out, int64_t outer, int32_t n_in, int32_t n_out, int64_t inner,
                       const int32_t* kk, const int32_t* bounds, int32_t ksize, void* stream);
diff --git a/skiing_analysis_pytorch_amd/_lib.py b/skiing_analysis_pytorch_amd/_lib.py
--- a/skiing_analysis_pytorch_amd/_lib.py
+++ b/skiing_analysis_pytorch_amd/_lib.py
@@ -77,6 +77,8 @@
                                           C.c_float, _vp]),
     "skimi_conv3x3_n32_pack": (C.c_int, [_vp, _vp, C.c_int32, _vp]),
     "skimi_conv3x3_n32": (C.c_int, [_vp, _vp, _vp, _vp, _vp, C.c_int32, C.c_int32, C.c_int32, C.c_int32, C.c_int32, _vp]),
+    "skimi_conv3x3_n32_upsampled": (C.c_int, [_vp, C.c_int32, C.c_int32, _vp, _vp, _vp, _vp, _vp, C.c_int32, C.c_int32, C.c_int32,
+                                              C.c_int32, C.c_int32, _vp, _vp, _vp]),
     "skimi_conv3x3_n32_strided": (C.c_int, [_vp, _vp, _vp, _vp, _vp, C.c_int32, C.c_int32, C.c_int32, C.c_int32, C.c_int32,
                                             C.c_int64, _vp]),
     "skimi_layernorm": (C.c_int, [_vp, _vp, C.c_int64, C.c_int64, C.c_int32, _vp, _vp, C.c_float, _vp,
diff --git a/skiing_analysis_pytorch_amd/csrc/api.hip b/skiing_analysis_pytorch_amd/csrc/api.hip
--- a/skiing_analysis_pytorch_amd/csrc/api.hip
+++ b/skiing_analysis_pytorch_amd/csrc/api.hip
@@ -156,6 +156,21 @@
     return conv_direct_n32_launch((const unsigned short*)in_hi, (const unsigned short*)in_lo,
                                   (const unsigned short*)packed_w, bias, out, F, H, W, C, relu, (hipStream_t)stream,
                                   (long)px_stride);
+}
+
+int skimi_conv3x3_n32_upsampled(const float* src, int32_t h, int32_t w, const float* tabx, const float* taby,
+                                const void* packed_w, const float* bias, float* out, int32_t F, int32_t H, int32_t W, int32_t C,
+                                int32_t relu, void* rec, int32_t* fused, void* stream) {
+    const bool up = conv_direct_n32_up_eligible(h, w, H, W, C);
+    if (fused) *fused = up;
+    if (up)
+        return conv_direct_n32_up_launch(src, h, w, tabx, taby, (const unsigned short*)packed_w, bias, out, F, H, W, C, relu,
+                                         (hipStream_t)stream);
+    SKIMI_CHECK_ARG(rec != nullptr, "skimi_conv3x3_n32_upsampled: the two-launch path needs rec");
+    const int rc = bilinear_ac_planes_launch(src, (unsigned short*)rec, F, h, w, H, W, C, (hipStream_t)stream, tabx, taby);
+    if (rc != SKIMI_OK) return rc;
+    return conv_direct_n32_launch((const unsigned short*)rec, (const unsigned short*)rec + C, (const unsigned short*)packed_w, bias,
+                                  out, F, H, W, C, relu, (hipStream_t)stream, 2L * C);
 }
 
 int skimi_split_planes(const float* x, int64_t ld, int64_t rows, int32_t C, void* hi, void* lo, void* stream) {
diff --git a/skiing_analysis_pytorch_amd/csrc/conv_direct.hip b/skiing_analysis_pytorch_amd/csrc/conv_direct.hip
--- a/skiing_analysis_pytorch_amd/csrc/conv_direct.hip
+++ b/skiing_analysis_pytorch_amd/csrc/conv_direct.hip
@@ -1,6 +1,8 @@
 #include "common.h"
+#include "env.h"
 #include "gfx950.h"
 #include "kernels.h"
+#include "vggt_kernels.h"
 
 namespace skimi {
 
@@ -42,76 +44,151 @@
     float* out;
     int F, H, W, C, relu, tiles_x, tiles_y;
     long px_stride;
+    const float* src;
+    const float* tabx;
+    const float* taby;
+    int h, w_src;
+    float sy, sx;
 };
 
+constexpr int CU_SRC = 12;
+constexpr int CU_SRC_BUF = CU_SRC * CU_SRC * 128;
+constexpr int CU_TAB_BUF = 3 * 1024;
+constexpr int CU_W0 = 2 * CD_IN_PLANE;
+constexpr int CU_SRC0 = CU_W0 + 2 * 2 * CD_W_PLANE;
+constexpr int CU_TAB0 = CU_SRC0 + 2 * CU_SRC_BUF;
+constexpr int CU_LDS = CU_TAB0 + 2 * CU_TAB_BUF;
+static_assert(CU_LDS <= 160 * 1024, "conv_direct: the fused window staging does not fit the LDS");
+
+template <bool UP>
 __global__ __launch_bounds__(512, 2) void conv_direct_n32_kernel(const ConvDirectArgs p) {
     extern __shared__ __attribute__((aligned(16))) char smem[];
     const int tid = threadIdx.x, lane = tid & 63;
     const int wave = __builtin_amdgcn_readfirstlane(tid >> 6);
     const int l31 = lane & 31, lh = lane >> 5;
 
-    int bid = blockIdx.x;
-    const int tx = bid % p.tiles_x;
-    bid /= p.tiles_x;
-    const int ty = bid % p.tiles_y;
-    const int f = bid / p.tiles_y;
-    const int y0 = ty * 16, x0 = tx * 16;
+    const int ntiles = p.F * p.tiles_y * p.tiles_x;
     const int nsl = p.C / 32;
     const unsigned short* zero = reinterpret_cast<const unsigned short*>(g_conv_zero_page);
 
+    const int nin = UP ? (wave < 2 ? 3 : 2) : (wave < 5 ? 3 : 2);
+    int f, y0, x0;
+    int ys0 = 0, xs0 = 0;
     long in_off[3];
-    int in_piece[3];
-    int nin = 0;
+    int tab_row[2] = {0, 0};
+    auto plan_tile = [&](int t) {
+        x0 = (t % p.tiles_x) * 16;
+        t /= p.tiles_x;
+        y0 = (t % p.tiles_y) * 16;
+        f = t / p.tiles_y;
+        if constexpr (UP) {
+            ys0 = bilinear_ac_tap(p.sy, max(y0 - 1, 0), p.h).i0;
+            xs0 = bilinear_ac_tap(p.sx, max(x0 - 1, 0), p.w_src).i0;
+#pragma unroll
+            for (int j = 0; j < 3; ++j) {
+                const int sp = 8 * (wave + 8 * j) + (lane >> 3);
+                const int ry = sp / CU_SRC, rx = sp - ry * CU_SRC;
+                const int y = min(ys0 + ry, p.h - 1), x = min(xs0 + rx, p.w_src - 1);
+                in_off[j] = (((long)f * p.h + y) * p.w_src + x) * p.C + (lane & 7) * 4;
+            }
+            const int i = min(8 * (7 - wave) + (lane >> 3), 17);
+            tab_row[0] = min(max(x0 - 1 + i, 0), p.W - 1) * (p.C / 2);
+            tab_row[1] = min(max(y0 - 1 + i, 0), p.H - 1) * (p.C / 2);
+        } else {
+#pragma unroll
+            for (int j = 0; j < 3; ++j) {
+                const int px = 16 * (wave + 8 * j) + (lane >> 2);
+                const int hy = px / 18, hx = px - hy * 18;
+                const int y = y0 - 1 + hy, x = x0 - 1 + hx;
+                const int sc = (lane & 3) ^ (((hx + 2 * hy) >> 2) & 3);
+                in_off[j] = -1;
+                if (px < CD_WIN && y >= 0 && y < p.H && x >= 0 && x < p.W)
+                    in_off[j] = (((long)f * p.H + y) * p.W + x) * p.px_stride + sc * 8;
+            }
+        }
+    };
+    int w_off[3];
+    const int nw = wave < 2 ? 3 : 2;
 #pragma unroll
     for (int j = 0; j < 3; ++j) {
-        const int q = wave + 8 * j;
-        in_piece[j] = q;
-        in_off[j] = -1;
-        if (q < 21) {
-            nin = j + 1;
-            const int px = 16 * q + (lane >> 2);
-            const int hy = px / 18, hx = px - hy * 18;
-            const int y = y0 - 1 + hy, x = x0 - 1 + hx;
-            const int sc = (lane & 3) ^ (((hx + 2 * hy) >> 2) & 3);
-            if (px < CD_WIN && y >= 0 && y < p.H && x >= 0 && x < p.W)
-                in_off[j] = (((long)f * p.H + y) * p.W + x) * p.px_stride + sc * 8;
-        }
-    }
-    int w_off[3], w_piece[3];
-    int nw = 0;
-#pragma unroll
-    for (int j = 0; j < 3; ++j) {
-        const int q = wave + 8 * j;
-        w_piece[j] = q;
-        w_off[j] = 0;
-        if (q < 18) {
-            nw = j + 1;
-            const int row = 16 * q + (lane >> 2);
-            const int sc = (lane & 3) ^ ((row >> 2) & 3);
-            w_off[j] = row * 32 + sc * 8;
-        }
+        const int row = 16 * (wave + 8 * j) + (lane >> 2);
+        const int sc = (lane & 3) ^ ((row >> 2) & 3);
+        w_off[j] = row * 32 + sc * 8;
     }
     auto stage = [&](int buf, int s) {
-        char* base = smem + buf * CD_BUF;
-#pragma unroll
-        for (int j = 0; j < 3; ++j) {
-            if (j < nin) {
-                const bool ok = in_off[j] >= 0;
-                const unsigned short* sh = ok ? p.in_hi + in_off[j] + s * 32 : zero;
-                const unsigned short* sl = ok ? p.in_lo + in_off[j] + s * 32 : zero;
-                char* dst = base + in_piece[j] * 1024;
-                __builtin_amdgcn_global_load_lds((gbl_void*)sh, (lds_void*)dst, 16, 0, 0);
-                __builtin_amdgcn_global_load_lds((gbl_void*)sl, (lds_void*)(dst + CD_IN_PLANE), 16, 0, 0);
+        char* base = smem + (UP ? 0 : buf * CD_BUF);
+        if constexpr (UP) {
+            char* sb = smem + CU_SRC0 + buf * CU_SRC_BUF;
+#pragma unroll
+            for (int j = 0; j < 3; ++j) {
+                if (j < nin)
+                    __builtin_amdgcn_global_load_lds((gbl_void*)(p.src + in_off[j] + s * 32), (lds_void*)(sb + (wave + 8 * j) * 1024),
+                                                     16, 0, 0);
+            }
+            if (p.tabx != nullptr && wave >= 5) {
+                const int half = p.C / 2, cg = s * 32 + (lane & 7) * 4;
+                const float* e = cg < half ? p.tabx + tab_row[0] + cg : p.taby + tab_row[1] + (cg - half);
+                __builtin_amdgcn_global_load_lds((gbl_void*)e, (lds_void*)(smem + CU_TAB0 + buf * CU_TAB_BUF + (7 - wave) * 1024), 16,
+                                                 0, 0);
+            }
+        } else {
+#pragma unroll
+            for (int j = 0; j < 3; ++j) {
+                if (j < nin) {
+                    const bool ok = in_off[j] >= 0;
+                    const unsigned short* sh = ok ? p.in_hi + in_off[j] + s * 32 : zero;
+                    const unsigned short* sl = ok ? p.in_lo + in_off[j] + s * 32 : zero;
+                    char* dst = base + (wave + 8 * j) * 1024;
+                    __builtin_amdgcn_global_load_lds((gbl_void*)sh, (lds_void*)dst, 16, 0, 0);
+                    __builtin_amdgcn_global_load_lds((gbl_void*)sl, (lds_void*)(dst + CD_IN_PLANE), 16, 0, 0);
+                }
             }
         }
         const unsigned short* ws = p.w + (long)s * 2 * 9216;
+        char* wb = base + 2 * CD_IN_PLANE + (UP ? buf * 2 * CD_W_PLANE : 0);
 #pragma unroll
         for (int j = 0; j < 3; ++j) {
             if (j < nw) {
-                char* dst = base + 2 * CD_IN_PLANE + w_piece[j] * 1024;
+                char* dst = wb + (wave + 8 * j) * 1024;
                 __builtin_amdgcn_global_load_lds((gbl_void*)(ws + w_off[j]), (lds_void*)dst, 16, 0, 0);
                 __builtin_amdgcn_global_load_lds((gbl_void*)(ws + 9216 + w_off[j]), (lds_void*)(dst + CD_W_PLANE), 16, 0, 0);
             }
+        }
+    };
+    auto interpolate = [&](int buf, int s, int ty0, int tx0, int tys0, int txs0) {
+        const char* sb = smem + CU_SRC0 + buf * CU_SRC_BUF;
+        const char* tb = smem + CU_TAB0 + buf * CU_TAB_BUF;
+        const bool add_e = p.tabx != nullptr;
+#pragma unroll 1
+        for (int i = tid; i < 4 * CD_WIN; i += 512) {
+            const int px = i >> 2, c4 = i & 3;
+            const int hy = px / 18, hx = px - hy * 18;
+            const int Y = ty0 - 1 + hy, X = tx0 - 1 + hx;
+            bf16x8 hi = {0, 0, 0, 0, 0, 0, 0, 0}, lo = {0, 0, 0, 0, 0, 0, 0, 0};
+            if (Y >= 0 && Y < p.H && X >= 0 && X < p.W) {
+                const BilinearTap ty = bilinear_ac_tap(p.sy, Y, p.h), tx = bilinear_ac_tap(p.sx, X, p.w_src);
+                const int r0 = (ty.i0 - tys0) * CU_SRC, r1 = (ty.i1 - tys0) * CU_SRC, c0 = tx.i0 - txs0, c1 = tx.i1 - txs0;
+                float p00[8], p01[8], p10[8], p11[8], e[8] = {0.f, 0.f, 0.f, 0.f, 0.f, 0.f, 0.f, 0.f};
+                auto ld8 = [&](const char* q, float* d) {
+                    const float4 a = *reinterpret_cast<const float4*>(q), b = *reinterpret_cast<const float4*>(q + 16);
+                    d[0] = a.x; d[1] = a.y; d[2] = a.z; d[3] = a.w; d[4] = b.x; d[5] = b.y; d[6] = b.z; d[7] = b.w;
+                };
+                ld8(sb + (r0 + c0) * 128 + c4 * 32, p00);
+                ld8(sb + (r0 + c1) * 128 + c4 * 32, p01);
+                ld8(sb + (r1 + c0) * 128 + c4 * 32, p10);
+                ld8(sb + (r1 + c1) * 128 + c4 * 32, p11);
+                if (add_e) ld8(tb + (s * 32 + c4 * 8 < p.C / 2 ? hx : hy) * 128 + c4 * 32, e);
+#pragma unroll
+                for (int k = 0; k < 8; ++k) {
+                    short hb, lb;
+                    bilinear_ac_split(ty, tx, p00[k], p01[k], p10[k], p11[k], add_e, e[k], hb, lb);
+                    hi[k] = hb;
+                    lo[k] = lb;
+                }
+            }
+            char* dst = smem + px * 64 + ((c4 ^ (((hx + 2 * hy) >> 2) & 3)) << 4);
+            *reinterpret_cast<bf16x8*>(dst) = hi;
+            *reinterpret_cast<bf16x8*>(dst + CD_IN_PLANE) = lo;
         }
     };
 
@@ -129,55 +206,89 @@
 #pragma unroll
     for (int ks = 0; ks < 2; ++ks) b_off[ks] = l31 * 64 + (((2 * ks + lh) ^ ((l31 >> 2) & 3)) << 4);
 
-    f32x16 acc;
-#pragma unroll
-    for (int r = 0; r < 16; ++r) acc[r] = 0.f;
-
+    float bs = p.bias ? p.bias[l31] : 0.f;
+
+    int t = blockIdx.x;
+    int par = 0;
+    plan_tile(t);
     stage(0, 0);
     __syncthreads();
-    for (int s = 0; s < nsl; ++s) {
-        const int cur = s & 1;
-        if (s + 1 < nsl) stage(cur ^ 1, s + 1);
-        const char* ih = smem + cur * CD_BUF;
-        const char* wh = ih + 2 * CD_IN_PLANE;
-#pragma unroll
-        for (int tap = 0; tap < 9; ++tap) {
-#pragma unroll
-            for (int ks = 0; ks < 2; ++ks) {
-                const bf16x8 a_hi = *reinterpret_cast<const bf16x8*>(ih + a_off[tap][ks]);
-                const bf16x8 a_lo = *reinterpret_cast<const bf16x8*>(ih + CD_IN_PLANE + a_off[tap][ks]);
-                const bf16x8 w_hi = *reinterpret_cast<const bf16x8*>(wh + tap * 2048 + b_off[ks]);
-                const bf16x8 w_lo = *reinterpret_cast<const bf16x8*>(wh + CD_W_PLANE + tap * 2048 + b_off[ks]);
-                acc = __builtin_amdgcn_mfma_f32_32x32x16_bf16(a_lo, w_hi, acc, 0, 0, 0);
-                acc = __builtin_amdgcn_mfma_f32_32x32x16_bf16(a_hi, w_lo, acc, 0, 0, 0);
-                acc = __builtin_amdgcn_mfma_f32_32x32x16_bf16(a_hi, w_hi, acc, 0, 0, 0);
-            }
-        }
-        __syncthreads();
-    }
-
-    const float bs = p.bias ? p.bias[l31] : 0.f;
-    const bool interior = y0 + 16 <= p.H && x0 + 16 <= p.W;
-    float* ob = p.out + ((long)f * p.H * p.W) * 32 + l31;
-    if (interior) {
-#pragma unroll
-        for (int r = 0; r < 16; ++r) {
-            const int pix = (r & 3) + 8 * (r >> 2) + 4 * lh;
-            const int y = y0 + 2 * wave + (pix >> 4), x = x0 + (((pix & 15) + ((pix >> 4) ? 14 : 0)) & 15);
-            float v = acc[r] + bs;
-            if (p.relu) v = fmaxf(v, 0.f);
-            ob[((long)y * p.W + x) * 32] = v;
-        }
-    } else {
+    asm volatile("" : "+v"(bs));
+    for (;;) {
+        const int tf = f, ty0 = y0, tx0 = x0, tys0 = ys0, txs0 = xs0;
+        const bool more = UP && ntiles - t > (int)gridDim.x;
+        f32x16 acc;
+#pragma unroll
+        for (int r = 0; r < 16; ++r) acc[r] = 0.f;
+        for (int s = 0; s < nsl; ++s) {
+            if constexpr (UP) interpolate(par, s, ty0, tx0, tys0, txs0);
+            if (s + 1 < nsl) {
+                stage(par ^ 1, s + 1);
+            } else if (more) {
+                plan_tile(t + (int)gridDim.x);
+                stage(par ^ 1, 0);
+            }
+            if constexpr (UP) {
+                wait_lgkmcnt0();
+                fenced_barrier();
+            }
+            const char* ih = smem + (UP ? 0 : par * CD_BUF);
+            const char* wh = ih + 2 * CD_IN_PLANE + (UP ? par * 2 * CD_W_PLANE : 0);
+#pragma unroll
+            for (int tap = 0; tap < 9; ++tap) {
+#pragma unroll
+                for (int ks = 0; ks < 2; ++ks) {
+                    const bf16x8 a_hi = *reinterpret_cast<const bf16x8*>(ih + a_off[tap][ks]);
+                    const bf16x8 a_lo = *reinterpret_cast<const bf16x8*>(ih + CD_IN_PLANE + a_off[tap][ks]);
+                    const bf16x8 w_hi = *reinterpret_cast<const bf16x8*>(wh + tap * 2048 + b_off[ks]);
+                    const bf16x8 w_lo = *reinterpret_cast<const bf16x8*>(wh + CD_W_PLANE + tap * 2048 + b_off[ks]);
+                    acc = __builtin_amdgcn_mfma_f32_32x32x16_bf16(a_lo, w_hi, acc, 0, 0, 0);
+                    acc = __builtin_amdgcn_mfma_f32_32x32x16_bf16(a_hi, w_lo, acc, 0, 0, 0);
+                    acc = __builtin_amdgcn_mfma_f32_32x32x16_bf16(a_hi, w_hi, acc, 0, 0, 0);
+                }
+            }
+            par ^= 1;
+            __syncthreads();
+        }
+
+        const bool interior = ty0 + 16 <= p.H && tx0 + 16 <= p.W;
+        float* ob = p.out + ((long)tf * p.H * p.W) * 32 + l31;
+        if (interior) {
+#pragma unroll
+            for (int r = 0; r < 16; ++r) {
+                const int pix = (r & 3) + 8 * (r >> 2) + 4 * lh;
+                const int y = ty0 + 2 * wave + (pix >> 4), x = tx0 + (((pix & 15) + ((pix >> 4) ? 14 : 0)) & 15);
+                float v = acc[r] + bs;
+                if (p.relu) v = fmaxf(v, 0.f);
+                ob[((long)y * p.W + x) * 32] = v;
+            }
+        } else {
 #pragma unroll 1
-        for (int r = 0; r < 16; ++r) {
-            const int pix = (r & 3) + 8 * (r >> 2) + 4 * lh;
-            const int y = y0 + 2 * wave + (pix >> 4), x = x0 + (((pix & 15) + ((pix >> 4) ? 14 : 0)) & 15);
-            float v = acc[r] + bs;
-            if (p.relu) v = fmaxf(v, 0.f);
-            if (y < p.H && x < p.W) ob[((long)y * p.W + x) * 32] = v;
-        }
-    }
+            for (int r = 0; r < 16; ++r) {
+                const int pix = (r & 3) + 8 * (r >> 2) + 4 * lh;
+                const int y = ty0 + 2 * wave + (pix >> 4), x = tx0 + (((pix & 15) + ((pix >> 4) ? 14 : 0)) & 15);
+                float v = acc[r] + bs;
+                if (p.relu) v = fmaxf(v, 0.f);
+                if (y < p.H && x < p.W) ob[((long)y * p.W + x) * 32] = v;
+            }
+        }
+        if (!more) break;
+        t += (int)gridDim.x;
+    }
+}
+
+static int cu_count(int* cus) {
+    static std::atomic<int> seen[32];
+    int dev = 0;
+    SKIMI_HIP(hipGetDevice(&dev));
+    int n = seen[dev & 31].load(std::memory_order_relaxed);
+    if (n == 0) {
+        SKIMI_HIP(hipDeviceGetAttribute(&n, hipDeviceAttributeMultiprocessorCount, dev));
+        SKIMI_CHECK_ARG(n > 0, "conv_direct: the device reports no compute units");
+        seen[dev & 31].store(n, std::memory_order_relaxed);
+    }
+    *cus = n;
+    return SKIMI_OK;
 }
 
 int conv_direct_n32_launch(const unsigned short* in_hi, const unsigned short* in_lo, const unsigned short* w_packed,
@@ -190,8 +301,8 @@
     SKIMI_CHECK_ARG(px_stride >= C, "conv_direct: px_stride < C");
     SKIMI_CHECK_ARG(px_stride % 8 == 0, "conv_direct: px_stride %% 8 != 0 (16-B aligned pixels)");
     constexpr size_t lds = 2ull * CD_BUF;
-    SKIMI_LDS_OPT_IN(conv_direct_n32_kernel, lds, "conv_direct");
-    ConvDirectArgs a;
+    SKIMI_LDS_OPT_IN(conv_direct_n32_kernel<false>, lds, "conv_direct");
+    ConvDirectArgs a = {};
     a.in_hi = in_hi; a.in_lo = in_lo; a.w = w_packed; a.bias = bias; a.out = out;
     a.F = F; a.H = H; a.W = W; a.C = C; a.relu = relu;
     a.px_stride = px_stride;
@@ -199,9 +310,52 @@
     a.tiles_y = (int)cdiv(H, 16);
     const long nblk = (long)F * a.tiles_x * a.tiles_y;
     SKIMI_CHECK_ARG(nblk < (1l << 31), "conv_direct: grid too large");
-    hipLaunchKernelGGL(conv_direct_n32_kernel, dim3((unsigned)nblk), dim3(512), lds, st, a);
+    hipLaunchKernelGGL(conv_direct_n32_kernel<false>, dim3((unsigned)nblk), dim3(512), lds, st, a);
     SKIMI_LAUNCH_CHECK();
     return SKIMI_OK;
 }
 
-}
+static bool up_axis_fits(int n_src, int n_out) {
+    const float scale = n_out > 1 ? (float)(n_src - 1) / (float)(n_out - 1) : 0.f;
+    for (int o = 0; o < n_out; o += 16) {
+        const int first = o > 0 ? o - 1 : 0, last = o + 16 < n_out ? o + 16 : n_out - 1;
+        if (bilinear_ac_tap(scale, last, n_src).i1 - bilinear_ac_tap(scale, first, n_src).i0 + 1 > CU_SRC) return false;
+    }
+    return true;
+}
+
+bool conv_direct_n32_up_eligible(int h, int w, int H, int W, int C) {
+    return env_switch("SKIMI_DPT_TAIL_FUSED", 1) != 0 && C % 32 == 0 && C >= 32 && h > 0 && w > 0 && H > 0 && W > 0 &&
+           up_axis_fits(h, H) && up_axis_fits(w, W);
+}
+
+int conv_direct_n32_up_launch(const float* src, int h, int w, const float* tabx, const float* taby,
+                              const unsigned short* w_packed, const float* bias, float* out, int F, int H, int W, int C, int relu,
+                              hipStream_t st) {
+    SKIMI_CHECK_ARG(src && w_packed && out, "conv_direct: null buffer");
+    SKIMI_CHECK_ARG(F > 0 && conv_direct_n32_up_eligible(h, w, H, W, C), "conv_direct: shape not eligible for the fused upsample");
+    SKIMI_CHECK_ARG((((uintptr_t)src | (uintptr_t)w_packed | (uintptr_t)tabx | (uintptr_t)taby) & 15) == 0, "conv_direct: 16-B alignment");
+    SKIMI_CHECK_ARG(tabx == nullptr || taby != nullptr, "fused uv pos embed needs both tables");
+    ConvDirectArgs a = {};
+    a.w = w_packed; a.bias = bias; a.out = out;
+    a.F = F; a.H = H; a.W = W; a.C = C; a.relu = relu;
+    a.src = src; a.tabx = tabx; a.taby = taby; a.h = h; a.w_src = w;
+    a.sy = H > 1 ? (float)(h - 1) / (float)(H - 1) : 0.f;
+    a.sx = W > 1 ? (float)(w - 1) / (float)(W - 1) : 0.f;
+    a.tiles_x = (int)cdiv(W, 16);
+    a.tiles_y = (int)cdiv(H, 16);
+    const long nblk = (long)F * a.tiles_x * a.tiles_y;
+    SKIMI_CHECK_ARG(nblk < (1l << 31), "conv_direct: grid too large");
+    int cus = 0;
+    const int rc = cu_count(&cus);
+    if (rc != SKIMI_OK) return rc;
+    long grid = nblk < cus ? nblk : cus;
+    const long cap = env_switch("SKIMI_CONV_DIRECT_GRID", 0);
+    if (cap > 0 && cap < grid) grid = cap;
+    SKIMI_LDS_OPT_IN(conv_direct_n32_kernel<true>, CU_LDS, "conv_direct");
+    hipLaunchKernelGGL(conv_direct_n32_kernel<true>, dim3((unsigned)grid), dim3(512), CU_LDS, st, a);
+    SKIMI_LAUNCH_CHECK();
+    return SKIMI_OK;
+}
+
+}
diff --git a/skiing_analysis_pytorch_amd/csrc/kernels.h b/skiing_analysis_pytorch_amd/csrc/kernels.h
--- a/skiing_analysis_pytorch_amd/csrc/kernels.h
+++ b/skiing_analysis_pytorch_amd/csrc/kernels.h
@@ -87,6 +87,10 @@
 int conv_direct_n32_launch(const unsigned short* in_hi, const unsigned short* in_lo, const unsigned short* w_packed,
                            const float* bias, float* out, int F, int H, int W, int C, int relu, hipStream_t st,
                            long px_stride = 0);
+bool conv_direct_n32_up_eligible(int h, int w, int H, int W, int C);
+int conv_direct_n32_up_launch(const float* src, int h, int w, const float* tabx, const float* taby,
+                              const unsigned short* w_packed, const float* bias, float* out, int F, int H, int W, int C, int relu,
+                              hipStream_t st);
 
 int vp3d_im2col_launch(const float* x, float* a0, int B, int L, int Cin, int k, int Kpad, hipStream_t st);
 
diff --git a/skiing_analysis_pytorch_amd/csrc/vggt_dpt.hip b/skiing_analysis_pytorch_amd/csrc/vggt_dpt.hip
--- a/skiing_analysis_pytorch_amd/csrc/vggt_dpt.hip
+++ b/skiing_analysis_pytorch_amd/csrc/vggt_dpt.hip
@@ -214,17 +214,25 @@
     const bool direct = !w.feature_only && w.oc2a_direct != nullptr && adt == SKIMI_F32 && !no_direct;
     void* c2 = nullptr;
     if (direct) {
+        const bool up = conv_direct_n32_up_eligible(h1, w1, Ho, Wo, f2);
         const size_t pe = (size_t)F * Ho * Wo * f2;
-        unsigned short* rec = (unsigned short*)c.ar.alloc(pe * 4);
+        unsigned short* rec = up ? nullptr : (unsigned short*)c.ar.alloc(pe * 4);
         c2 = c.ar.alloc((size_t)F * Ho * Wo * 32 * es);
-        c.run([&] {
-            return bilinear_ac_planes_launch((const float*)c1, rec, F, h1, w1, Ho, Wo, f2, c.st, uvt ? uvt->tx : nullptr,
-                                             uvt ? uvt->ty : nullptr);
-        });
-        c.run([&] {
-            return conv_direct_n32_launch(rec, rec + f2, w.oc2a_direct, w.oc2a.lin.b, (float*)c2, F, Ho, Wo, f2, 1, c.st,
-                                          2L * f2);
-        });
+        if (up) {
+            c.run([&] {
+                return conv_direct_n32_up_launch((const float*)c1, h1, w1, uvt ? uvt->tx : nullptr, uvt ? uvt->ty : nullptr,
+                                                 w.oc2a_direct, w.oc2a.lin.b, (float*)c2, F, Ho, Wo, f2, 1, c.st);
+            });
+        } else {
+            c.run([&] {
+                return bilinear_ac_planes_launch((const float*)c1, rec, F, h1, w1, Ho, Wo, f2, c.st, uvt ? uvt->tx : nullptr,
+                                                 uvt ? uvt->ty : nullptr);
+            });
+            c.run([&] {
+                return conv_direct_n32_launch(rec, rec + f2, w.oc2a_direct, w.oc2a.lin.b, (float*)c2, F, Ho, Wo, f2, 1, c.st,
+                                              2L * f2);
+            });
+        }
     } else {
         const int udt = (w.feature_only && w.out_f32) ? SKIMI_F32 : adt;
         void* c1u = c.ar.alloc((size_t)F * Ho * Wo * f2 * Ctx::esz(udt));
diff --git a/skiing_analysis_pytorch_amd/csrc/vggt_kernels.h b/skiing_analysis_pytorch_amd/csrc/vggt_kernels.h
--- a/skiing_analysis_pytorch_amd/csrc/vggt_kernels.h
+++ b/skiing_analysis_pytorch_amd/csrc/vggt_kernels.h
@@ -29,4 +29,30 @@
 int pad_cols_launch(const float* in, float* out, long rows, int K, int Kp, hipStream_t st);
 int tile_vec_launch(const float* in, float* out, int n, int reps, hipStream_t st);
 
+struct BilinearTap {
+    int i0, i1;
+    float l0, l1;
+};
+inline __host__ __device__ BilinearTap bilinear_ac_tap(float scale, int I, int n) {
+#pragma clang fp contract(off)
+    const float f = scale * I;
+    BilinearTap t;
+    t.i0 = (int)f < n - 1 ? (int)f : n - 1;
+    t.i1 = t.i0 + 1 < n - 1 ? t.i0 + 1 : n - 1;
+    t.l1 = fminf(fmaxf(f - t.i0, 0.f), 1.f);
+    t.l0 = 1.f - t.l1;
+    return t;
 }
+#ifdef __HIPCC__
+__device__ __forceinline__ void bilinear_ac_split(const BilinearTap& ty, const BilinearTap& tx, float p00, float p01, float p10,
+                                                  float p11, bool add_e, float e, short& hi, short& lo) {
+#pragma clang fp contract(off)
+    float r = ty.l0 * (tx.l0 * p00 + tx.l1 * p01) + ty.l1 * (tx.l0 * p10 + tx.l1 * p11);
+    if (add_e) r += e;
+    const unsigned short hb = f2bf(r);
+    hi = (short)hb;
+    lo = (short)f2bf(r - bf2f(hb));
+}
+#endif
+
+}
diff --git a/skiing_analysis_pytorch_amd/csrc/vggt_kernels.hip b/skiing_analysis_pytorch_amd/csrc/vggt_kernels.hip
--- a/skiing_analysis_pytorch_amd/csrc/vggt_kernels.hip
+++ b/skiing_analysis_pytorch_amd/csrc/vggt_kernels.hip
@@ -163,11 +163,8 @@
     for (int i = blockIdx.x * 256 + threadIdx.x; i < rowlen; i += gridDim.x * 256) {
         const int X = i / C8;
         const int c8 = i - X * C8;
-        const float fy = sy * Y, fx = sx * X;
-        const int y0 = min((int)fy, h - 1), x0 = min((int)fx, w - 1);
-        const int y1 = min(y0 + 1, h - 1), x1 = min(x0 + 1, w - 1);
-        const float ly1 = fminf(fmaxf(fy - y0, 0.f), 1.f), lx1 = fminf(fmaxf(fx - x0, 0.f), 1.f);
-        const float ly0 = 1.f - ly1, lx0 = 1.f - lx1;
+        const BilinearTap ty = bilinear_ac_tap(sy, Y, h), tx = bilinear_ac_tap(sx, X, w);
+        const int y0 = ty.i0, y1 = ty.i1, x0 = tx.i0, x1 = tx.i1;
         const float* base = in + n * (long)h * w * C + c8 * 8;
         float p00[8], p01[8], p10[8], p11[8];
         auto ld8 = [&](const float* q, float* d) {
@@ -178,23 +175,18 @@
         ld8(base + ((long)y0 * w + x1) * C, p01);
         ld8(base + ((long)y1 * w + x0) * C, p10);
         ld8(base + ((long)y1 * w + x1) * C, p11);
-        float r[8];
-#pragma unroll
-        for (int k = 0; k < 8; ++k)
-            r[k] = ly0 * (lx0 * p00[k] + lx1 * p01[k]) + ly1 * (lx0 * p10[k] + lx1 * p11[k]);
+        float e[8] = {0.f, 0.f, 0.f, 0.f, 0.f, 0.f, 0.f, 0.f};
         if (tabx != nullptr) {
             const int half = C / 2, c = c8 * 8;
-            float e[8];
             ld8(c < half ? tabx + (long)X * half + c : taby + (long)Y * half + (c - half), e);
-#pragma unroll
-            for (int k = 0; k < 8; ++k) r[k] += e[k];
         }
         bf16x8 hi, lo;
 #pragma unroll
         for (int k = 0; k < 8; ++k) {
-            const unsigned short hb = f2bf(r[k]);
-            hi[k] = (short)hb;
-            lo[k] = (short)f2bf(r[k] - bf2f(hb));
+            short hb, lb;
+            bilinear_ac_split(ty, tx, p00[k], p01[k], p10[k], p11[k], tabx != nullptr, e[k], hb, lb);
+            hi[k] = hb;
+            lo[k] = lb;
         }
         const long pix = ((n * H + Y) * (long)W + X) * 2 * C;
         if (slice_records) {
diff --git a/skiing_analysis_pytorch_amd/ops.py b/skiing_analysis_pytorch_amd/ops.py
--- a/skiing_analysis_pytorch_amd/ops.py
+++ b/skiing_analysis_pytorch_amd/ops.py
@@ -317,6 +317,20 @@
     return out
 
 
+def conv3x3_n32_upsampled(src, H, W, packed, bias=None, relu=False, *, tabx=None, taby=None, out=None):
+    _require_cuda(src, packed, bias, tabx, taby, out)
+    F_, h, w, Cc = src.shape
+    assert src.dtype == torch.float32 and src.is_contiguous()
+    if out is None:
+        out = torch.empty((F_, H, W, 32), dtype=torch.float32, device=src.device)
+    rec = torch.empty((F_, H, W, 2 * Cc), dtype=torch.bfloat16, device=src.device)
+    fused = C.c_int32(-1)
+    check(lib().skimi_conv3x3_n32_upsampled(ptr(src), h, w, ptr(tabx), ptr(taby), ptr(packed), ptr(bias), ptr(out), F_, H, W, Cc,
+                                            1 if relu else 0, ptr(rec), C.byref(fused), _lib.current_stream()),
+          "skimi_conv3x3_n32_upsampled")
+    return out, bool(fused.value)
+
+
 def split_records(x):
     _require_cuda(x)
     rows, Cc = x.shape
```

Result: faster. 18.25 (median of 6 runs) (+1.0%).
